# zengyan-97/X2-VLM

Hardware: AMD Instinct MI355X
Metric: image-text pairs/sec (fwd+bwd) X2VLM-base 224px bs=64/GPU (higher is better)
Workload: dtype bf16

## Files before the change

include/x2vlm_hip.h:

```cpp
#ifndef X2VLM_HIP_H
#define X2VLM_HIP_H
#include <stdint.h>
#ifdef __cplusplus
extern "C" {
#endif

const char* x2_last_error(void);
int x2_abi_version(void);
int x2_device_cus(void);
int x2_tune(int key, int value);
int x2_tune_get(int key);

int x2_gemm_nt(const void* A, const void* B, void* C, int M, int N, int K, int lda, int ldb, int ldc,
               const float* bias, const float* gamma, const float* resid, int ldr, void* aux, int ldaux,
               int act, int out_f32, unsigned drop_thr16, unsigned drop_seed, float drop_scale, const unsigned* drop_epoch,
               const float* rowscale, float* colsum, void* stream);

int x2_gemm_nt_dgelu_colparts(const void* A, const void* B, void* C, int M, int N, int K, int lda, int ldb, int ldc,
                              const void* aux, int ldaux, float* colparts, int* nrows_out, void* stream);
int x2_gemm_nt_splitk(const void* A, const void* B, float* C, int M, int N, int K, int lda, int ldb, int ldc,
                      int slices, float* ws, long ws_floats, void* stream);

int x2_gemm_tn_grouped(const int64_t* problems, int count, int accumulate, int split, float* ws, long ws_floats,
                       void* stream);

typedef struct X2AttnArgs {
  const void *Q, *K, *V, *O, *dO;
  void *Out, *dQ, *dK, *dV, *dS;
  float *LSE, *Delta;
  long q_bs, q_rs, k_bs, k_rs, v_bs, v_rs, o_bs, o_rs;
  long dq_bs, dq_rs, dk_bs, dk_rs, dv_bs, dv_rs, do_bs, do_rs;
  int B, Bkv, H, Lq, Lk;
  float scale;
  const float* bias;  int bias_ld;
  const float* biasT; int biasT_ld;
  const float* mask;  int mask_ld;
  const int* kv_idx;
  const int* seq_off; const int* seq_ids;
  int ds_ld;
  unsigned drop_thr16, drop_seed; float drop_scale;
  int dbg;
  int head_dim;
  const unsigned* drop_epoch;
  int grid_nx, grid_ny, grid_nz, grid_map;
  int phase;
  float* ws; long ws_floats;
  float* colsum_ws;
} X2AttnArgs;
int x2_attn_fwd(const X2AttnArgs* args, void* stream);
int x2_attn_bwd(const X2AttnArgs* args, void* stream);
int x2_attn_bwd_one_pass(const X2AttnArgs* args);

int x2_layernorm_fwd(const float* x, const float* w, const float* b, void* y_bf16, float* y_f32, float* mean,
                     float* rstd, int rows, int D, float eps, int period, unsigned drop_thr16, unsigned drop_seed,
                     float drop_scale, const unsigned* drop_epoch, void* stream);
int x2_layernorm_bwd(const void* dy , int dy_is_bf16, const float* x, const float* mean, const float* rstd, const float* w,
                     const float* dres, float* dx, void* dx_bf16, float* dw, float* db, float* dcol, int rows, int D,
                     int period, unsigned in_thr16, unsigned in_seed, float in_scale, unsigned out_thr16,
                     unsigned out_seed, float out_scale, const unsigned* drop_epoch, float* ws ,
                     int defer, int post, const float* post_rowscale, void* stream);
int x2_colsum_bf16(const void* y, float* out, int M, int N, int ld, float* ws , int defer, void* stream);
int x2_reduce_partials(const float* part, int nblk, int nk, int width, float* o0, float* o1, float* o2, void* stream);
int x2_reduce_partials_multi(const int64_t* desc, int count, void* stream);
int x2_layerscale_finish(const int64_t* desc, int count, void* stream);
int x2_rowscale_cast_colsum(const float* dx, const float* rowscale, void* dx_bf16, float* colsum, int M, int D,
                            float* ws , int defer, void* stream);
int x2_cast_bf16(const float* src, void* dst, long n, void* stream);
int x2_cast_transpose_bf16(const float* src, void* dst, void* dstT, int R, int C, int ldt, void* stream);
int x2_cast_transpose_multi(const int64_t* desc, int count, void* stream);
int x2_copy_f32_multi(const int64_t* desc, int count, void* stream);
int x2_patchify(const float* image, void* cols, int B, int R, int ps, void* stream);
int x2_assemble_tokens(const float* patch, const float* cls, float* x, int B, int P, int D, void* stream);
int x2_assemble_tokens_bwd(const float* dx, void* dpatch_bf16, float* dcls, int B, int P, int D, void* stream);
int x2_pool_tokens(float* x, const float* w, int B, int P, int D, int bwd, void* stream);
int x2_relpos_bias(const float* table, const long* index, const long* indexT , float* bias, float* biasT, int N, int H, int ld, int ldT,
                   float scale, void* stream);
int x2_relpos_bias_bwd(const void* dS, const int* inv_off, const int* inv_pos, float* dtable, int B, int N, int H, int ld,
                       int T, float* ws, int slices, void* stream);

int x2_embed_fwd(const long* ids, const float* word, const float* pos, const float* type0, float* out, int R, int L,
                 int D, void* stream);
int x2_embed_bwd(const long* ids, const float* g, float* dword, float* dpos, float* dtype0, int R, int L, int D,
                 float* scratch, void* stream);
int x2_gather_rows(const float* src, const int* idx, float* dst, void* dst_bf16, int R, long len, void* stream);
int x2_scatter_rows(const float* src, const int* idx, float* dst, int R, int D, long len, void* stream);
int x2_linear_f32(const float* A, const float* B, float* C, const float* bias, const float* alpha_ptr, float alpha,
                  int M, int N, int K, long sam, long sak, long sbn, long sbk, long ldc, int accumulate,
                  int ksplit ,
                  float* ws , void* stream);
int x2_l2norm(const float* x, const float* dy, float* out, int R, int D, int bwd, void* stream);
int x2_ce_fwd(const float* logits, long ld, const long* labels, int R, int C, float* lse, float* loss_row, float* out2,
              void* stream);
int x2_ce_bwd(const float* logits, long ld, const long* labels, const float* lse, const float* g, const float* stat,
              float gscale, int R, int C, float* dl_f32, void* dl_bf16, long ldd, void* stream);
int x2_mlm_ce_fwd(const void* X, const void* E, const float* bias, const long* labels, int R, int Vp, int V, int Hd,
                  int ldx, int lde, float* part, float* zlab, void* stream);
int x2_ce_combine(const float* part, int chunks, const float* zlab, const long* labels, int R, float* lse, float* loss_row,
                  float* out2, void* stream);
int x2_mlm_ce_bwd(const void* X, const void* E, const float* bias, const long* labels, const float* lse, const float* g,
                  const float* stat, float gscale, int R, int Vp, int V, int Hd, int ldx, int lde, void* dl_bf16, long ldd,
                  void* stream);
int x2_mask_tokens(const long* text_ids, const long* text_atts, int B, int L, const unsigned char* is_subword, int vocab,
                   const unsigned* words, int words_ld, unsigned seed, const unsigned* epoch, double mask_prob, int max_masks,
                   double skipgram_prb, int skipgram_size, int mask_whole_word, long cls_id, long mask_id, long pad_id, long pad_mask,
                   long* text_ids_masked, long* masked_pos, long* masked_ids, void* stream);
int x2_sample_negatives(const float* sim, int n, const long* group, const float* u, int* out, void* stream);
int x2_additive_mask(const long* atts, float* out, int S, int L, int Lp, float neg, void* stream);

int x2_attn_fwd_mask2d(const X2AttnArgs* args, const float* mask2d, int mask2d_ld, void* stream);
int x2_attn_bwd_mask2d(const X2AttnArgs* args, const float* mask2d, int mask2d_ld, void* stream);
int x2_additive_mask2d(const long* m, float* out, int S, int L, int Lp, float neg, void* stream);
int x2_embed_fwd_pid(const long* ids, const long* pids, const float* word, const float* pos, const float* type0, float* out, int R, int D,
                     void* stream);
int x2_embed_bwd_pid(const long* ids, const long* pids, const float* g, float* dword, float* dpos, float* dtype0, int R, int L, int D,
                     float* scratch, void* stream);
int x2_mlm_ls_fwd(const void* X, const void* E, const float* bias, const long* labels, long ignore, int R, int Vp, int V, int Hd, int ldx,
                  int lde, float* part, float* sumz, float* zlab, float* zign, void* stream);
int x2_ls_combine(const float* part, const float* sumz, int chunks, const float* zlab, const float* zign, const long* labels, const float* w,
                  int R, int V, long ignore, float ls, float* lse, float* kl_row, float* out2, void* stream);
int x2_mlm_ls_bwd(const void* X, const void* E, const float* bias, const long* labels, const float* w, const float* lse, const float* g,
                  const float* stat, float gscale, float ls, long ignore, int R, int Vp, int V, int Hd, int ldx, int lde, void* dl_bf16,
                  long ldd, void* stream);
int x2_kv_csr(const int* kv, int S, int Bi, int* off, int* order, void* stream);
int x2_tail_index(const int* ineg, const int* tneg, const long* text_atts , const long* image_atts , int B, int L,
                  int T, int with_match, int* t_idx, int* kv, long* atts_out , long* enc_out , void* stream);
int x2_droppath_rows(const float* rates, unsigned seed, const unsigned* epoch, int depth, int B, int T, float* out, void* stream);
int x2_frame_mean(const float* x, const float* pos, const float* dy, float* out, float* dpos, int Bc, int F, int T, int D, int bwd,
                  void* stream);
int x2_gelu_f32(const float* x, const float* dy, float* out, long n, void* stream);
int x2_colsum_f32(const float* x, float* out, int M, int N, void* stream);

int x2_attn_decode(const void* qkv, int qkv_ld, void* cache, void* out, int out_ld, int S, int H, int n_new, int hist, int Lmax, float scale,
                   void* stream);
int x2_beam_gather(const void* src, void* dst, const int* parent, int layers, int S, int Lmax, int row_elems, int hist, void* stream);
int x2_logprob_topk(const float* logits, int ldv, int V, int S, const int* seq, int Lseq, int seq_len, int ngram, int eos_id, int forbid_eos,
                    int K, float* out_vals, int* out_ids, float* logs, void* stream);

int x2_grad_norm(const void* table, int ntensors, int nblocks, float max_norm, float* partial, float* out2, void* stream);
int x2_adamw_multi(const void* table, int ntensors, int nblocks, const float* lr, const float* wd, int ngroups, float b1,
                   float b2, float eps, const float* clip2 , void* stream);

int x2_comm_unique_id(void* out128);
int x2_comm_init(const void* id128, int rank, int world, void** comm_out);
int x2_comm_info(void* comm, int* rank, int* world);
int x2_comm_allreduce_bucket(void* comm, void* buf, long count, int dtype, int average, void* done_event, void* stream);
int x2_comm_allgather(void* comm, const void* send, void* recv, long count_per_rank, int dtype, void* done_event, void* stream);
int x2_comm_broadcast(void* comm, void* buf, long count, int dtype, int root, void* done_event, void* stream);
int x2_comm_destroy(void* comm);

#ifdef __cplusplus
}
#endif
#endif
```

x2-vlm_amd/_lib.py:

```python
import ctypes as C
import os

import torch

_HERE = os.path.dirname(os.path.abspath(__file__))
LIB_PATH = os.environ.get("X2VLM_HIP_LIB") or os.path.join(_HERE, "libx2vlm_hip.so")

P, I, L, F, U = C.c_void_p, C.c_int, C.c_long, C.c_float, C.c_uint


class AttnArgs(C.Structure):
    _fields_ = [(n, P) for n in ("Q", "K", "V", "O", "dO", "Out", "dQ", "dK", "dV", "dS", "LSE", "Delta")] + \
               [(n, L) for n in ("q_bs", "q_rs", "k_bs", "k_rs", "v_bs", "v_rs", "o_bs", "o_rs",
                                 "dq_bs", "dq_rs", "dk_bs", "dk_rs", "dv_bs", "dv_rs", "do_bs", "do_rs")] + \
               [(n, I) for n in ("B", "Bkv", "H", "Lq", "Lk")] + [("scale", F)] + \
               [("bias", P), ("bias_ld", I), ("biasT", P), ("biasT_ld", I), ("mask", P), ("mask_ld", I),
                ("kv_idx", P), ("seq_off", P), ("seq_ids", P), ("ds_ld", I),
                ("drop_thr16", C.c_uint), ("drop_seed", C.c_uint), ("drop_scale", F), ("dbg", I), ("head_dim", I), ("drop_epoch", P),
                ("grid_nx", I), ("grid_ny", I), ("grid_nz", I), ("grid_map", I),
                ("phase", I), ("ws", P), ("ws_floats", L), ("colsum_ws", P)]


_SIGS = {
    "x2_gemm_nt": [P, P, P, I, I, I, I, I, I, P, P, P, I, P, I, I, I, U, U, F, P, P, P, P],
    "x2_gemm_nt_splitk": [P, P, P, I, I, I, I, I, I, I, P, L, P],
    "x2_gemm_nt_dgelu_colparts": [P, P, P, I, I, I, I, I, I, P, I, P, C.POINTER(I), P],
    "x2_gemm_tn_grouped": [P, I, I, I, P, L, P],
    "x2_attn_fwd": [C.POINTER(AttnArgs), P],
    "x2_attn_bwd": [C.POINTER(AttnArgs), P],
    "x2_layernorm_fwd": [P, P, P, P, P, P, P, I, I, F, I, U, U, F, P, P],
    "x2_layernorm_bwd": [P, I, P, P, P, P, P, P, P, P, P, P, I, I, I, U, U, F, U, U, F, P, P, I, I, P, P],
    "x2_colsum_bf16": [P, P, I, I, I, P, I, P],
    "x2_reduce_partials": [P, I, I, I, P, P, P, P],
    "x2_reduce_partials_multi": [P, I, P],
    "x2_cast_transpose_multi": [P, I, P],
    "x2_copy_f32_multi": [P, I, P],
    "x2_layerscale_finish": [P, I, P],
    "x2_rowscale_cast_colsum": [P, P, P, P, I, I, P, I, P],
    "x2_cast_bf16": [P, P, L, P],
    "x2_cast_transpose_bf16": [P, P, P, I, I, I, P],
    "x2_patchify": [P, P, I, I, I, P],
    "x2_assemble_tokens": [P, P, P, I, I, I, P],
    "x2_assemble_tokens_bwd": [P, P, P, I, I, I, P],
    "x2_pool_tokens": [P, P, I, I, I, I, P],
    "x2_relpos_bias": [P, P, P, P, P, I, I, I, I, F, P],
    "x2_relpos_bias_bwd": [P, P, P, P, I, I, I, I, I, P, I, P],
    "x2_embed_fwd": [P, P, P, P, P, I, I, I, P],
    "x2_embed_bwd": [P, P, P, P, P, I, I, I, P, P],
    "x2_gather_rows": [P, P, P, P, I, L, P],
    "x2_scatter_rows": [P, P, P, I, I, L, P],
    "x2_linear_f32": [P, P, P, P, P, F, I, I, I, L, L, L, L, L, I, I, P, P],
    "x2_l2norm": [P, P, P, I, I, I, P],
    "x2_ce_fwd": [P, L, P, I, I, P, P, P, P],
    "x2_ce_bwd": [P, L, P, P, P, P, F, I, I, P, P, L, P],
    "x2_mlm_ce_fwd": [P, P, P, P, I, I, I, I, I, I, P, P, P],
    "x2_ce_combine": [P, I, P, P, I, P, P, P, P],
    "x2_mlm_ce_bwd": [P, P, P, P, P, P, P, F, I, I, I, I, I, I, P, L, P],
    "x2_sample_negatives": [P, I, P, P, P, P],
    "x2_mask_tokens": [P, P, I, I, P, I, P, I, U, P, C.c_double, I, C.c_double, I, I, L, L, L, L, P, P, P, P],
    "x2_additive_mask": [P, P, I, I, I, F, P],
    "x2_kv_csr": [P, I, I, P, P, P],
    "x2_tail_index": [P, P, P, P, I, I, I, I, P, P, P, P, P],
    "x2_droppath_rows": [P, U, P, I, I, I, P, P],
    "x2_frame_mean": [P, P, P, P, P, I, I, I, I, I, P],
    "x2_gelu_f32": [P, P, P, L, P],
    "x2_grad_norm": [P, I, I, F, P, P, P],
    "x2_adamw_multi": [P, I, I, P, P, I, F, F, F, P, P],
    "x2_colsum_f32": [P, P, I, I, P],
    "x2_attn_fwd_mask2d": [C.POINTER(AttnArgs), P, I, P],
    "x2_attn_bwd_mask2d": [C.POINTER(AttnArgs), P, I, P],
    "x2_additive_mask2d": [P, P, I, I, I, F, P],
    "x2_embed_fwd_pid": [P, P, P, P, P, P, I, I, P],
    "x2_embed_bwd_pid": [P, P, P, P, P, P, I, I, I, P, P],
    "x2_mlm_ls_fwd": [P, P, P, P, L, I, I, I, I, I, I, P, P, P, P, P],
    "x2_ls_combine": [P, P, I, P, P, P, P, I, I, L, F, P, P, P, P],
    "x2_mlm_ls_bwd": [P, P, P, P, P, P, P, P, F, F, L, I, I, I, I, I, I, P, L, P],
    "x2_attn_decode": [P, I, P, P, I, I, I, I, I, I, F, P],
    "x2_beam_gather": [P, P, P, I, I, I, I, I, P],
    "x2_logprob_topk": [P, I, I, I, P, I, I, I, I, I, I, P, P, P, P],
}
_COMM_SIGS = {
    "x2_comm_unique_id": [P],
    "x2_comm_init": [P, I, I, C.POINTER(P)],
    "x2_comm_info": [P, C.POINTER(I), C.POINTER(I)],
    "x2_comm_allreduce_bucket": [P, P, L, I, I, P, P],
    "x2_comm_allgather": [P, P, P, L, I, P, P],
    "x2_comm_broadcast": [P, P, L, I, I, P, P],
    "x2_comm_destroy": [P],
}
EXPORTS = sorted(list(_SIGS) + list(_COMM_SIGS) + ["x2_last_error", "x2_abi_version", "x2_device_cus", "x2_tune", "x2_tune_get",
                                                         "x2_attn_bwd_one_pass"])

_lib = None


class X2HipError(RuntimeError):
    pass


def lib():
    global _lib
    if _lib is None:
        if not os.path.exists(LIB_PATH):
            raise X2HipError("HIP extension %s not built: run `python -c 'import __graft_entry__ as g; g.build()'`"
                             % LIB_PATH)
        try:
            h = C.CDLL(LIB_PATH)
        except OSError as e:
            raise X2HipError("cannot load %s: %s" % (LIB_PATH, e))
        for name, sig in list(_SIGS.items()) + list(_COMM_SIGS.items()):
            fn = getattr(h, name)
            fn.argtypes, fn.restype = sig, I
        h.x2_last_error.restype = C.c_char_p
        h.x2_abi_version.restype = I
        h.x2_device_cus.restype = I
        h.x2_tune.argtypes, h.x2_tune.restype = [I, I], I
        h.x2_tune_get.argtypes, h.x2_tune_get.restype = [I], I
        h.x2_attn_bwd_one_pass.argtypes, h.x2_attn_bwd_one_pass.restype = [C.POINTER(AttnArgs)], I
        for kv in filter(None, os.environ.get("X2_TUNE", "").split(",")):
            k, v = kv.split("=")
            if h.x2_tune(int(k), int(v)) != 0:
                raise X2HipError("X2_TUNE=%s: %s" % (kv, h.x2_last_error().decode()))
        _lib = h
    return _lib


_get_device = torch._C._cuda_getDevice if hasattr(torch._C, "_cuda_getDevice") else None
_get_raw_stream = getattr(torch._C, "_cuda_getCurrentRawStream", None)


def raw_stream():
    return _get_raw_stream(_get_device())


def call(name, *args):
    h = _lib or lib()
    rc = getattr(h, name)(*args, _get_raw_stream(_get_device()))
    if rc != 0:
        raise X2HipError("%s failed (%d): %s" % (name, rc, h.x2_last_error().decode()))


def ptr(t):
    return None if t is None else t.data_ptr()
```

x2-vlm_amd/csrc/gemm.hip:

```cpp
#include "x2_common.h"
#include <type_traits>

#define BM 128
#define BN 128
#define BK 64
#define TILE_BYTES (128 * 128)
#define STAGE_BYTES (2 * TILE_BYTES)
#define GEMM_LDS_BYTES (2 * STAGE_BYTES)

struct GemmNT {
  const bf16_t* A; const bf16_t* B; void* C;
  const float* bias; const float* gamma; const float* resid; bf16_t* aux;
  int M, N, K;
  int lda, ldb, ldc, ldr, ldaux;
  int act;
  int out_f32;
  int group_m;
  DropSpec drop;
  const uint32_t* drop_epoch;
  const float* rowscale;
  float* colsum;
  int dbg;
  int ksplit;
  const long* ce_labels;
  const float* ce_lse;
  const float* ce_g;
  const float* ce_stat;
  float* ce_part;
  float* ce_zlab;
  float ce_gscale;
  int ce_C;
  float* ce_sumz;
  float* ce_zign;
  long ce_ignore;
  float ce_ls;
  const float* ce_w;
};

__device__ __forceinline__ void tile_coords(int t, int tiles_m, int tiles_n, int gm, int& tm, int& tn) {
  const int gsz = gm * tiles_n, g = t / gsz, first = g * gm;
  const int rows = min(gm, tiles_m - first), r = t - g * gsz;
  tm = first + r % rows;
  tn = r / rows;
}

__device__ __forceinline__ void st16(void* p, u32x4 v, bool wt) {
  if (wt) asm volatile("global_store_dwordx4 %0, %1, off sc1\n\ts_nop 1" ::"v"(p), "v"(v) : "memory");
  else *reinterpret_cast<u32x4*>(p) = v;
}

#ifdef X2_PROBE
#define NT_DBG(p, bit) (((p).dbg & (bit)) != 0)
static __device__ unsigned long long* g_nt_probe = nullptr;
#define NT_STAMP(i) do { if (g_nt_probe && threadIdx.x == 0) g_nt_probe[(size_t)blockIdx.x * 4 + (i)] = wall_clock64(); } while (0)
#define NT_ABL_DECL(p) const bool abl_dma_ = NT_DBG(p, 32), abl_rd_ = NT_DBG(p, 64), abl_mm_ = NT_DBG(p, 128); bool rd_ = true
#define NT_ABL_NO_DMA(kt) if (abl_dma_ && (kt) >= 2) return
#define NT_ABL_NO_READ() if (!rd_) return
#define NT_ABL_NO_MFMA() if (abl_mm_) return
#define NT_ABL_STEP(kt) if (abl_rd_ && (kt) > 0) rd_ = false
#else
#define NT_ABL_DECL(p)
#define NT_ABL_NO_DMA(kt)
#define NT_ABL_NO_READ()
#define NT_ABL_NO_MFMA()
#define NT_ABL_STEP(kt)
#define NT_DBG(p, bit) false
#define NT_STAMP(i) do { } while (0)
#endif
typedef __attribute__((ext_vector_type(16))) float f32x16;
template <int TM>
__device__ __forceinline__ void epi_stage_half(f32x4 (&acc)[TM][4], int half, bool full, float* stg, int lane) {
  const int frow = lane & 15, fg = lane >> 4;
#pragma unroll
  for (int ii = 0; ii < 2; ++ii)
#pragma unroll
    for (int j = 0; j < 4; ++j)
      if (full || ii == 0) *reinterpret_cast<f32x4*>(stg + (ii * 16 + frow) * 68 + j * 16 + fg * 4) = acc[full ? half * 2 + ii : half * 2][j];
}
template <int RT>
__device__ __forceinline__ void epi_stage_half(f32x16 (&acc)[RT][2], int half, bool, float* stg, int lane) {
  const int row = lane & 31, h = lane >> 5;
#pragma unroll
  for (int tj = 0; tj < 2; ++tj)
#pragma unroll
    for (int g = 0; g < 4; ++g)
      *reinterpret_cast<f32x4*>(stg + row * 68 + tj * 32 + g * 8 + h * 4) =
          f32x4{acc[half][tj][4 * g], acc[half][tj][4 * g + 1], acc[half][tj][4 * g + 2], acc[half][tj][4 * g + 3]};
}
template <int V> struct EpiTraits {
  static constexpr bool generic = V == 4;
  static constexpr int act = V == 2 ? 1 : (V == 3 || V == 10) ? 2 : 0;
  static constexpr bool out_f32 = V == 1 || V == 5 || V == 6 || V == 7;
  static constexpr bool resid = V == 5 || V == 6;
  static constexpr bool scale = V == 6;
  static constexpr bool aux0 = false;
  static constexpr bool drop = V == 5;
  static constexpr bool colsum = false;
  static constexpr bool colparts = V == 10;
};
template <int TM, int VAR, class Acc>
__device__ __forceinline__ void nt_epilogue(const GemmNT& p, Acc& acc, char* smem, int wave, int lane, int mw0, int nw0, int prow = 0) {
  using E = EpiTraits<VAR>;
  const int act = E::generic ? p.act : E::act;
  const bool out_f32 = E::generic ? p.out_f32 != 0 : E::out_f32;
  const bool has_resid = E::generic ? p.resid != nullptr : E::resid;
  const bool has_scale = E::generic ? (p.gamma != nullptr || p.rowscale != nullptr) : E::scale;
  const bool has_aux0 = E::generic ? (p.act == 0 && p.aux != nullptr) : E::aux0;
  const bool has_drop = (E::generic || E::drop) ? p.drop.thr16 != 0 : false;
  const bool has_colsum = E::generic ? p.colsum != nullptr : (E::colsum && p.colsum != nullptr);
  float* stg = reinterpret_cast<float*>(smem) + wave * (32 * 68);
  const int er = lane >> 3, ec = (lane & 7) * 8;
  const int n = nw0 + ec;
  const bool nok = n < p.N;
  float bb[8], gg[8];
#pragma unroll
  for (int e = 0; e < 8; ++e) { bb[e] = 0.f; gg[e] = 1.f; }
  if (nok && p.bias) { const float4 b0 = *reinterpret_cast<const float4*>(p.bias + n), b1 = *reinterpret_cast<const float4*>(p.bias + n + 4);
    bb[0] = b0.x; bb[1] = b0.y; bb[2] = b0.z; bb[3] = b0.w; bb[4] = b1.x; bb[5] = b1.y; bb[6] = b1.z; bb[7] = b1.w; }
  if (nok && has_scale && p.gamma) { const float4 g0 = *reinterpret_cast<const float4*>(p.gamma + n), g1 = *reinterpret_cast<const float4*>(p.gamma + n + 4);
    gg[0] = g0.x; gg[1] = g0.y; gg[2] = g0.z; gg[3] = g0.w; gg[4] = g1.x; gg[5] = g1.y; gg[6] = g1.z; gg[7] = g1.w; }
  float cs[8] = {0.f, 0.f, 0.f, 0.f, 0.f, 0.f, 0.f, 0.f};
  const bool wt = NT_DBG(p, 16);
  const DropSpec drop_ = drop_at_epoch(p.drop, p.drop_epoch);
#pragma unroll
  for (int half = 0; half < (TM + 1) / 2; ++half) {
    const bool full = half * 2 + 1 < TM;
    float4 r0[4], r1[4];
    u32x4 pre[4];
    const int nc = nok ? n : 0;
    if (has_resid) {
#pragma unroll
      for (int rr = 0; rr < 4; ++rr) {
        if (!full && rr >= 2) continue;
        const int mc = min(mw0 + half * 32 + rr * 8 + er, p.M - 1);
        r0[rr] = *reinterpret_cast<const float4*>(p.resid + (size_t)mc * p.ldr + nc);
        r1[rr] = *reinterpret_cast<const float4*>(p.resid + (size_t)mc * p.ldr + nc + 4);
      }
    }
    if (act == 2) {
#pragma unroll
      for (int rr = 0; rr < 4; ++rr) {
        if (!full && rr >= 2) continue;
        const int mc = min(mw0 + half * 32 + rr * 8 + er, p.M - 1);
        pre[rr] = *reinterpret_cast<const u32x4*>(p.aux + (size_t)mc * p.ldaux + nc);
      }
    }
    epi_stage_half(acc, half, full, stg, lane);
#pragma unroll
    for (int rr = 0; rr < 4; ++rr) {
      if (!full && rr >= 2) continue;
      const int row = rr * 8 + er;
      const int m = mw0 + half * 32 + row;
      const float4 a0 = *reinterpret_cast<const float4*>(stg + row * 68 + ec), a1 = *reinterpret_cast<const float4*>(stg + row * 68 + ec + 4);
      if (m >= p.M || !nok) continue;
      float v[8] = {a0.x + bb[0], a0.y + bb[1], a0.z + bb[2], a0.w + bb[3], a1.x + bb[4], a1.y + bb[5], a1.z + bb[6], a1.w + bb[7]};
      if constexpr (VAR == 8) {
        const long lab = p.ce_labels[m];
        float mx = -INFINITY;
#pragma unroll
        for (int e = 0; e < 8; ++e) mx = n + e < p.ce_C ? fmaxf(mx, v[e]) : mx;
        mx = fmaxf(mx, __shfl_xor(mx, 1, 64)); mx = fmaxf(mx, __shfl_xor(mx, 2, 64)); mx = fmaxf(mx, __shfl_xor(mx, 4, 64));
        float se = 0.f;
#pragma unroll
        for (int e = 0; e < 8; ++e) {
          se += n + e < p.ce_C ? __expf(v[e] - mx) : 0.f;
          if ((long)(n + e) == lab) p.ce_zlab[m] = v[e];
        }
        se += __shfl_xor(se, 1, 64); se += __shfl_xor(se, 2, 64); se += __shfl_xor(se, 4, 64);
        if ((lane & 7) == 0) *reinterpret_cast<float2*>(p.ce_part + ((size_t)m * (p.N >> 6) + (nw0 >> 6)) * 2) = float2{mx, se};
        continue;
      }
      if constexpr (VAR == 11) {
        const long lab = p.ce_labels[m];
        float mx = -INFINITY, sz = 0.f;
#pragma unroll
        for (int e = 0; e < 8; ++e) { mx = n + e < p.ce_C ? fmaxf(mx, v[e]) : mx; sz += n + e < p.ce_C ? v[e] : 0.f; }
        mx = fmaxf(mx, __shfl_xor(mx, 1, 64)); mx = fmaxf(mx, __shfl_xor(mx, 2, 64)); mx = fmaxf(mx, __shfl_xor(mx, 4, 64));
        sz += __shfl_xor(sz, 1, 64); sz += __shfl_xor(sz, 2, 64); sz += __shfl_xor(sz, 4, 64);
        float se = 0.f;
#pragma unroll
        for (int e = 0; e < 8; ++e) {
          se += n + e < p.ce_C ? __expf(v[e] - mx) : 0.f;
          if ((long)(n + e) == lab) p.ce_zlab[m] = v[e];
          if ((long)(n + e) == p.ce_ignore) p.ce_zign[m] = v[e];
        }
        se += __shfl_xor(se, 1, 64); se += __shfl_xor(se, 2, 64); se += __shfl_xor(se, 4, 64);
        if ((lane & 7) == 0) {
          *reinterpret_cast<float2*>(p.ce_part + ((size_t)m * (p.N >> 6) + (nw0 >> 6)) * 2) = float2{mx, se};
          p.ce_sumz[(size_t)m * (p.N >> 6) + (nw0 >> 6)] = sz;
        }
        continue;
      }
      if constexpr (VAR == 12) {
        const long lab = p.ce_labels[m];
        const bool live = lab >= 0 && lab != p.ce_ignore;
        const float conf = 1.f - p.ce_ls, sm = p.ce_ls / (float)(p.ce_C - 2), qsum = conf + sm * (float)(p.ce_C - 2);
        const float sc = live ? p.ce_gscale * p.ce_g[0] * p.ce_w[m] / (p.ce_stat[1] + 1e-5f) : 0.f, l = p.ce_lse[m];
#pragma unroll
        for (int e = 0; e < 8; ++e) {
          const long c = n + e;
          const float q = c == lab ? conf : (c == p.ce_ignore ? 0.f : sm);
          v[e] = c < p.ce_C ? (qsum * __expf(v[e] - l) - q) * sc : 0.f;
        }
        st16(reinterpret_cast<bf16_t*>(p.C) + (size_t)m * p.ldc + n,
             u32x4{pack_bf16(v[0], v[1]), pack_bf16(v[2], v[3]), pack_bf16(v[4], v[5]), pack_bf16(v[6], v[7])}, false);
        continue;
      }
      if constexpr (VAR == 9) {
        const long lab = p.ce_labels[m];
        const float sc = lab >= 0 ? p.ce_gscale * p.ce_g[0] / p.ce_stat[1] : 0.f, l = p.ce_lse[m];
#pragma unroll
        for (int e = 0; e < 8; ++e) v[e] = n + e < p.ce_C ? (__expf(v[e] - l) - ((long)(n + e) == lab ? 1.f : 0.f)) * sc : 0.f;
        st16(reinterpret_cast<bf16_t*>(p.C) + (size_t)m * p.ldc + n,
             u32x4{pack_bf16(v[0], v[1]), pack_bf16(v[2], v[3]), pack_bf16(v[4], v[5]), pack_bf16(v[6], v[7])}, false);
        continue;
      }
      if (act == 1) {
        st16(p.aux + (size_t)m * p.ldaux + n, u32x4{pack_bf16(v[0], v[1]), pack_bf16(v[2], v[3]), pack_bf16(v[4], v[5]), pack_bf16(v[6], v[7])}, wt);
#pragma unroll
        for (int r = 0; r < 8; ++r) v[r] = gelu_f(v[r]);
      } else if (act == 2) {
#pragma unroll
        for (int r = 0; r < 4; ++r) { v[2 * r] *= dgelu_f(bf_lo(pre[rr][r])); v[2 * r + 1] *= dgelu_f(bf_hi(pre[rr][r])); }
      } else if (has_aux0) {
        st16(p.aux + (size_t)m * p.ldaux + n, u32x4{pack_bf16(v[0], v[1]), pack_bf16(v[2], v[3]), pack_bf16(v[4], v[5]), pack_bf16(v[6], v[7])}, wt);
      }
      if (has_drop) {
        float dm[4];
        drop_mul4(drop_, (uint32_t)m * (uint32_t)p.N + (uint32_t)n, dm);
        v[0] *= dm[0]; v[1] *= dm[1]; v[2] *= dm[2]; v[3] *= dm[3];
        drop_mul4(drop_, (uint32_t)m * (uint32_t)p.N + (uint32_t)n + 4u, dm);
        v[4] *= dm[0]; v[5] *= dm[1]; v[6] *= dm[2]; v[7] *= dm[3];
      }
      if (has_scale) {
        const float rs_ = p.rowscale ? p.rowscale[m] : 1.f;
#pragma unroll
        for (int r = 0; r < 8; ++r) v[r] *= gg[r] * rs_;
      }
      if (has_resid) {
        v[0] += r0[rr].x; v[1] += r0[rr].y; v[2] += r0[rr].z; v[3] += r0[rr].w;
        v[4] += r1[rr].x; v[5] += r1[rr].y; v[6] += r1[rr].z; v[7] += r1[rr].w;
      }
      if (has_colsum || E::colparts) {
#pragma unroll
        for (int r = 0; r < 8; ++r) cs[r] += v[r];
      }
      if (out_f32) {
        float* c = reinterpret_cast<float*>(p.C) + (size_t)m * p.ldc + n;
        st16(c, u32x4{__float_as_uint(v[0]), __float_as_uint(v[1]), __float_as_uint(v[2]), __float_as_uint(v[3])}, wt);
        st16(c + 4, u32x4{__float_as_uint(v[4]), __float_as_uint(v[5]), __float_as_uint(v[6]), __float_as_uint(v[7])}, wt);
      } else {
        st16(reinterpret_cast<bf16_t*>(p.C) + (size_t)m * p.ldc + n,
             u32x4{pack_bf16(v[0], v[1]), pack_bf16(v[2], v[3]), pack_bf16(v[4], v[5]), pack_bf16(v[6], v[7])}, wt);
      }
    }
  }
  if constexpr (E::colparts) {
#pragma unroll
    for (int e = 0; e < 8; ++e) { cs[e] += __shfl_xor(cs[e], 8, 64); cs[e] += __shfl_xor(cs[e], 16, 64); cs[e] += __shfl_xor(cs[e], 32, 64); }
    if (er == 0 && nok) {
      float* dst = p.colsum + (size_t)prow * p.N + n;
      *reinterpret_cast<float4*>(dst) = float4{cs[0], cs[1], cs[2], cs[3]};
      *reinterpret_cast<float4*>(dst + 4) = float4{cs[4], cs[5], cs[6], cs[7]};
    }
  }
  if (has_colsum) {
#pragma unroll
    for (int e = 0; e < 8; ++e) { cs[e] += __shfl_xor(cs[e], 8, 64); cs[e] += __shfl_xor(cs[e], 16, 64); cs[e] += __shfl_xor(cs[e], 32, 64); }
    if (er == 0 && nok) {
#pragma unroll
      for (int e = 0; e < 8; ++e) atomicAdd(p.colsum + n + e, cs[e]);
    }
  }
}

template <int TM, int VAR, class Acc>
__device__ __forceinline__ void nt_epilogue_f4(const GemmNT& p, Acc& acc, char* smem, int wave, int lane, int mw0, int nw0) {
  using E = EpiTraits<VAR>;
  static_assert(!E::generic && E::out_f32 && E::act == 0 && VAR <= 6, "nt_epilogue_f4: feature sets 1, 5, 6");
  const bool has_drop = E::drop ? p.drop.thr16 != 0 : false;
  float* stg = reinterpret_cast<float*>(smem) + wave * (32 * 68);
  const int er = lane >> 4, ec = (lane & 15) * 4;
  const int n = nw0 + ec;
  const bool nok = n < p.N;
  float bb[4] = {0.f, 0.f, 0.f, 0.f}, gg[4] = {1.f, 1.f, 1.f, 1.f};
  if (nok && p.bias) { const float4 b0 = *reinterpret_cast<const float4*>(p.bias + n); bb[0] = b0.x; bb[1] = b0.y; bb[2] = b0.z; bb[3] = b0.w; }
  if (E::scale && nok && p.gamma) { const float4 g0 = *reinterpret_cast<const float4*>(p.gamma + n); gg[0] = g0.x; gg[1] = g0.y; gg[2] = g0.z; gg[3] = g0.w; }
  const DropSpec drop_ = drop_at_epoch(p.drop, p.drop_epoch);
#pragma unroll
  for (int half = 0; half < (TM + 1) / 2; ++half) {
    const bool full = half * 2 + 1 < TM;
    float4 rs[4][2];
    const int nc = nok ? n : 0;
    if (E::resid) {
#pragma unroll
      for (int rr = 0; rr < 4; ++rr) {
        if (!full && rr >= 2) continue;
#pragma unroll
        for (int h = 0; h < 2; ++h) {
          const int mc = min(mw0 + half * 32 + rr * 8 + h * 4 + er, p.M - 1);
          rs[rr][h] = *reinterpret_cast<const float4*>(p.resid + (size_t)mc * p.ldr + nc);
        }
      }
    }
    epi_stage_half(acc, half, full, stg, lane);
#pragma unroll
    for (int rr = 0; rr < 4; ++rr) {
      if (!full && rr >= 2) continue;
#pragma unroll
      for (int h = 0; h < 2; ++h) {
        const int row = rr * 8 + h * 4 + er;
        const int m = mw0 + half * 32 + row;
        const float4 a0 = *reinterpret_cast<const float4*>(stg + row * 68 + ec);
        if (m >= p.M || !nok) continue;
        float v[4] = {a0.x + bb[0], a0.y + bb[1], a0.z + bb[2], a0.w + bb[3]};
        if (has_drop) {
          float dm[4];
          drop_mul4(drop_, (uint32_t)m * (uint32_t)p.N + (uint32_t)n, dm);
          v[0] *= dm[0]; v[1] *= dm[1]; v[2] *= dm[2]; v[3] *= dm[3];
        }
        if (E::scale) {
          const float rs_ = p.rowscale ? p.rowscale[m] : 1.f;
#pragma unroll
          for (int r = 0; r < 4; ++r) v[r] *= gg[r] * rs_;
        }
        if (E::resid) { v[0] += rs[rr][h].x; v[1] += rs[rr][h].y; v[2] += rs[rr][h].z; v[3] += rs[rr][h].w; }
        st16(reinterpret_cast<float*>(p.C) + (size_t)m * p.ldc + n,
             u32x4{__float_as_uint(v[0]), __float_as_uint(v[1]), __float_as_uint(v[2]), __float_as_uint(v[3])}, false);
      }
    }
  }
}

template <int TM, int VAR, bool F4 = false>
__global__ __launch_bounds__(256, 2) void gemm_nt_kernel(GemmNT p) {
  constexpr int BMT = 32 * TM;
  if constexpr (VAR == 7) {
    const int koff = blockIdx.y * p.ksplit;
    p.A += koff; p.B += koff;
    p.K = min(p.ksplit, p.K - koff);
    p.C = reinterpret_cast<float*>(p.C) + (size_t)blockIdx.y * p.M * p.ldc;
  }
  constexpr int A_BYTES = BMT * 128, STG = A_BYTES + TILE_BYTES;
  extern __shared__ __attribute__((aligned(16))) char smem[];
  const int tid = threadIdx.x, lane = tid & 63;
  const int wave = __builtin_amdgcn_readfirstlane(tid >> 6);
  const int wm = wave >> 1, wn = wave & 1;
  const int tiles_n = (p.N + BN - 1) / BN, tiles_m = (p.M + BMT - 1) / BMT;
  int tm, tn;
  tile_coords(xcd_remap(blockIdx.x, gridDim.x), tiles_m, tiles_n, p.group_m, tm, tn);
  const int m0 = tm * BMT, n0 = tn * BN;

  const bf16_t* srcA[TM]; const bf16_t* srcB[4];
#pragma unroll
  for (int i = 0; i < TM; ++i) {
    const int q = i * 256 + tid, row = q >> 3, c = (q & 7) ^ (row & 7);
    int ra = m0 + row; ra = ra < p.M ? ra : p.M - 1;
    srcA[i] = p.A + (size_t)ra * p.lda + c * 8;
  }
#pragma unroll
  for (int i = 0; i < 4; ++i) {
    const int q = i * 256 + tid, row = q >> 3, c = (q & 7) ^ (row & 7);
    int rb = n0 + row; rb = rb < p.N ? rb : p.N - 1;
    srcB[i] = p.B + (size_t)rb * p.ldb + c * 8;
  }
  auto stage = [&](int kt, int buf) {
    char* base = smem + buf * STG;
#pragma unroll
    for (int i = 0; i < TM; ++i) glds16(srcA[i] + (size_t)kt * BK, base + (i * 256 + wave * 64) * 16);
#pragma unroll
    for (int i = 0; i < 4; ++i) glds16(srcB[i] + (size_t)kt * BK, base + A_BYTES + (i * 256 + wave * 64) * 16);
  };

  f32x4 acc[TM][4];
#pragma unroll
  for (int i = 0; i < TM; ++i)
#pragma unroll
    for (int j = 0; j < 4; ++j) acc[i][j] = f32x4{0.f, 0.f, 0.f, 0.f};

  const uint32_t lds0 = lds_addr(smem);
  const int frow = lane & 15, fg = lane >> 4, fsw = lane & 7;
  const uint32_t offA = (uint32_t)((wm * 16 * TM + frow) * 128);
  const uint32_t offB = (uint32_t)(A_BYTES + (wn * 64 + frow) * 128);

  const int nk = p.K / BK;
  bf16x8 a0[TM], b0[4], a1[TM], b1[4];
  auto frags = [&](uint32_t sb, int ks, bf16x8 (&a)[TM], bf16x8 (&b)[4]) {
    const uint32_t cs = (uint32_t)(((ks * 4 + fg) ^ fsw) << 4);
#pragma unroll
    for (int j = 0; j < 4; ++j) b[j] = lds_read_b128(sb + offB + j * 2048 + cs);
#pragma unroll
    for (int i = 0; i < TM; ++i) a[i] = lds_read_b128(sb + offA + i * 2048 + cs);
  };
  auto mma = [&](bf16x8 (&a)[TM], bf16x8 (&b)[4], auto first, auto last) {
#pragma unroll
    for (int t = decltype(first)::value; t < decltype(last)::value; ++t)
      acc[t >> 2][t & 3] = __builtin_amdgcn_mfma_f32_16x16x32_bf16(b[t & 3], a[t >> 2], acc[t >> 2][t & 3], 0, 0, 0);
  };
  using I0 = std::integral_constant<int, 0>; using I1 = std::integral_constant<int, 1>; using IN = std::integral_constant<int, 4 * TM>;
  auto step = [&](int kt, auto refill, auto has_next) {
    mma(a0, b0, I0{}, I1{});
// ... 619 lines not shown
  X2_REQUIRE(K % BK == 0, "x2_gemm_nt: K=%d must be a multiple of %d", K, BK);
  X2_REQUIRE(N % 8 == 0, "x2_gemm_nt: N=%d must be a multiple of 8", N);
  X2_REQUIRE(lda % 8 == 0 && ldb % 8 == 0 && ldc % 8 == 0, "x2_gemm_nt: leading dims must keep 16-byte rows");
  X2_REQUIRE(act == 0 || aux, "x2_gemm_nt: act=%d needs aux", act);
  X2_REQUIRE((!resid || ldr % 4 == 0) && (!aux || ldaux % 8 == 0), "x2_gemm_nt: ldr/ldaux alignment");
  GemmNT p{(const bf16_t*)A, (const bf16_t*)B, C, bias, gamma, resid, (bf16_t*)aux, M, N, K, lda, ldb, ldc, ldr, ldaux, act, out_f32,
           g_tune[0] > 0 ? g_tune[0] : 8, DropSpec{drop_thr16, drop_seed, drop_scale}, drop_epoch, rowscale, colsum, g_tune[2], 0};
  int var = 4;
  {
    const bool plain = !gamma && !rowscale && !drop_thr16 && !colsum;
    if (act == 1 && !out_f32 && !resid && plain) var = 2;
    else if (act == 2 && !out_f32 && !resid && plain) var = 3;
    else if (act == 0 && !aux && !resid && plain) var = out_f32 ? 1 : 0;
    else if (act == 0 && !aux && resid && out_f32 && !gamma && !rowscale && !colsum) var = 5;
    else if (act == 0 && !aux && resid && out_f32 && gamma && !drop_thr16 && !colsum) var = 6;
  }
  double eff256 = 0.0;
  int tmw = nt256_plan(M, N, &eff256);
  if (g_tune[3] >= 5 && g_tune[3] <= 8) tmw = g_tune[3];
  const bool light = var == 0 || var == 1;
  bool auto256 = (light || K >= 2048) && eff256 * 100.0 >= NT256_MIN_FILL && !(resid && M < 8192);
  if ((var == 5 || var == 6) && M >= 8192 && eff256 * 100.0 >= NT256_MIN_FILL) auto256 = true;
  if (var == 2 && eff256 * 100.0 >= 90.0) auto256 = true;
  const bool use256 = var != 4 && N % 8 == 0 && (g_tune[1] == 3 || (g_tune[1] == 0 && g_tune[3] == 0 && auto256));
  const bool pp_ok = var != 4 && ((size_t)(M - 1) * lda + K) * 2 < (1ull << 31) && ((size_t)(N - 1) * ldb + K) * 2 < (1ull << 31);
  int pp_h = 0;
  if (g_tune[15] >= 3 && g_tune[15] <= 6) pp_h = g_tune[15];
  else if (g_tune[15] == 0 && g_tune[1] == 0 && g_tune[3] == 0 && !use256 && K >= 2048 && (var == 0 || var == 1 || var == 5)) {
    const int cus = x2_cus(), tn256 = (N + 255) / 256;
    for (int h = 3; h <= 4 && !pp_h; ++h) {
      const int tiles = ((M + 32 * h - 1) / (32 * h)) * tn256;
      if (tiles <= cus && tiles * 10 >= cus * 7) pp_h = h;
    }
  }
  if (pp_ok && pp_h) {
    switch (var) {
      case 0: launch_nt_pp_h<0>(p, pp_h, (hipStream_t)stream); break;
      case 1: launch_nt_pp_h<1>(p, pp_h, (hipStream_t)stream); break;
      case 2: launch_nt_pp_h<2>(p, pp_h, (hipStream_t)stream); break;
      case 3: launch_nt_pp_h<3>(p, pp_h, (hipStream_t)stream); break;
      case 5: launch_nt_pp_h<5>(p, pp_h, (hipStream_t)stream); break;
      default: launch_nt_pp_h<6>(p, pp_h, (hipStream_t)stream); break;
    }
    return x2_check_launch("x2_gemm_nt");
  }
  if (use256) {
    switch (var) {
      case 0: launch_nt256_h<0>(p, tmw, (hipStream_t)stream); break;
      case 1: launch_nt256_h<1>(p, tmw, (hipStream_t)stream); break;
      case 2: launch_nt256_h<2>(p, tmw, (hipStream_t)stream); break;
      case 3: launch_nt256_h<3>(p, tmw, (hipStream_t)stream); break;
      case 5: launch_nt256_h<5>(p, tmw, (hipStream_t)stream); break;
      default: launch_nt256_h<6>(p, tmw, (hipStream_t)stream); break;
    }
  } else {
    const int t128 = ((M + 127) / 128) * ((N + BN - 1) / BN), t192 = ((M + 191) / 192) * ((N + BN - 1) / BN);
    const int t64 = ((M + 63) / 64) * ((N + BN - 1) / BN);
    const int slots = 2 * x2_cus();
    const bool use64 = g_tune[3] == 3 || (g_tune[3] == 0 && (t128 <= slots || (t128 <= slots + slots / 6 && K <= 1024)));
    const bool use192 = !use64 && (g_tune[3] == 2 || (g_tune[3] == 0 && t128 > slots && t192 <= slots));
    const int t160 = ((M + 159) / 160) * ((N + BN - 1) / BN);
    const bool use160 = g_tune[3] == 4 || (use192 && g_tune[3] == 0 && t160 <= slots);
#define X2_NT_LAUNCH(V, SW)                                                                          \
    do {                                                                                              \
      if (use64) launch_nt<2, V, SW>(p, t64, (hipStream_t)stream);                                    \
      else if (use160) launch_nt<5, V, SW>(p, t160, (hipStream_t)stream);                             \
      else if (use192) launch_nt<6, V, SW>(p, t192, (hipStream_t)stream);                             \
      else launch_nt<4, V, SW>(p, t128, (hipStream_t)stream);                                         \
    } while (0)
    switch (var) {
      case 0: X2_NT_LAUNCH(0, false); break;
      case 2: X2_NT_LAUNCH(2, false); break;
      case 3: X2_NT_LAUNCH(3, false); break;
      case 1: X2_NT_LAUNCH(1, true); break;
      case 5: X2_NT_LAUNCH(5, true); break;
      case 6: X2_NT_LAUNCH(6, true); break;
      default: X2_NT_LAUNCH(4, false); break;
    }
#undef X2_NT_LAUNCH
  }
  return x2_check_launch("x2_gemm_nt");
}

extern "C" int x2_gemm_nt_dgelu_colparts(const void* A, const void* B, void* C, int M, int N, int K, int lda, int ldb, int ldc,
                                         const void* aux, int ldaux, float* colparts, int* nrows_out, void* stream) {
  X2_REQUIRE(A && B && C && aux && colparts && nrows_out, "x2_gemm_nt_dgelu_colparts: null argument");
  X2_REQUIRE(M > 0 && N > 0 && K > 0 && K % BK == 0 && N % 8 == 0, "x2_gemm_nt_dgelu_colparts: M=%d N=%d K=%d", M, N, K);
  X2_REQUIRE(lda % 8 == 0 && ldb % 8 == 0 && ldc % 8 == 0 && ldaux % 8 == 0, "x2_gemm_nt_dgelu_colparts: leading dims must keep 16-byte rows");
  GemmNT p{(const bf16_t*)A, (const bf16_t*)B, C, nullptr, nullptr, nullptr, (bf16_t*)aux, M, N, K, lda, ldb, ldc, 0, ldaux, 2, 0,
           g_tune[0] > 0 ? g_tune[0] : 8, DropSpec{0u, 0u, 1.f}, nullptr, nullptr, colparts, 0, 0};
  const int tiles_n = (N + BN - 1) / BN, t128 = ((M + 127) / 128) * tiles_n, t192 = ((M + 191) / 192) * tiles_n, t64 = ((M + 63) / 64) * tiles_n;
  const int slots = 2 * x2_cus();
  const bool use64 = g_tune[3] == 3 || (g_tune[3] == 0 && (t128 <= slots || (t128 <= slots + slots / 6 && K <= 1024)));
  const bool use192 = !use64 && (g_tune[3] == 2 || (g_tune[3] == 0 && t128 > slots && t192 <= slots));
  if (use64) { launch_nt<2, 10, false>(p, t64, (hipStream_t)stream); *nrows_out = 2 * ((M + 63) / 64); }
  else if (use192) { launch_nt<6, 10, false>(p, t192, (hipStream_t)stream); *nrows_out = 2 * ((M + 191) / 192); }
  else { launch_nt<4, 10, false>(p, t128, (hipStream_t)stream); *nrows_out = 2 * ((M + 127) / 128); }
  return x2_check_launch("x2_gemm_nt_dgelu_colparts");
}

__global__ __launch_bounds__(256) void gemm_nt_sum_slices_kernel(const float* __restrict__ ws, float* __restrict__ C, int M, int N, int ldc, int S) {
  const long e = (long)blockIdx.x * 256 + threadIdx.x, per = (long)M * N / 4;
  if (e >= per) return;
  const int m = (int)(e * 4 / N), n = (int)(e * 4 % N);
  float4 o = *reinterpret_cast<const float4*>(ws + e * 4);
  for (int s_ = 1; s_ < S; ++s_) {
    const float4 v = *reinterpret_cast<const float4*>(ws + (size_t)s_ * M * N + e * 4);
    o.x += v.x; o.y += v.y; o.z += v.z; o.w += v.w;
  }
  *reinterpret_cast<float4*>(C + (size_t)m * ldc + n) = o;
}
extern "C" int x2_gemm_nt_splitk(const void* A, const void* B, float* C, int M, int N, int K, int lda, int ldb, int ldc,
                                 int slices, float* ws, long ws_floats, void* stream) {
  X2_REQUIRE(A && B && C && M > 0 && N > 0 && K > 0, "x2_gemm_nt_splitk: empty problem M=%d N=%d K=%d", M, N, K);
  X2_REQUIRE(K % BK == 0 && N % 8 == 0, "x2_gemm_nt_splitk: K=%d must be a multiple of %d, N=%d of 8", K, BK, N);
  X2_REQUIRE(lda % 8 == 0 && ldb % 8 == 0 && ldc % 4 == 0 && ldc >= N, "x2_gemm_nt_splitk: leading dims must keep 16-byte rows");
  X2_REQUIRE(slices >= 0, "x2_gemm_nt_splitk: slices=%d", slices);
  const int nk = K / BK, tiles_n = (N + BN - 1) / BN;
  const bool small = M <= 64;
  const int tiles = (small ? (M + 63) / 64 : (M + 127) / 128) * tiles_n;
  int S = slices;
  if (S == 0) { S = (2 * x2_cus() + tiles - 1) / tiles; if (S > nk / 8) S = nk / 8; }
  if (S > nk) S = nk;
  const long per = (long)M * N;
  if (ws == nullptr) S = 1;
  else if ((long)S * per > ws_floats) S = (int)(ws_floats / per);
  if (S < 1) S = 1;
  const int steps = (nk + S - 1) / S;
  S = (nk + steps - 1) / steps;
  GemmNT p{(const bf16_t*)A, (const bf16_t*)B, S > 1 ? (void*)ws : (void*)C, nullptr, nullptr, nullptr, nullptr, M, N, K, lda, ldb,
           S > 1 ? N : ldc, 0, 0, 0, 1, g_tune[0] > 0 ? g_tune[0] : 8, DropSpec{0u, 0u, 1.f}, nullptr, nullptr, nullptr, 0, steps * BK};
  if (small) hipLaunchKernelGGL((gemm_nt_kernel<2, 7>), dim3(tiles, S), dim3(256), 2 * (64 * 128 + TILE_BYTES), (hipStream_t)stream, p);
  else hipLaunchKernelGGL((gemm_nt_kernel<4, 7>), dim3(tiles, S), dim3(256), GEMM_LDS_BYTES, (hipStream_t)stream, p);
  if (S > 1)
    hipLaunchKernelGGL(gemm_nt_sum_slices_kernel, dim3((unsigned)((per / 4 + 255) / 256)), dim3(256), 0, (hipStream_t)stream, ws, C, M, N, ldc, S);
  return x2_check_launch("x2_gemm_nt_splitk");
}

static int launch_nt_ce(GemmNT& p, int var, hipStream_t stream) {
  const int tiles_n = (p.N + BN - 1) / BN, t128 = ((p.M + 127) / 128) * tiles_n, t64 = ((p.M + 63) / 64) * tiles_n;
  const bool use64 = t128 <= 2 * x2_cus();
  if (var == 8) {
    if (use64) hipLaunchKernelGGL((gemm_nt_kernel<2, 8>), dim3(t64), dim3(256), 2 * (64 * 128 + TILE_BYTES), stream, p);
    else hipLaunchKernelGGL((gemm_nt_kernel<4, 8>), dim3(t128), dim3(256), GEMM_LDS_BYTES, stream, p);
  } else if (var == 11) {
    if (use64) hipLaunchKernelGGL((gemm_nt_kernel<2, 11>), dim3(t64), dim3(256), 2 * (64 * 128 + TILE_BYTES), stream, p);
    else hipLaunchKernelGGL((gemm_nt_kernel<4, 11>), dim3(t128), dim3(256), GEMM_LDS_BYTES, stream, p);
  } else if (var == 12) {
    if (use64) hipLaunchKernelGGL((gemm_nt_kernel<2, 12>), dim3(t64), dim3(256), 2 * (64 * 128 + TILE_BYTES), stream, p);
    else hipLaunchKernelGGL((gemm_nt_kernel<4, 12>), dim3(t128), dim3(256), GEMM_LDS_BYTES, stream, p);
  } else {
    if (use64) hipLaunchKernelGGL((gemm_nt_kernel<2, 9>), dim3(t64), dim3(256), 2 * (64 * 128 + TILE_BYTES), stream, p);
    else hipLaunchKernelGGL((gemm_nt_kernel<4, 9>), dim3(t128), dim3(256), GEMM_LDS_BYTES, stream, p);
  }
  return 0;
}
static bool mlm_ce_shapes_ok(int R, int Vp, int V, int Hd, int ldx, int lde) {
  return R > 0 && V > 0 && V <= Vp && Vp % 64 == 0 && Hd > 0 && Hd % BK == 0 && ldx % 8 == 0 && lde % 8 == 0 && ldx >= Hd && lde >= Hd;
}
extern "C" int x2_mlm_ce_fwd(const void* X, const void* E, const float* bias, const long* labels, int R, int Vp, int V, int Hd,
                             int ldx, int lde, float* part, float* zlab, void* stream) {
  X2_REQUIRE(X && E && labels && part && zlab, "x2_mlm_ce_fwd: null argument");
  X2_REQUIRE(mlm_ce_shapes_ok(R, Vp, V, Hd, ldx, lde), "x2_mlm_ce_fwd: R=%d Vp=%d V=%d Hd=%d ldx=%d lde=%d", R, Vp, V, Hd, ldx, lde);
  GemmNT p{(const bf16_t*)X, (const bf16_t*)E, nullptr, bias, nullptr, nullptr, nullptr, R, Vp, Hd, ldx, lde, Vp, 0, 0, 0, 0,
           g_tune[0] > 0 ? g_tune[0] : 8, DropSpec{0u, 0u, 1.f}, nullptr, nullptr, nullptr, 0, 0,
           labels, nullptr, nullptr, nullptr, part, zlab, 1.f, V};
// ... 395 lines not shown
```

x2-vlm_amd/csrc/heads.hip:

```cpp
#include "x2_common.h"
#define SCATTER_MAX_R_E 8192

__global__ __launch_bounds__(256) void embed_fwd_kernel(const long* __restrict__ ids, const float* __restrict__ word,
                                                        const float* __restrict__ pos, const float* __restrict__ type0,
                                                        float* __restrict__ out, int R, int L, int D) {
  const int r = blockIdx.x;
  const long id = ids[r];
  const int l = r % L;
  for (int d = threadIdx.x * 4; d < D; d += 1024) {
    const float4 a = *reinterpret_cast<const float4*>(word + id * D + d), b = *reinterpret_cast<const float4*>(pos + (long)l * D + d),
                 c = *reinterpret_cast<const float4*>(type0 + d);
    *reinterpret_cast<float4*>(out + (long)r * D + d) = float4{a.x + b.x + c.x, a.y + b.y + c.y, a.z + b.z + c.z, a.w + b.w + c.w};
  }
}
extern "C" int x2_embed_fwd(const long* ids, const float* word, const float* pos, const float* type0, float* out, int R, int L, int D,
                            void* stream) {
  X2_REQUIRE(R > 0 && L > 0 && D % 4 == 0, "x2_embed_fwd: R=%d L=%d D=%d", R, L, D);
  hipLaunchKernelGGL(embed_fwd_kernel, dim3(R), dim3(256), 0, (hipStream_t)stream, ids, word, pos, type0, out, R, L, D);
  return x2_check_launch("x2_embed_fwd");
}
__global__ __launch_bounds__(1024) void embed_bwd_word_kernel(const long* __restrict__ ids, const float* __restrict__ g, float* dword, int R,
                                                              int D) {
  __shared__ uint32_t bm[SCATTER_MAX_R_E / 32];
  __shared__ uint16_t lst[SCATTER_MAX_R_E];
// ... 369 lines not shown
  const int s_ = (int)(e / Lp), l = (int)(e % Lp);
  out[e] = l < L ? (1.0f - (float)atts[(long)s_ * L + l]) * neg : 0.f;
}
extern "C" int x2_additive_mask(const long* atts, float* out, int S, int L, int Lp, float neg, void* stream) {
  X2_REQUIRE(atts && out && S > 0 && L > 0 && Lp >= L, "x2_additive_mask: S=%d L=%d Lp=%d", S, L, Lp);
  hipLaunchKernelGGL(additive_mask_kernel, dim3((unsigned)(((long)S * Lp + 255) / 256)), dim3(256), 0, (hipStream_t)stream, atts, out, S, L, Lp, neg);
  return x2_check_launch("x2_additive_mask");
}
__global__ __launch_bounds__(256) void kv_csr_kernel(const int* __restrict__ kv, int S, int Bi, int* __restrict__ off, int* __restrict__ order) {
  extern __shared__ int cnt[];
  __shared__ int part[256];
  for (int b = threadIdx.x; b <= Bi; b += 256) cnt[b] = 0;
  __syncthreads();
  for (int e = threadIdx.x; e < S; e += 256) atomicAdd(&cnt[kv[e]], 1);
  __syncthreads();
  const int per = (Bi + 255) / 256, b0 = threadIdx.x * per, b1 = min(Bi, b0 + per);
  int sum = 0;
  for (int b = b0; b < b1; ++b) sum += cnt[b];
  part[threadIdx.x] = sum;
  __syncthreads();
  if (threadIdx.x == 0) { int run = 0; for (int t = 0; t < 256; ++t) { const int v = part[t]; part[t] = run; run += v; } }
  __syncthreads();
  int run = part[threadIdx.x];
  for (int b = b0; b < b1; ++b) { const int v = cnt[b]; cnt[b] = run; run += v; }
  __syncthreads();
  if (threadIdx.x == 0) cnt[Bi] = S;
  __syncthreads();
  for (int b = threadIdx.x; b <= Bi; b += 256) off[b] = cnt[b];
  for (int b = threadIdx.x; b < Bi; b += 256) {
    int pos = cnt[b];
    const int end = cnt[b + 1];
    for (int e = 0; e < S && pos < end; ++e) if (kv[e] == b) order[pos++] = e;
  }
}
extern "C" int x2_kv_csr(const int* kv, int S, int Bi, int* off, int* order, void* stream) {
  X2_REQUIRE(kv && off && order && S > 0 && Bi > 0 && Bi <= 8192, "x2_kv_csr: S=%d Bi=%d (Bi <= 8192)", S, Bi);
  hipLaunchKernelGGL(kv_csr_kernel, dim3(1), dim3(256), (size_t)(Bi + 1) * sizeof(int), (hipStream_t)stream, kv, S, Bi, off, order);
  return x2_check_launch("x2_kv_csr");
}

__global__ __launch_bounds__(256) void gelu_f32_kernel(const float* __restrict__ x, const float* __restrict__ dy, float* out, long n) {
  const long i = blockIdx.x * 256L + threadIdx.x;
  if (i < n) out[i] = dy ? dy[i] * dgelu_f(x[i]) : gelu_f(x[i]);
}
extern "C" int x2_gelu_f32(const float* x, const float* dy, float* out, long n, void* stream) {
  X2_REQUIRE(n > 0, "x2_gelu_f32: n=%ld", n);
  hipLaunchKernelGGL(gelu_f32_kernel, dim3((int)((n + 255) / 256)), dim3(256), 0, (hipStream_t)stream, x, dy, out, n);
  return x2_check_launch("x2_gelu_f32");
}
__global__ __launch_bounds__(256) void colsum_f32_kernel(const float* __restrict__ x, float* out, int M, int N) {
  const int n = blockIdx.x * 256 + threadIdx.x;
  if (n >= N) return;
  float s = 0.f;
  for (int m = 0; m < M; ++m) s += x[(long)m * N + n];
  out[n] += s;
}
extern "C" int x2_colsum_f32(const float* x, float* out, int M, int N, void* stream) {
  X2_REQUIRE(M > 0 && N > 0, "x2_colsum_f32: M=%d N=%d", M, N);
  hipLaunchKernelGGL(colsum_f32_kernel, dim3((N + 255) / 256), dim3(256), 0, (hipStream_t)stream, x, out, M, N);
  return x2_check_launch("x2_colsum_f32");
}

__global__ __launch_bounds__(256) void tail_index_kernel(const int* __restrict__ ineg, const int* __restrict__ tneg,
                                                         const long* __restrict__ text_atts, const long* __restrict__ image_atts, int B, int L,
                                                         int T, int with_match, int* __restrict__ t_idx, int* __restrict__ kv,
                                                         long* __restrict__ atts_out, long* __restrict__ enc_out) {
  const int r = blockIdx.x, q = with_match ? r / B : 3, b = r % B;
  const int ti = q == 2 ? tneg[b] : (q == 3 ? B + b : b), ki = q == 1 ? ineg[b] : b;
  if (threadIdx.x == 0) { t_idx[r] = ti; kv[r] = ki; }
  const long* ta = text_atts + (long)(ti % B) * L;
  for (int l = threadIdx.x; l < L; l += 256) atts_out[(long)r * L + l] = ta[l];
  const long* ia = image_atts + (long)ki * T;
  for (int t = threadIdx.x; t < T; t += 256) enc_out[(long)r * T + t] = ia[t];
}
extern "C" int x2_tail_index(const int* ineg, const int* tneg, const long* text_atts, const long* image_atts, int B, int L, int T,
                             int with_match, int* t_idx, int* kv, long* atts_out, long* enc_out, void* stream) {
  X2_REQUIRE(text_atts && image_atts && t_idx && kv && atts_out && enc_out && B > 0 && L > 0 && T > 0, "x2_tail_index: B=%d L=%d T=%d", B, L, T);
  X2_REQUIRE(!with_match || (ineg && tneg), "x2_tail_index: with_match needs the negative indices");
  hipLaunchKernelGGL(tail_index_kernel, dim3(with_match ? 4 * B : B), dim3(256), 0, (hipStream_t)stream, ineg, tneg, text_atts, image_atts, B, L, T,
                     with_match, t_idx, kv, atts_out, enc_out);
  return x2_check_launch("x2_tail_index");
}

__global__ __launch_bounds__(256) void droppath_rows_kernel(const float* __restrict__ rates, uint32_t seed, const uint32_t* __restrict__ epoch,
                                                            int depth, int B, int T, float* __restrict__ out) {
  const long e = blockIdx.x * 256L + threadIdx.x, rows = (long)B * T;
  if (e >= 2L * depth * rows) return;
  const int lb = (int)(e / rows), b = (int)((e % rows) / T), l = lb >> 1;
  uint32_t s_ = seed;
  if (epoch) s_ = x2_hash(s_ + 0x9E3779B1u * epoch[0]);
  const uint32_t h = x2_hash(((uint32_t)lb * (uint32_t)B + (uint32_t)b) ^ s_);
  const float rate = rates[l], u = (float)(h >> 8) * (1.0f / 16777216.0f);
  out[e] = u >= rate ? 1.0f / (1.0f - rate) : 0.0f;
}
extern "C" int x2_droppath_rows(const float* rates, unsigned seed, const unsigned* epoch, int depth, int B, int T, float* out, void* stream) {
  X2_REQUIRE(rates && out && depth > 0 && B > 0 && T > 0, "x2_droppath_rows: depth=%d B=%d T=%d", depth, B, T);
  const long n = 2L * depth * B * T;
  hipLaunchKernelGGL(droppath_rows_kernel, dim3((unsigned)((n + 255) / 256)), dim3(256), 0, (hipStream_t)stream, rates, seed, epoch, depth, B, T, out);
  return x2_check_launch("x2_droppath_rows");
}

__global__ __launch_bounds__(256) void frame_mean_fwd_kernel(const float* __restrict__ x, const float* __restrict__ pos, float* __restrict__ out,
                                                             int Bc, int F, long TD, int D) {
  const long e = (blockIdx.x * 256L + threadIdx.x) * 4;
  if (e >= (long)Bc * TD) return;
  const long b = e / TD, o = e % TD;
  const int d = (int)(o % D);
  float4 a = float4{0.f, 0.f, 0.f, 0.f};
  for (int f = 0; f < F; ++f) {
    const float4 v = *reinterpret_cast<const float4*>(x + (b * F + f) * TD + o);
    float4 pp = float4{0.f, 0.f, 0.f, 0.f};
    if (pos) pp = *reinterpret_cast<const float4*>(pos + (long)f * D + d);
    a.x += v.x + pp.x; a.y += v.y + pp.y; a.z += v.z + pp.z; a.w += v.w + pp.w;
  }
  const float inv = 1.0f / (float)F;
  *reinterpret_cast<float4*>(out + e) = float4{a.x * inv, a.y * inv, a.z * inv, a.w * inv};
}
__global__ __launch_bounds__(256) void frame_mean_bwd_kernel(const float* __restrict__ dy, float* __restrict__ dx, int Bc, int F, long TD) {
  const long e = (blockIdx.x * 256L + threadIdx.x) * 4;
  if (e >= (long)Bc * TD) return;
  const long b = e / TD, o = e % TD;
  const float inv = 1.0f / (float)F;
  float4 g = *reinterpret_cast<const float4*>(dy + e);
  g.x *= inv; g.y *= inv; g.z *= inv; g.w *= inv;
  for (int f = 0; f < F; ++f) *reinterpret_cast<float4*>(dx + (b * F + f) * TD + o) = g;
}
__global__ __launch_bounds__(256) void frame_pos_grad_kernel(const float* __restrict__ dy, float* __restrict__ dpos, long rows, int D, int F) {
  __shared__ float sh[4][64];
  const int c = blockIdx.x * 64 + (threadIdx.x & 63), sl = threadIdx.x >> 6;
  float s = 0.f;
  if (c < D) for (long r = sl; r < rows; r += 4) s += dy[r * D + c];
  sh[sl][threadIdx.x & 63] = s;
  __syncthreads();
  if (sl == 0 && c < D) {
    const float v = (sh[0][threadIdx.x] + sh[1][threadIdx.x] + sh[2][threadIdx.x] + sh[3][threadIdx.x]) / (float)F;
    for (int f = 0; f < F; ++f) dpos[(long)f * D + c] = v;
  }
}
extern "C" int x2_frame_mean(const float* x, const float* pos, const float* dy, float* out, float* dpos, int Bc, int F, int T, int D, int bwd,
                             void* stream) {
  X2_REQUIRE(Bc > 0 && F > 0 && T > 0 && D > 0 && D % 4 == 0, "x2_frame_mean: Bc=%d F=%d T=%d D=%d", Bc, F, T, D);
  const long TD = (long)T * D, n4 = (long)Bc * TD / 4;
  if (!bwd) {
    X2_REQUIRE(x && out, "x2_frame_mean: forward needs x and out");
    hipLaunchKernelGGL(frame_mean_fwd_kernel, dim3((unsigned)((n4 + 255) / 256)), dim3(256), 0, (hipStream_t)stream, x, pos, out, Bc, F, TD, D);
  } else {
    X2_REQUIRE(dy && out, "x2_frame_mean: backward needs dy and out (= dx)");
    hipLaunchKernelGGL(frame_mean_bwd_kernel, dim3((unsigned)((n4 + 255) / 256)), dim3(256), 0, (hipStream_t)stream, dy, out, Bc, F, TD);
    if (dpos) hipLaunchKernelGGL(frame_pos_grad_kernel, dim3((D + 63) / 64), dim3(256), 0, (hipStream_t)stream, dy, dpos, (long)Bc * T, D, F);
  }
  return x2_check_launch("x2_frame_mean");
}

__global__ __launch_bounds__(256) void embed_fwd_pid_kernel(const long* __restrict__ ids, const long* __restrict__ pids, const float* __restrict__ word,
                                                            const float* __restrict__ pos, const float* __restrict__ type0, float* __restrict__ out, int D) {
  const int r = blockIdx.x;
  const long id = ids[r], l = pids[r];
  for (int d = threadIdx.x * 4; d < D; d += 1024) {
    const float4 a = *reinterpret_cast<const float4*>(word + id * D + d), b = *reinterpret_cast<const float4*>(pos + l * D + d),
                 c = *reinterpret_cast<const float4*>(type0 + d);
    *reinterpret_cast<float4*>(out + (long)r * D + d) = float4{a.x + b.x + c.x, a.y + b.y + c.y, a.z + b.z + c.z, a.w + b.w + c.w};
  }
}
extern "C" int x2_embed_fwd_pid(const long* ids, const long* pids, const float* word, const float* pos, const float* type0, float* out, int R, int D,
                                void* stream) {
  X2_REQUIRE(ids && pids && word && pos && type0 && out && R > 0 && D % 4 == 0, "x2_embed_fwd_pid: R=%d D=%d", R, D);
// ... 91 lines not shown
```

x2-vlm_amd/csrc/rowwise.hip:

```cpp
#include "x2_common.h"

__device__ __forceinline__ long remap_row(int r, int period) { return period > 0 ? (long)r + r / period + 1 : r; }

#define LN_MAXV 8
#define LN_DISPATCH(D, CALL) do { const int nv_ = ((D) + 255) / 256; \
  if (nv_ <= 1) { CALL(1); } else if (nv_ == 2) { CALL(2); } else if (nv_ == 3) { CALL(3); } else if (nv_ == 4) { CALL(4); } \
  else if (nv_ <= 6) { CALL(6); } else { CALL(8); } } while (0)
template <int NV>
__global__ __launch_bounds__(256) void layernorm_fwd_kernel(const float* __restrict__ x, const float* __restrict__ w,
                                                            const float* __restrict__ bsh, bf16_t* yb, float* yf,
                                                            float* mean, float* rstd, int rows, int D, float eps, int period,
                                                            DropSpec drop_in_, const uint32_t* __restrict__ epoch) {
  const int row = blockIdx.x * 4 + (threadIdx.x >> 6), lane = threadIdx.x & 63;
  if (row >= rows) return;
  const DropSpec drop = drop_at_epoch(drop_in_, epoch);
  const long gr = remap_row(row, period);
  const float* xr = x + gr * D;
  float4 v[NV];
  float s = 0.f;
  const int nv = D >> 2;
#pragma unroll
  for (int i = 0; i < NV; ++i) {
    const int c = lane + i * 64;
    if (c < nv) { v[i] = *reinterpret_cast<const float4*>(xr + c * 4); s += v[i].x + v[i].y + v[i].z + v[i].w; }
// ... 122 lines not shown
}
extern "C" int x2_reduce_partials(const float* part, int nblk, int nk, int width, float* o0, float* o1, float* o2, void* stream) {
  X2_REQUIRE(part && nblk > 0 && nk >= 1 && nk <= 3 && width > 0, "x2_reduce_partials: nblk=%d nk=%d width=%d", nblk, nk, width);
  launch_reduce(part, nblk, nk, width, o0, o1, o2, (hipStream_t)stream);
  return x2_check_launch("x2_reduce_partials");
}

#define RPM_MAX 16
struct ReduceDesc { const float* part; float* o[4]; int nblk, nk, width, blk0; };
struct ReduceGroup { ReduceDesc d[RPM_MAX]; int count; };
#define RPM_COLS 16
__global__ __launch_bounds__(256) void reduce_partials_multi_kernel(ReduceGroup g) {
  int e = 0;
#pragma unroll
  for (int i = 1; i < RPM_MAX; ++i) if (i < g.count && (int)blockIdx.x >= g.d[i].blk0) e = i;
  const ReduceDesc d = g.d[e];
  const int local = blockIdx.x - d.blk0, ctiles = (d.width + RPM_COLS - 1) / RPM_COLS;
  const int k = local / ctiles, cg = threadIdx.x & 3, sl = threadIdx.x >> 2;
  const int c = (local % ctiles) * RPM_COLS + cg * 4;
  __shared__ float4 red[63][4];
  float4 s = float4{0.f, 0.f, 0.f, 0.f};
  float* o = d.o[k];
  const bool vec = (d.width & 3) == 0;
  if (o && c < d.width) {
    const float* base = d.part + (size_t)k * d.width + c;
    const size_t rs = (size_t)d.nk * d.width;
    if (vec) {
      int b = sl;
      for (; b + 192 < d.nblk; b += 256) {
        const float4 v0 = *reinterpret_cast<const float4*>(base + (size_t)b * rs), v1 = *reinterpret_cast<const float4*>(base + (size_t)(b + 64) * rs),
                     v2 = *reinterpret_cast<const float4*>(base + (size_t)(b + 128) * rs), v3 = *reinterpret_cast<const float4*>(base + (size_t)(b + 192) * rs);
        s.x += (v0.x + v1.x) + (v2.x + v3.x); s.y += (v0.y + v1.y) + (v2.y + v3.y);
        s.z += (v0.z + v1.z) + (v2.z + v3.z); s.w += (v0.w + v1.w) + (v2.w + v3.w);
      }
      for (; b < d.nblk; b += 64) {
        const float4 v = *reinterpret_cast<const float4*>(base + (size_t)b * rs);
        s.x += v.x; s.y += v.y; s.z += v.z; s.w += v.w;
      }
    } else {
      for (int b = sl; b < d.nblk; b += 64) {
        const float* r = base + (size_t)b * rs;
        s.x += r[0]; if (c + 1 < d.width) s.y += r[1]; if (c + 2 < d.width) s.z += r[2]; if (c + 3 < d.width) s.w += r[3];
      }
    }
  }
  if (sl > 0) red[sl - 1][cg] = s;
  __syncthreads();
  if (sl == 0 && o && c < d.width) {
#pragma unroll 9
    for (int i = 0; i < 63; ++i) { const float4 v = red[i][cg]; s.x += v.x; s.y += v.y; s.z += v.z; s.w += v.w; }
    o[c] += s.x;
    if (c + 1 < d.width) o[c + 1] += s.y;
    if (c + 2 < d.width) o[c + 2] += s.z;
    if (c + 3 < d.width) o[c + 3] += s.w;
  }
}
extern "C" int x2_reduce_partials_multi(const int64_t* desc, int count, void* stream) {
  X2_REQUIRE(desc && count >= 1, "x2_reduce_partials_multi: count=%d", count);
  for (int i0 = 0; i0 < count; i0 += RPM_MAX) {
    ReduceGroup g; g.count = count - i0 < RPM_MAX ? count - i0 : RPM_MAX;
    int blocks = 0;
    for (int i = 0; i < g.count; ++i) {
      const int64_t* q = desc + (size_t)(i0 + i) * 8;
      ReduceDesc& d = g.d[i];
      d.part = (const float*)q[0]; d.nblk = (int)q[1]; d.nk = (int)q[2]; d.width = (int)q[3];
      d.o[0] = (float*)q[4]; d.o[1] = (float*)q[5]; d.o[2] = (float*)q[6]; d.o[3] = (float*)q[7];
      X2_REQUIRE(d.part && d.nblk > 0 && d.nk >= 1 && d.nk <= 4 && d.width > 0, "x2_reduce_partials_multi[%d]: nblk=%d nk=%d width=%d",
                 i0 + i, d.nblk, d.nk, d.width);
      d.blk0 = blocks;
      blocks += ((d.width + RPM_COLS - 1) / RPM_COLS) * d.nk;
    }
    hipLaunchKernelGGL(reduce_partials_multi_kernel, dim3(blocks), dim3(256), 0, (hipStream_t)stream, g);
  }
  return x2_check_launch("x2_reduce_partials_multi");
}

#define LNB_ROWS 16
template <int NV, int MODE>
__global__ __launch_bounds__(256, NV <= 3 ? 4 : 1) void layernorm_bwd_kernel(const void* __restrict__ dy_, const float* __restrict__ x,
                                                            const float* __restrict__ mean, const float* __restrict__ rstd,
                                                            const float* __restrict__ w, const float* dres, float* dx, bf16_t* dxb,
                                                            float* ws, int rows, int D, int period,
                                                            DropSpec din_, DropSpec dout_, const uint32_t* __restrict__ epoch,
                                                            const float* __restrict__ post_rs) {
  constexpr int NSET = 3;
  constexpr bool DYB = MODE != 0;
  extern __shared__ __attribute__((aligned(16))) float red[];
  const DropSpec din = drop_at_epoch(din_, epoch), dout = drop_at_epoch(dout_, epoch);
  const int lane = threadIdx.x & 63, wv = threadIdx.x >> 6;
  const int nv = D >> 2;
  float4 ww[NV], aw[NV], ab[NV], ac[NV];
#pragma unroll
  for (int i = 0; i < NV; ++i) {
    const int c = lane + i * 64;
    ww[i] = c < nv ? *reinterpret_cast<const float4*>(w + c * 4) : float4{0.f, 0.f, 0.f, 0.f};
    aw[i] = float4{0.f, 0.f, 0.f, 0.f}; ab[i] = float4{0.f, 0.f, 0.f, 0.f}; ac[i] = float4{0.f, 0.f, 0.f, 0.f};
  }
  const int r0 = blockIdx.x * LNB_ROWS, r1 = min(rows, r0 + LNB_ROWS);
  for (int row = r0 + wv; row < r1; row += 4) {
    const long gr = remap_row(row, period);
    const float mu = mean[row], rs = rstd[row];
    float4 g[NV], xh[NV];
    float s1 = 0.f, s2 = 0.f;
#pragma unroll
    for (int i = 0; i < NV; ++i) {
      const int c = lane + i * 64;
      if (c < nv) {
        float4 d;
        if constexpr (DYB) {
          const u32x2 raw = *reinterpret_cast<const u32x2*>(reinterpret_cast<const bf16_t*>(dy_) + gr * D + c * 4);
          d = float4{bf_lo(raw.x), bf_hi(raw.x), bf_lo(raw.y), bf_hi(raw.y)};
        } else {
          d = *reinterpret_cast<const float4*>(reinterpret_cast<const float*>(dy_) + gr * D + c * 4);
        }
        const float4 xv = *reinterpret_cast<const float4*>(x + gr * D + c * 4);
        if (din.thr16) {
          float dm[4];
          drop_mul4(din, (uint32_t)gr * (uint32_t)D + (uint32_t)(c * 4), dm);
          d.x *= dm[0]; d.y *= dm[1]; d.z *= dm[2]; d.w *= dm[3];
        }
        xh[i] = float4{(xv.x - mu) * rs, (xv.y - mu) * rs, (xv.z - mu) * rs, (xv.w - mu) * rs};
        g[i] = float4{d.x * ww[i].x, d.y * ww[i].y, d.z * ww[i].z, d.w * ww[i].w};
        s1 += g[i].x + g[i].y + g[i].z + g[i].w;
        s2 += g[i].x * xh[i].x + g[i].y * xh[i].y + g[i].z * xh[i].z + g[i].w * xh[i].w;
        aw[i].x += d.x * xh[i].x; aw[i].y += d.y * xh[i].y; aw[i].z += d.z * xh[i].z; aw[i].w += d.w * xh[i].w;
        ab[i].x += d.x; ab[i].y += d.y; ab[i].z += d.z; ab[i].w += d.w;
      }
    }
    const float m1 = wave_sum(s1) / D, m2 = wave_sum(s2) / D;
#pragma unroll
    for (int i = 0; i < NV; ++i) {
      const int c = lane + i * 64;
      if (c < nv) {
        float4 o{rs * (g[i].x - m1 - xh[i].x * m2), rs * (g[i].y - m1 - xh[i].y * m2), rs * (g[i].z - m1 - xh[i].z * m2), rs * (g[i].w - m1 - xh[i].w * m2)};
        float4 om = o;
        if (dout.thr16) {
          float dm[4];
          drop_mul4(dout, (uint32_t)gr * (uint32_t)D + (uint32_t)(c * 4), dm);
          om.x *= dm[0]; om.y *= dm[1]; om.z *= dm[2]; om.w *= dm[3];
        }
        if (dres) { const float4 rr = *reinterpret_cast<const float4*>(dres + gr * D + c * 4); o.x += rr.x; o.y += rr.y; o.z += rr.z; o.w += rr.w; }
        if (dx) *reinterpret_cast<float4*>(dx + gr * D + c * 4) = o;
        if constexpr (MODE == 2) { om = o; if (post_rs) { const float f = post_rs[gr]; om.x *= f; om.y *= f; om.z *= f; om.w *= f; } }
        ac[i].x += om.x; ac[i].y += om.y; ac[i].z += om.z; ac[i].w += om.w;
        if (dxb) *reinterpret_cast<u32x2*>(dxb + gr * D + c * 4) = u32x2{pack_bf16(om.x, om.y), pack_bf16(om.z, om.w)};
      }
    }
  }
  if (wv > 0) {
#pragma unroll
    for (int i = 0; i < NV; ++i) {
      const int c = lane + i * 64;
      if (c < nv) {
        *reinterpret_cast<float4*>(red + ((0 * 3 + wv - 1) * D) + c * 4) = aw[i];
        *reinterpret_cast<float4*>(red + ((1 * 3 + wv - 1) * D) + c * 4) = ab[i];
        *reinterpret_cast<float4*>(red + ((2 * 3 + wv - 1) * D) + c * 4) = ac[i];
      }
    }
  }
  __syncthreads();
  if (wv == 0) {
#pragma unroll
    for (int i = 0; i < NV; ++i) {
      const int c = lane + i * 64;
      if (c < nv) {
#pragma unroll
        for (int k = 0; k < 3; ++k) {
          const float4 a = *reinterpret_cast<const float4*>(red + ((0 * 3 + k) * D) + c * 4), b = *reinterpret_cast<const float4*>(red + ((1 * 3 + k) * D) + c * 4),
                       cc = *reinterpret_cast<const float4*>(red + ((2 * 3 + k) * D) + c * 4);
          aw[i].x += a.x; aw[i].y += a.y; aw[i].z += a.z; aw[i].w += a.w;
          ab[i].x += b.x; ab[i].y += b.y; ab[i].z += b.z; ab[i].w += b.w;
          ac[i].x += cc.x; ac[i].y += cc.y; ac[i].z += cc.z; ac[i].w += cc.w;
        }
        float* wp = ws + (long)blockIdx.x * NSET * D + c * 4;
        *reinterpret_cast<float4*>(wp) = aw[i];
        *reinterpret_cast<float4*>(wp + D) = ab[i];
        *reinterpret_cast<float4*>(wp + 2 * D) = ac[i];
      }
    }
  }
}

extern "C" int x2_layernorm_bwd(const void* dy, int dy_is_bf16, const float* x, const float* mean, const float* rstd, const float* w,
                                const float* dres, float* dx, void* dx_bf16, float* dw, float* db, float* dcol, int rows, int D,
                                int period, unsigned in_thr16, unsigned in_seed, float in_scale, unsigned out_thr16,
                                unsigned out_seed, float out_scale, const unsigned* drop_epoch, float* ws, int defer, int post,
                                const float* post_rowscale, void* stream) {
  X2_REQUIRE(rows > 0 && D > 0 && D % 4 == 0 && D <= 256 * LN_MAXV, "x2_layernorm_bwd: rows=%d D=%d", rows, D);
  X2_REQUIRE(dw && db && ws, "x2_layernorm_bwd: dw/db and the workspace ws[ceil(rows/%d)*3*D] are required", LNB_ROWS);
  X2_REQUIRE(post || !(dcol && dres), "x2_layernorm_bwd: dcol sums the LN-input gradient, which excludes dres (post = 0)");
  X2_REQUIRE(!(out_thr16 && dres), "x2_layernorm_bwd: an output mask applies to the bf16 copy, which excludes dres");
  X2_REQUIRE(!post || (dy_is_bf16 && dx_bf16 && dcol && !out_thr16 && period == 0),
             "x2_layernorm_bwd: post = 1 (by-products of the final output) takes a bf16 dy, dx_bf16 and dcol, no output mask, period 0");
#define X2_LNB_T(NV, B) hipLaunchKernelGGL((layernorm_bwd_kernel<NV, B>), dim3((rows + LNB_ROWS - 1) / LNB_ROWS), dim3(256), 9 * D * sizeof(float), \
                     (hipStream_t)stream, dy, x, mean, rstd, w, dres, dx, (bf16_t*)dx_bf16, ws, rows, D, period,                \
                     DropSpec{in_thr16, in_seed, in_scale}, DropSpec{out_thr16, out_seed, out_scale}, drop_epoch, post_rowscale)
#define X2_LNB(NV) do { if (post) X2_LNB_T(NV, 2); else if (dy_is_bf16) X2_LNB_T(NV, 1); else X2_LNB_T(NV, 0); } while (0)
  LN_DISPATCH(D, X2_LNB);
  if (!defer) launch_reduce(ws, (rows + LNB_ROWS - 1) / LNB_ROWS, 3, D, dw, db, dcol, (hipStream_t)stream);
  return x2_check_launch("x2_layernorm_bwd");
}

#define CS_ROWS 64
__global__ __launch_bounds__(256) void colsum_bf16_kernel(const bf16_t* __restrict__ y, float* ws, int M, int N, int ld) {
  __shared__ float red[3][512];
  const int tx = threadIdx.x & 63, ty = threadIdx.x >> 6;
  const int c0 = blockIdx.y * 512 + tx * 8;
  const int r0 = blockIdx.x * CS_ROWS, r1 = min(M, r0 + CS_ROWS);
  float acc[8] = {0.f, 0.f, 0.f, 0.f, 0.f, 0.f, 0.f, 0.f};
  if (c0 < N) {
#pragma unroll 4
    for (int r = r0 + ty; r < r1; r += 4) {
      const u32x4 v = *reinterpret_cast<const u32x4*>(y + (long)r * ld + c0);
#pragma unroll
      for (int e = 0; e < 4; ++e) { acc[2 * e] += bf_lo(v[e]); acc[2 * e + 1] += bf_hi(v[e]); }
    }
  }
  if (ty > 0) {
#pragma unroll
    for (int e = 0; e < 8; ++e) red[ty - 1][tx * 8 + e] = acc[e];
  }
  __syncthreads();
  if (ty == 0 && c0 < N) {
#pragma unroll
    for (int e = 0; e < 8; ++e) {
      const float v = acc[e] + red[0][tx * 8 + e] + red[1][tx * 8 + e] + red[2][tx * 8 + e];
      if (c0 + e < N) ws[(long)blockIdx.x * N + c0 + e] = v;
    }
  }
}
extern "C" int x2_colsum_bf16(const void* y, float* out, int M, int N, int ld, float* ws, int defer, void* stream) {
  X2_REQUIRE(M > 0 && N > 0 && N % 8 == 0 && ld % 8 == 0, "x2_colsum_bf16: M=%d N=%d ld=%d (N, ld multiples of 8)", M, N, ld);
  X2_REQUIRE(ws, "x2_colsum_bf16: workspace ws[ceil(M/%d)*N] required", CS_ROWS);
  hipLaunchKernelGGL(colsum_bf16_kernel, dim3((M + CS_ROWS - 1) / CS_ROWS, (N + 511) / 512), dim3(256), 0, (hipStream_t)stream,
                     (const bf16_t*)y, ws, M, N, ld);
  if (!defer) launch_reduce(ws, (M + CS_ROWS - 1) / CS_ROWS, 1, N, out, nullptr, nullptr, (hipStream_t)stream);
  return x2_check_launch("x2_colsum_bf16");
}

#define LS_ROWS 32
__global__ __launch_bounds__(256) void rowscale_cast_colsum_kernel(const float* __restrict__ dx, const float* __restrict__ rowscale,
                                                                   bf16_t* dxb, float* ws, int M, int D) {
  __shared__ float red[3][256];
  const int tx = threadIdx.x & 63, ty = threadIdx.x >> 6;
  const int c0 = blockIdx.y * 256 + tx * 4;
  const int r0 = blockIdx.x * LS_ROWS, r1 = min(M, r0 + LS_ROWS);
  float ab[4] = {0.f, 0.f, 0.f, 0.f};
  if (c0 < D) {
#pragma unroll 4
    for (int r = r0 + ty; r < r1; r += 4) {
      float4 d = *reinterpret_cast<const float4*>(dx + (long)r * D + c0);
      if (rowscale) { const float rs_ = rowscale[r]; d.x *= rs_; d.y *= rs_; d.z *= rs_; d.w *= rs_; }
      *reinterpret_cast<u32x2*>(dxb + (long)r * D + c0) = u32x2{pack_bf16(d.x, d.y), pack_bf16(d.z, d.w)};
      ab[0] += d.x; ab[1] += d.y; ab[2] += d.z; ab[3] += d.w;
    }
  }
  if (ty > 0) {
#pragma unroll
    for (int e = 0; e < 4; ++e) red[ty - 1][tx * 4 + e] = ab[e];
  }
  __syncthreads();
  if (ty == 0 && c0 < D) {
#pragma unroll
    for (int e = 0; e < 4; ++e) ws[(long)blockIdx.x * D + c0 + e] = ab[e] + red[0][tx * 4 + e] + red[1][tx * 4 + e] + red[2][tx * 4 + e];
  }
}
extern "C" int x2_rowscale_cast_colsum(const float* dx, const float* rowscale, void* dx_bf16, float* colsum, int M, int D, float* ws,
                                       int defer, void* stream) {
  X2_REQUIRE(dx && dx_bf16 && colsum && M > 0 && D > 0 && D % 4 == 0 && ws,
             "x2_rowscale_cast_colsum: M=%d D=%d (workspace ws[ceil(M/%d)*D] required)", M, D, LS_ROWS);
  hipLaunchKernelGGL(rowscale_cast_colsum_kernel, dim3((M + LS_ROWS - 1) / LS_ROWS, (D + 255) / 256), dim3(256), 0, (hipStream_t)stream, dx,
                     rowscale, (bf16_t*)dx_bf16, ws, M, D);
  if (!defer) launch_reduce(ws, (M + LS_ROWS - 1) / LS_ROWS, 1, D, colsum, nullptr, nullptr, (hipStream_t)stream);
  return x2_check_launch("x2_rowscale_cast_colsum");
}

#define LSF_MAX 8
struct LsfDesc { float* G; const float* W; const float* bias; const float* gamma; const float* cs; float* dgamma; float* dbias; int N, K, blk0; };
struct LsfGroup { LsfDesc d[LSF_MAX]; int count; };
__global__ __launch_bounds__(256) void layerscale_finish_kernel(LsfGroup g) {
  int e = 0;
#pragma unroll
  for (int i = 1; i < LSF_MAX; ++i) if (i < g.count && (int)blockIdx.x >= g.d[i].blk0) e = i;
// ... 406 lines not shown
```

x2-vlm_amd/engine.py:

```python
import itertools
import math
import weakref

import torch

from . import kernels as K
from ._lib import raw_stream

BF16, F32 = torch.bfloat16, torch.float32



_SERIAL = itertools.count(1)


def _tok(w):
    t = w.__dict__.get("_x2_serial")
    if t is None:
        t = w.__dict__["_x2_serial"] = next(_SERIAL)
    return t


class TScale:

# ... 493 lines not shown
                dxb = K.rowscale_cast_colsum(dx, G["_cs2"], rowscale=rs2)
            dpre = K.gemm_nt_dgelu_colsum(dxb, w2T, pre, G["mlp.fc1.bias"])
            dh2 = K.gemm_nt(dpre, w1T)
            dx1, dx1b = K.layernorm_bwd(dh2, x1, mean2, rstd2, p[b + "norm2.weight"], G["norm2.weight"], G["norm2.bias"], dres=dx,
                                        post=(rs1, G["_cs1"]))
            datt = K.gemm_nt(dx1b, wprojT)
            dqkv = torch.empty_like(qkv)
            delta = torch.empty_like(lse)
            po = []
            dS_i = torch.empty_like(dS) if WGRAD_QUEUE is not None else dS
            cs = torch.empty(B, 2, D, device=qkv.device, dtype=F32)
            form = K.attn_bwd(K.view3(qkv, B, T, 0), K.view3(qkv, B, T, D), K.view3(qkv, B, T, 2 * D), K.view3(att, B, T),
                              K.view3(datt, B, T), B, B, H, T, T, scale, lse, delta, K.view3(dqkv, B, T, 0), K.view3(dqkv, B, T, D),
                              K.view3(dqkv, B, T, 2 * D), dS=dS_i, bias=bias, biasT=biasT, bias_log2=True, colsum_ws=cs)
            fused_cs = form in (1, 3)
            if fused_cs:
                item = (cs, B, 2, D, (G["qkv_bias"][:D], G["qkv_bias"][2 * D:]))
                if K.DEFERRED is not None:
                    K.DEFERRED.append(item)
                else:
                    K.reduce_partials(*item)
            if WGRAD_QUEUE is not None:
                tbl_a, qb_a = G["attn.relative_position_bias_table"].detach(), G["qkv_bias"].detach()
                po.append(lambda dS_i=dS_i, tbl_a=tbl_a: K.relpos_bias_bwd(dS_i, meta["rel_index"], tbl_a))
                if not fused_cs:
                    po.append(lambda dqkv=dqkv, qb_a=qb_a: K.colsum_bf16(dqkv, qb_a))
            else:
                K.relpos_bias_bwd(dS_i, meta["rel_index"], G["attn.relative_position_bias_table"])
                if not fused_cs:
                    K.colsum_bf16(dqkv, G["qkv_bias"])
            G.alias("attn.q_bias", G["qkv_bias"][:D])
            G.alias("attn.v_bias", G["qkv_bias"][2 * D:])
            dh1 = K.gemm_nt(dqkv, wqkvT)
            if i > lo:
                below = (dpath[i - 1][1] if dpath is not None else None, arenas[i - 1]["_cs2"])
                dxn, dxnb = K.layernorm_bwd(dh1, x, mean1, rstd1, p[b + "norm1.weight"], G["norm1.weight"], G["norm1.bias"], dres=dx1, post=below)
            else:
                dxn, dxnb = K.layernorm_bwd(dh1, x, mean1, rstd1, p[b + "norm1.weight"], G["norm1.weight"], G["norm1.bias"], dres=dx1)
            tn = [(dxb, act, G["mlp.fc2.weight"]), (dpre, h2, G["mlp.fc1.weight"]),
                  (dx1b, att, G["attn.proj.weight"]), (dqkv, h1, G["attn.qkv.weight"])]
            fin = [(G["mlp.fc2.weight"], p[b + "mlp.fc2.weight"], p[b + "mlp.fc2.bias"], p[b + "gamma_2"], G["_cs2"], G["gamma_2"], G["mlp.fc2.bias"]),
                   (G["attn.proj.weight"], p[b + "attn.proj.weight"], p[b + "attn.proj.bias"], p[b + "gamma_1"], G["_cs1"], G["gamma_1"],
                    G["attn.proj.bias"])]
            pairs.add(G, tn, po, fin)
            for n in names:
                if n.startswith(b):
                    out[n] = G.g[n[len(b):]]
            dx, dxb = dxn, dxnb
        pairs.flush()
        if stem:
            dpatch = K.assemble_tokens_bwd(dx.view(B, T, D), Gs["cls_token"].view(-1))
            K.colsum_bf16(dpatch, Gs["patch_embed.proj.bias"])
            K.gemm_tn_grouped([(dpatch, ctx.cols, Gs["patch_embed.proj.weight"].view(D, -1))], accumulate=True,
                              split=8 if B * P_ >= 4096 else 1)
            SIDE.join()
            Gs.publish()
            out.update(Gs.g)
            return (None, None) + tuple(out[n] for n in names)
        SIDE.join()
        return (dx.view(B, T, D), None) + tuple(out[n] for n in names)



_ATT = ("self.query.weight", "self.query.bias", "self.key.weight", "self.key.bias", "self.value.weight", "self.value.bias",
        "output.dense.weight", "output.dense.bias", "output.LayerNorm.weight", "output.LayerNorm.bias")
_FFN = ("intermediate.dense.weight", "intermediate.dense.bias", "output.dense.weight", "output.dense.bias",
        "output.LayerNorm.weight", "output.LayerNorm.bias")


def bert_layer_param_names(lo, hi, fusion_at, with_cross):
    names = []
    for i in range(lo, hi):
        b = "layer.%d." % i
        names += [b + "attention." + s for s in _ATT]
        if with_cross and i >= fusion_at:
            names += [b + "crossattention." + s for s in _ATT]
        names += [b + s for s in _FFN]
    return names


class BertLayersFn(torch.autograd.Function):

    @staticmethod
    def prepare_weights(p, lo, hi, fusion_at, cross):
        groups, vecs = [], []
        for i in range(lo, hi):
            b = "layer.%d." % i
            a, c = b + "attention.", b + "crossattention."
            groups += [(p[a + "self.query.weight"], p[a + "self.key.weight"], p[a + "self.value.weight"]),
                       (p[a + "output.dense.weight"],), (p[b + "intermediate.dense.weight"],), (p[b + "output.dense.weight"],)]
            vecs.append((p[a + "self.query.bias"], p[a + "self.key.bias"], p[a + "self.value.bias"]))
            if cross and i >= fusion_at:
                groups += [(p[c + "self.query.weight"],), (p[c + "self.key.weight"], p[c + "self.value.weight"]),
                           (p[c + "output.dense.weight"],)]
                vecs.append((p[c + "self.key.bias"], p[c + "self.value.bias"]))
        BANK.prepare(groups)
        BANK.prepare_vectors(vecs)

    @staticmethod
    def _drop(meta, layer, kind):
        d = meta.get("drop")
        if not d:
            return K.NO_DROP
        return K.dropout_spec(d["p_attn"] if kind in (0, 2) else d["p_hidden"], d["seed"], 8 * layer + kind)

    @staticmethod
    def forward(ctx, hidden, enc, meta, *params):
        cross = enc is not None
        names = bert_layer_param_names(meta["lo"], meta["hi"], meta["fusion_at"], cross)
        p = dict(zip(names, params))
        S, L, Hd = hidden.shape
        H, eps = meta["heads"], meta["eps"]
        M = S * L
        assert Hd == 64 * H, "hidden size %d / %d heads: the attention kernels are built for head dim 64" % (Hd, H)
        scale = 1.0 / math.sqrt(Hd // H)
        dev = hidden.device
        h = hidden.contiguous().view(M, Hd)
        hb = K.cast_bf16(h)
        encb = None
        if cross:
            Bi, T, Dv = enc.shape
            encb = K.cast_bf16(enc.contiguous().view(Bi * T, Dv))
        BertLayersFn.prepare_weights(p, meta["lo"], meta["hi"], meta["fusion_at"], cross)
        saved = []
        kv_ahead = {}
        use_aux = cross and AUX.enabled and not (AUX.auto and K.attn_bwd_form(L, enc.shape[1], shared_kv=meta.get("seq_off") is not None,
                                                                               dropout=BertLayersFn._drop(meta, meta["hi"] - 1, 2)[0] != 0) == 2)
        if use_aux:
            for i in range(max(meta["lo"], meta["fusion_at"]), meta["hi"]):
                c = "layer.%d.crossattention." % i
                wkv, _ = BANK.linear(p[c + "self.key.weight"], p[c + "self.value.weight"])
                bkv = BANK.vector(p[c + "self.key.bias"], p[c + "self.value.bias"])
                kv = torch.empty(Bi * T, wkv.shape[0], device=dev, dtype=BF16)
                kv_ahead[i] = (kv, AUX.launch(lambda kv=kv, wkv=wkv, bkv=bkv: K.gemm_nt(encb, wkv, bias=bkv, out=kv), [encb, wkv, bkv, kv]))
        for i in range(meta["lo"], meta["hi"]):
            b = "layer.%d." % i
            a = b + "attention."
            wqkv, _ = BANK.linear(p[a + "self.query.weight"], p[a + "self.key.weight"], p[a + "self.value.weight"])
            bqkv = BANK.vector(p[a + "self.query.bias"], p[a + "self.key.bias"], p[a + "self.value.bias"])
            qkv = K.gemm_nt(hb, wqkv, bias=bqkv)
            att = torch.empty(M, Hd, device=dev, dtype=BF16)
            lse = torch.empty(S * H * L, device=dev, dtype=F32)
            dr = BertLayersFn._drop
            if meta.get("self_mask2d") is not None:
                K.attn_fwd_mask2d(K.view3(qkv, S, L, 0), K.view3(qkv, S, L, Hd), K.view3(qkv, S, L, 2 * Hd), S, H, L, scale,
                                  K.view3(att, S, L), lse, meta["self_mask2d"], drop=dr(meta, i, 0))
            else:
                K.attn_fwd(K.view3(qkv, S, L, 0), K.view3(qkv, S, L, Hd), K.view3(qkv, S, L, 2 * Hd), S, S, H, L, L, scale,
                           K.view3(att, S, L), lse, mask=meta["self_mask"], drop=dr(meta, i, 0))
            wo, _ = BANK.linear(p[a + "output.dense.weight"])
            s1 = K.gemm_nt(att, wo, bias=p[a + "output.dense.bias"], resid=h, out_dtype=F32, drop=dr(meta, i, 1))
            h1b, h1, m1, r1 = K.layernorm_fwd(s1, p[a + "output.LayerNorm.weight"], p[a + "output.LayerNorm.bias"], eps, want_f32=True)
            cr = None
            h2b, h2 = h1b, h1
            if cross and i >= meta["fusion_at"]:
                c = b + "crossattention."
                wq, _ = BANK.linear(p[c + "self.query.weight"])
                wkv, _ = BANK.linear(p[c + "self.key.weight"], p[c + "self.value.weight"])
                bkv = BANK.vector(p[c + "self.key.bias"], p[c + "self.value.bias"])
                q2 = K.gemm_nt(h1b, wq, bias=p[c + "self.query.bias"])
                if i in kv_ahead:
                    kv, ev = kv_ahead.pop(i)
                    if ev is not None:
                        torch.cuda.current_stream().wait_event(ev)
                else:
                    kv = K.gemm_nt(encb, wkv, bias=bkv)
                att2 = torch.empty(M, Hd, device=dev, dtype=BF16)
                lse2 = torch.empty(S * H * L, device=dev, dtype=F32)
                K.attn_fwd(K.view3(q2, S, L), K.view3(kv, Bi, T, 0), K.view3(kv, Bi, T, Hd), S, Bi, H, L, T, scale,
                           K.view3(att2, S, L), lse2, mask=meta["enc_mask"], kv_idx=meta["kv_idx"], seq_off=meta.get("seq_off"),
                           seq_ids=meta.get("seq_ids"), drop=dr(meta, i, 2))
                wo2, _ = BANK.linear(p[c + "output.dense.weight"])
                s2 = K.gemm_nt(att2, wo2, bias=p[c + "output.dense.bias"], resid=h1, out_dtype=F32, drop=dr(meta, i, 3))
                h2b, h2, m2, r2 = K.layernorm_fwd(s2, p[c + "output.LayerNorm.weight"], p[c + "output.LayerNorm.bias"], eps, want_f32=True)
                cr = (q2, kv, att2, lse2, s2, m2, r2)
            wi, _ = BANK.linear(p[b + "intermediate.dense.weight"])
            wout, _ = BANK.linear(p[b + "output.dense.weight"])
            pre = torch.empty(M, wi.shape[0], device=dev, dtype=BF16)
            act = K.gemm_nt(h2b, wi, bias=p[b + "intermediate.dense.bias"], aux=pre, act=1)
            s3 = K.gemm_nt(act, wout, bias=p[b + "output.dense.bias"], resid=h2, out_dtype=F32, drop=dr(meta, i, 4))
            h3b, h3, m3, r3 = K.layernorm_fwd(s3, p[b + "output.LayerNorm.weight"], p[b + "output.LayerNorm.bias"], eps, want_f32=True)
            saved.append((hb, qkv, att, lse, s1, m1, r1, h1b, cr, h2b, pre, act, s3, m3, r3))
            h, hb = h3, h3b
        AUX.join()
        for i in range(meta["lo"], meta["hi"]):
            _count_call(("bert", id(p["layer.%d.attention.self.query.weight" % i])))
        ctx.meta, ctx.saved, ctx.params, ctx.encb = meta, saved, params, encb
        ctx.dims = (S, L, Hd, H, M, scale, cross, enc.shape if cross else None)
        return h.view(S, L, Hd)

    @staticmethod
    def backward(ctx, dh_out):
        meta, params, encb = ctx.meta, ctx.params, ctx.encb
        BANK.note_backward()
        S, L, Hd, H, M, scale, cross, enc_shape = ctx.dims
        names = bert_layer_param_names(meta["lo"], meta["hi"], meta["fusion_at"], cross)
        p = dict(zip(names, params))
        dev = dh_out.device
        dh = dh_out.contiguous().view(M, Hd)
        denc = None
        out = {}
        if cross:
            Bi, T, Dv = enc_shape
        pairs = _LayerPairs()
        arenas = {}
        for li, i in enumerate(range(meta["lo"], meta["hi"])):
            b = "layer.%d." % i
            Ff = p[b + "intermediate.dense.weight"].shape[0]
            spec = [("a.qkv_bias", (3 * Hd,), True), ("attention.output.dense.bias", (Hd,), True),
                    ("attention.output.LayerNorm.weight", (Hd,), True), ("attention.output.LayerNorm.bias", (Hd,), True),
                    ("intermediate.dense.bias", (Ff,), True), ("output.dense.bias", (Hd,), True),
                    ("output.LayerNorm.weight", (Hd,), True), ("output.LayerNorm.bias", (Hd,), True),
                    ("a.qkv_weight", (3 * Hd, Hd), False), ("attention.output.dense.weight", (Hd, Hd), False),
                    ("intermediate.dense.weight", (Ff, Hd), False), ("output.dense.weight", (Hd, Ff), False)]
            if ctx.saved[li][8] is not None:
                spec += [("crossattention.self.query.bias", (Hd,), True), ("c.kv_bias", (2 * Hd,), True),
                         ("crossattention.output.dense.bias", (Hd,), True), ("crossattention.output.LayerNorm.weight", (Hd,), True),
                         ("crossattention.output.LayerNorm.bias", (Hd,), True), ("crossattention.self.query.weight", (Hd, Hd), False),
                         ("c.kv_weight", (2 * Hd, Dv), False), ("crossattention.output.dense.weight", (Hd, Hd), False)]
            arenas[i] = Grads(dev, spec, key=("bert", id(p[b + "attention.self.query.weight"])), params=[p[n] for n in names if n.startswith(b)],
                              zero=False)
        Grads.zero_all(list(arenas.values()))
        for li, i in reversed(list(enumerate(range(meta["lo"], meta["hi"])))):
            b = "layer.%d." % i
            a = b + "attention."
            hb, qkv, att, lse, s1, m1, r1, h1b, cr, h2b, pre, act, s3, m3, r3 = ctx.saved[li]
            ctx.saved[li] = None
            Ff = p[b + "intermediate.dense.weight"].shape[0]
            G = arenas.pop(i)
            tn, po = [], []
            _begin_layer_backward()
            ds3, ds3b = K.layernorm_bwd(dh, s3, m3, r3, p[b + "output.LayerNorm.weight"], G["output.LayerNorm.weight"],
                                        G["output.LayerNorm.bias"], dcol=G["output.dense.bias"], want_bf16=True,
                                        drop_out=BertLayersFn._drop(meta, i, 4))
            _, woutT = BANK.linear(p[b + "output.dense.weight"])
            _, wiT = BANK.linear(p[b + "intermediate.dense.weight"])
            dpre = K.gemm_nt_dgelu_colsum(ds3b, woutT, pre, G["intermediate.dense.bias"])
            dh2 = K.gemm_nt(dpre, wiT, resid=ds3, out_dtype=F32)
            tn += [(ds3b, act, G["output.dense.weight"]), (dpre, h2b, G["intermediate.dense.weight"])]
            if cr is not None:
                c = b + "crossattention."
                q2, kv, att2, lse2, s2, m2, r2 = cr
                ds2, ds2b = K.layernorm_bwd(dh2, s2, m2, r2, p[c + "output.LayerNorm.weight"], G["crossattention.output.LayerNorm.weight"],
                                            G["crossattention.output.LayerNorm.bias"], dcol=G["crossattention.output.dense.bias"],
                                            want_bf16=True, drop_out=BertLayersFn._drop(meta, i, 3))
                _, wo2T = BANK.linear(p[c + "output.dense.weight"])
                datt2 = K.gemm_nt(ds2b, wo2T)
                dq2 = torch.empty_like(q2)
                dkv = torch.empty_like(kv)
                delta2 = torch.empty_like(lse2)
                kv_done = None

                def attn2(phase, ask_form=False):
                    return K.attn_bwd(K.view3(q2, S, L), K.view3(kv, Bi, T, 0), K.view3(kv, Bi, T, Hd), K.view3(att2, S, L),
                                      K.view3(datt2, S, L), S, Bi, H, L, T, scale, lse2, delta2, K.view3(dq2, S, L), K.view3(dkv, Bi, T, 0),
                                      K.view3(dkv, Bi, T, Hd), mask=meta["enc_mask"], kv_idx=meta["kv_idx"], seq_off=meta["seq_off"],
                                      seq_ids=meta["seq_ids"], drop=BertLayersFn._drop(meta, i, 2), phase=phase, ask_form=ask_form)
                one_pass = attn2(0, ask_form=True) != 0
                aux = AUX.enabled and not (AUX.auto and one_pass)
                attn2(1 if aux and not one_pass else 0)
                _param_only(po, K.colsum_bf16, dq2, G["crossattention.self.query.bias"])
                G.alias("crossattention.self.key.bias", G["c.kv_bias"][:Hd])
                G.alias("crossattention.self.value.bias", G["c.kv_bias"][Hd:])
                G.alias("crossattention.self.key.weight", G["c.kv_weight"][:Hd])
                G.alias("crossattention.self.value.weight", G["c.kv_weight"][Hd:])
                _, wqT = BANK.linear(p[c + "self.query.weight"])
                _, wkvT = BANK.linear(p[c + "self.key.weight"], p[c + "self.value.weight"])
                dh1 = K.gemm_nt(dq2, wqT, resid=ds2, out_dtype=F32)
                if aux:
                    first = denc is None
                    if first:
                        denc = torch.empty(Bi * T, Dv, device=dev, dtype=F32)

                    def kv_side(attn2=attn2, dkv=dkv, wkvT=wkvT, first=first, denc=denc, one_pass=one_pass):
                        if not one_pass:
                            attn2(2)
                        K.gemm_nt(dkv, wkvT, resid=None if first else denc, out=denc)
                    kv_done = AUX.launch(kv_side, [q2, kv, att2, datt2, lse2, delta2, dq2, dkv, wkvT, denc])
                else:
                    denc = K.gemm_nt(dkv, wkvT, resid=denc, out_dtype=F32)
                tn = [(dkv, encb, G["c.kv_weight"])] + tn + [(ds2b, att2, G["crossattention.output.dense.weight"]),
                                                            (dq2, h1b, G["crossattention.self.query.weight"])]
            else:
                dh1 = dh2
            ds1, ds1b = K.layernorm_bwd(dh1, s1, m1, r1, p[a + "output.LayerNorm.weight"], G["attention.output.LayerNorm.weight"],
                                        G["attention.output.LayerNorm.bias"], dcol=G["attention.output.dense.bias"], want_bf16=True,
                                        drop_out=BertLayersFn._drop(meta, i, 1))
            _, woT = BANK.linear(p[a + "output.dense.weight"])
            datt = K.gemm_nt(ds1b, woT)
            dqkv = torch.empty_like(qkv)
            delta = torch.empty_like(lse)
            if meta.get("self_mask2d") is not None:
                K.attn_bwd_mask2d(K.view3(qkv, S, L, 0), K.view3(qkv, S, L, Hd), K.view3(qkv, S, L, 2 * Hd), K.view3(att, S, L),
                                  K.view3(datt, S, L), S, H, L, scale, lse, delta, K.view3(dqkv, S, L, 0), K.view3(dqkv, S, L, Hd),
                                  K.view3(dqkv, S, L, 2 * Hd), meta["self_mask2d"], drop=BertLayersFn._drop(meta, i, 0))
            else:
                K.attn_bwd(K.view3(qkv, S, L, 0), K.view3(qkv, S, L, Hd), K.view3(qkv, S, L, 2 * Hd), K.view3(att, S, L), K.view3(datt, S, L),
                           S, S, H, L, L, scale, lse, delta, K.view3(dqkv, S, L, 0), K.view3(dqkv, S, L, Hd), K.view3(dqkv, S, L, 2 * Hd),
                           mask=meta["self_mask"], drop=BertLayersFn._drop(meta, i, 0))
            _param_only(po, K.colsum_bf16, dqkv, G["a.qkv_bias"])
            for k3, nm in enumerate(("query", "key", "value")):
                G.alias("attention.self.%s.bias" % nm, G["a.qkv_bias"][k3 * Hd:(k3 + 1) * Hd])
                G.alias("attention.self.%s.weight" % nm, G["a.qkv_weight"][k3 * Hd:(k3 + 1) * Hd])
            _, wqkvT = BANK.linear(p[a + "self.query.weight"], p[a + "self.key.weight"], p[a + "self.value.weight"])
            dh = K.gemm_nt(dqkv, wqkvT, resid=ds1, out_dtype=F32)
            tn += [(ds1b, att, G["attention.output.dense.weight"]), (dqkv, hb, G["a.qkv_weight"])]
            if cr is not None:
                if kv_done is not None and WGRAD_QUEUE is None:
                    torch.cuda.current_stream().wait_event(kv_done)
                _param_only(po, K.colsum_bf16, dkv, G["c.kv_bias"])
            pairs.add(G, tn, po)
            for n in names:
                if n.startswith(b):
                    out[n] = G.g[n[len(b):]]
        pairs.flush()
        SIDE.join()
        AUX.join()
        d_enc = denc.view(enc_shape) if denc is not None else None
        return (dh.view(S, L, Hd), d_enc, None) + tuple(out[n] for n in names)



class EmbeddingsFn(torch.autograd.Function):

    @staticmethod
    def forward(ctx, ids, eps, drop, word, pos, typ, lnw, lnb, pids=None):
        S, L = ids.shape
        ids = ids.contiguous()
        if pids is not None:
            pids = pids.to(torch.int64).expand(S, L).contiguous()
            e = K.embed_fwd_pid(ids, pids, word.detach(), pos.detach(), typ.detach())
        else:
            e = K.embed_fwd(ids, word.detach(), pos.detach(), typ.detach())
        _, y, mean, rstd = K.layernorm_fwd(e, lnw, lnb, eps, want_bf16=False, want_f32=True, drop=drop)
        ctx.save_for_backward(ids, e, mean, rstd, word, pos, typ, lnw)
        ctx.drop, ctx.pids = drop, pids
        return y.view(S, L, -1)

    @staticmethod
    def backward(ctx, dy):
        ids, e, mean, rstd, word, pos, typ, lnw = ctx.saved_tensors
        n = lnw.numel()
        zeros = torch.zeros(2 * n + pos.numel() + typ.numel(), device=dy.device, dtype=F32)
        dw, db = zeros[:n], zeros[n:2 * n]
        dpos, dtyp = zeros[2 * n:2 * n + pos.numel()].view_as(pos), zeros[2 * n + pos.numel():].view_as(typ)
        de, _ = K.layernorm_bwd(dy.contiguous().view(e.shape), e, mean, rstd, lnw, dw, db, drop_in=ctx.drop)
        dword = _TIED_DWORD.pop(_tok(word), None)
        if dword is None:
            dword = torch.zeros_like(word)
        if ctx.pids is not None:
            K.embed_bwd_pid(ids, ctx.pids, de, dword, dpos, dtyp)
        else:
            K.embed_bwd(ids, de, dword, dpos, dtyp)
        return None, None, None, dword, dpos, dtyp, dw, db, None



class MlmLossFn(torch.autograd.Function):

    @staticmethod
    def forward(ctx, rows, labels, eps, keep_logits, dw_, db_, lnw, lnb, dec_bias, word, smooth=None):
        R, Hd = rows.shape
        V = word.shape[0]
        rb = K.cast_bf16(rows.contiguous())
        wd, _ = BANK.linear(dw_)
        t_pre = torch.empty(R, Hd, device=rows.device, dtype=BF16)
        t_act = K.gemm_nt(rb, wd, bias=db_, aux=t_pre, act=1, out_dtype=F32)
        tb, _, mean, rstd = K.layernorm_fwd(t_act, lnw, lnb, eps)
        Eb, EbT = BANK.vocab(word)
        Vp = Eb.shape[0]
        bias_p = BANK.vector(dec_bias, Vp - V) if Vp > V else dec_bias.detach()
        labels = labels.contiguous().view(-1)
        ctx.smooth = smooth
        logits = None
        if keep_logits or KEEP_MLM_LOGITS:
            logits = K.gemm_nt(tb, Eb, bias=bias_p, out_dtype=F32)
        if smooth is not None:
            stat, lse = K.mlm_ls_fwd(tb, Eb, bias_p, labels, smooth[0], V, smooth[1], smooth[2])
        else:
            stat, lse = K.mlm_ce_fwd(tb, Eb, bias_p, labels, V)
        ctx.save_for_backward(rb, t_pre, t_act, mean, rstd, tb, bias_p, labels, lse, stat, dw_, lnw, word)
        ctx.V = V
        lse_out = lse.clone()
        ctx.mark_non_differentiable(*([lse_out] + ([logits] if logits is not None else [])))
        return stat[0].clone(), lse_out, logits

    @staticmethod
    def backward(ctx, g, _glse, _gl):
        rb, t_pre, t_act, mean, rstd, tb, bias_p, labels, lse, stat, dw_, lnw, word = ctx.saved_tensors
# ... 153 lines not shown
```

x2-vlm_amd/kernels.py:

```python
import ctypes as C

import torch

from . import _lib
from ._lib import AttnArgs, call, ptr, raw_stream

BF16, F32 = torch.bfloat16, torch.float32


GEMM_TIMER = None


class _timed:

    def __init__(self, flops, name="gemm_nt"):
        self.flops = flops
        self.name = name

    def __enter__(self):
        if GEMM_TIMER is not None:
            self.a = torch.cuda.Event(enable_timing=True)
            self.b = torch.cuda.Event(enable_timing=True)
            self.a.record()

# ... 33 lines not shown
    x = x ^ (x >> 15); x = (x * 0x846ca68b) & 0xFFFFFFFF
    x = x ^ (x >> 16)
    u = torch.where((e & 1) == 1, x >> 16, x & 0xFFFF)
    return (u >= thr).to(torch.float32) * scale


_WS = {}
_WS_RETIRED = []
_WS_CAPTURED = set()


def workspace(device, nfloats):
    key = (device, raw_stream())
    buf = _WS.get(key)
    if buf is None or buf.numel() < nfloats:
        if buf is not None and buf.data_ptr() in _WS_CAPTURED:
            _WS_RETIRED.append(buf)
        buf = torch.empty(max(nfloats, 1 << 22, 0 if buf is None else 2 * buf.numel()), device=device, dtype=F32)
        _WS[key] = buf
    if buf.is_cuda and torch.cuda.is_current_stream_capturing():
        _WS_CAPTURED.add(buf.data_ptr())
    return buf


DEFERRED = None


def _ws_and_defer(device, nfloats):
    if DEFERRED is not None:
        return torch.empty(nfloats, device=device, dtype=F32), 1
    return workspace(device, nfloats), 0


def reduce_partials(ws, nblk, nk, width, outs):
    o = list(outs) + [None] * (3 - len(outs))
    call("x2_reduce_partials", ptr(ws), nblk, nk, width, ptr(o[0]), ptr(o[1]), ptr(o[2]))


def reduce_partials_multi(items):
    flat = []
    for ws, nblk, nk, width, outs in items:
        o = list(outs) + [None] * (4 - len(outs))
        flat += [ws.data_ptr(), nblk, nk, width] + [0 if t is None else t.data_ptr() for t in o]
    call("x2_reduce_partials_multi", (C.c_int64 * len(flat))(*flat), len(items))


def cast_transpose_multi(desc):
    flat = [v for d in desc for v in (tuple(d) + (0,) if len(d) == 7 else d)]
    call("x2_cast_transpose_multi", (C.c_int64 * len(flat))(*flat), len(desc))


def copy_f32_multi(desc):
    flat = [v for d in desc for v in d]
    call("x2_copy_f32_multi", (C.c_int64 * len(flat))(*flat), len(desc))


def _rows(t):
    assert t.dim() == 2 and t.stride(1) == 1, "expected a row-major 2-D tensor (got strides %s)" % (t.stride(),)
    return t.stride(0)


def round_up(x, m):
    return (x + m - 1) // m * m



def gemm_nt(A, B, *, bias=None, gamma=None, resid=None, aux=None, act=0, out=None, out_dtype=BF16, drop=NO_DROP,
            rowscale=None, colsum=None):
    assert A.dtype == BF16 and B.dtype == BF16 and A.shape[1] == B.shape[1]
    M, K = A.shape
    N = B.shape[0]
    if out is None:
        out = torch.empty(M, N, device=A.device, dtype=out_dtype)
    assert out.shape == (M, N) and out.dtype in (BF16, F32)
    for t in (bias, gamma):
        assert t is None or (t.dtype == F32 and t.numel() == N and t.is_contiguous())
    assert resid is None or (resid.dtype == F32 and resid.shape == (M, N))
    assert aux is None or (aux.dtype == BF16 and aux.shape == (M, N))
    assert rowscale is None or (rowscale.dtype == F32 and rowscale.numel() == M and rowscale.is_contiguous())
    with _timed(2.0 * M * N * K):
        call("x2_gemm_nt", ptr(A), ptr(B), ptr(out), M, N, K, _rows(A), _rows(B), _rows(out), ptr(bias), ptr(gamma),
             ptr(resid), _rows(resid) if resid is not None else 0, ptr(aux), _rows(aux) if aux is not None else 0,
             act, 1 if out.dtype == F32 else 0, drop[0], drop[1], drop[2], ptr(drop[3]), ptr(rowscale), ptr(colsum))
    return out


def gemm_nt_dgelu_colsum(A, B, pre, colsum):
    assert A.dtype == BF16 and B.dtype == BF16 and A.shape[1] == B.shape[1] and pre.dtype == BF16
    M, K = A.shape
    N = B.shape[0]
    assert pre.shape == (M, N) and colsum.dtype == F32 and colsum.numel() == N
    out = torch.empty(M, N, device=A.device, dtype=BF16)
    ws, defer = _ws_and_defer(A.device, 2 * ((M + 63) // 64) * N)
    nrows = C.c_int(0)
    with _timed(2.0 * M * N * K):
        call("x2_gemm_nt_dgelu_colparts", ptr(A), ptr(B), ptr(out), M, N, K, _rows(A), _rows(B), _rows(out), ptr(pre), _rows(pre),
             ptr(ws), C.byref(nrows))
    if defer:
        DEFERRED.append((ws, nrows.value, 1, N, (colsum,)))
    else:
        reduce_partials(ws, nrows.value, 1, N, (colsum,))
    return out


def gemm_nt_splitk(A, B, out=None, slices=0):
    assert A.dtype == BF16 and B.dtype == BF16 and A.shape[1] == B.shape[1]
    M, K = A.shape
    N = B.shape[0]
    if out is None:
        out = torch.empty(M, N, device=A.device, dtype=F32)
    assert out.shape == (M, N) and out.dtype == F32
    ws = workspace(A.device, min(32, max(1, K // 64)) * M * N)
    with _timed(2.0 * M * N * K):
        call("x2_gemm_nt_splitk", ptr(A), ptr(B), ptr(out), M, N, K, _rows(A), _rows(B), _rows(out), slices, ptr(ws), ws.numel())
    return out


def gemm_tn_grouped(problems, accumulate=False, split=0):
    rows = []
    for pr in problems:
        dY, X, dW = pr[:3]
        assert dY.dtype == BF16 and X.dtype == BF16 and dW.dtype == F32 and dY.shape[0] == X.shape[0]
        N, K = dW.shape
        n_ld, k_ld = (pr[3], pr[4]) if len(pr) == 5 else (dY.shape[1], X.shape[1])
        assert dY.shape[1] >= N or n_ld >= N
        rows.append([dY.data_ptr(), X.data_ptr(), dW.data_ptr(), dY.shape[0], N, K, _rows(dY), _rows(X), _rows(dW),
                     n_ld, k_ld])
    dev = problems[0][0].device
    for i in range(0, len(rows), 8):
        chunk = rows[i:i + 8]
        arr = (C.c_int64 * (11 * len(chunk)))(*[v for r in chunk for v in r])
        tiles256 = sum(((r[4] + 255) // 256) * ((r[5] + 255) // 256) for r in chunk)
        want = (split if split else 4) * tiles256 * 65536
        ws = workspace(dev, want) if split != 1 else None
        with _timed(sum(2.0 * r[3] * r[4] * r[5] for r in chunk), "gemm_tn"):
            call("x2_gemm_tn_grouped", arr, len(chunk), 1 if accumulate else 0, split, ptr(ws), 0 if ws is None else ws.numel())



def _attn_args(q, k, v, B, Bkv, H, Lq, Lk, scale, bias=None, biasT=None, mask=None, kv_idx=None, seq_off=None,
               seq_ids=None, drop=NO_DROP, head_dim=64, bias_log2=False):
    a = AttnArgs()
    a.Q, a.q_bs, a.q_rs = q
    a.K, a.k_bs, a.k_rs = k
    a.V, a.v_bs, a.v_rs = v
    a.B, a.Bkv, a.H, a.Lq, a.Lk, a.scale = B, Bkv, H, Lq, Lk, scale
    a.head_dim = head_dim
    a.dbg = 16 if bias_log2 else 0
    a.drop_thr16, a.drop_seed, a.drop_scale = drop[:3]
    a.drop_epoch = ptr(drop[3])
    if bias is not None:
        assert bias.dtype == F32 and bias.dim() == 3 and bias.is_contiguous()
        a.bias, a.bias_ld = bias.data_ptr(), bias.shape[2]
    if biasT is not None:
        assert biasT.dtype == F32 and biasT.dim() == 3 and biasT.is_contiguous()
        a.biasT, a.biasT_ld = biasT.data_ptr(), biasT.shape[2]
    if mask is not None:
        assert mask.dtype == F32 and mask.dim() == 2 and mask.is_contiguous() and mask.shape[0] == B
        a.mask, a.mask_ld = mask.data_ptr(), mask.shape[1]
    if kv_idx is not None:
        assert kv_idx.dtype == torch.int32 and kv_idx.numel() == B
        a.kv_idx = kv_idx.data_ptr()
    if seq_off is not None:
        assert seq_off.dtype == torch.int32 and seq_ids.dtype == torch.int32
        a.seq_off, a.seq_ids = seq_off.data_ptr(), seq_ids.data_ptr()
    return a
# ... 41 lines not shown
    if phase == 0 and Lq > 208 and Lk > 208 and a.kv_idx is None and not a.drop_thr16:
        ws = workspace(lse.device, B * H * ((Lq + 127) // 128) * 8192)
        a.ws, a.ws_floats = ws.data_ptr(), ws.numel()
    if ask_form:
        return _lib.lib().x2_attn_bwd_one_pass(C.byref(a))
    if colsum_ws is not None:
        assert colsum_ws.dtype == F32 and colsum_ws.is_contiguous() and colsum_ws.shape == (B, 2, H * 64)
        form = _lib.lib().x2_attn_bwd_one_pass(C.byref(a))
        if form in (1, 3):
            a.colsum_ws = colsum_ws.data_ptr()
        call("x2_attn_bwd", C.byref(a))
        return form
    call("x2_attn_bwd", C.byref(a))


def _check_mask2d(mask2d, B, L):
    assert mask2d.dtype == F32 and mask2d.dim() == 3 and mask2d.is_contiguous() and mask2d.shape[:2] == (B, L)
    assert mask2d.shape[2] % 64 == 0 and mask2d.shape[2] >= L


def attn_fwd_mask2d(q, k, v, B, H, L, scale, out, lse, mask2d, drop=NO_DROP, head_dim=64):
    _check_mask2d(mask2d, B, L)
    a = _attn_args(q, k, v, B, B, H, L, L, scale, drop=drop, head_dim=head_dim)
    a.Out, a.o_bs, a.o_rs = out
    assert lse.dtype == F32 and lse.numel() == B * H * L
    a.LSE = lse.data_ptr()
    call("x2_attn_fwd_mask2d", C.byref(a), mask2d.data_ptr(), mask2d.shape[2])


def attn_bwd_mask2d(q, k, v, o, do, B, H, L, scale, lse, delta, dq, dk, dv, mask2d, drop=NO_DROP, head_dim=64):
    _check_mask2d(mask2d, B, L)
    a = _attn_args(q, k, v, B, B, H, L, L, scale, drop=drop, head_dim=head_dim)
    a.O, a.o_bs, a.o_rs = o
    a.dO, a.do_bs, a.do_rs = do
    a.dQ, a.dq_bs, a.dq_rs = dq
    a.dK, a.dk_bs, a.dk_rs = dk
    a.dV, a.dv_bs, a.dv_rs = dv
    a.LSE, a.Delta = lse.data_ptr(), delta.data_ptr()
    call("x2_attn_bwd_mask2d", C.byref(a), mask2d.data_ptr(), mask2d.shape[2])



def layernorm_fwd(x, w, b, eps, *, rows=None, period=0, want_bf16=True, want_f32=False, y_bf16=None, y_f32=None,
                  drop=NO_DROP):
    assert x.dtype == F32 and x.is_contiguous()
    D = x.shape[-1]
    x2 = x.view(-1, D)
    R = x2.shape[0] if rows is None else rows
    if want_bf16 and y_bf16 is None:
        y_bf16 = torch.empty_like(x2, dtype=BF16)
    if want_f32 and y_f32 is None:
        y_f32 = torch.empty_like(x2)
    mean = torch.empty(R, device=x.device, dtype=F32)
    rstd = torch.empty(R, device=x.device, dtype=F32)
    call("x2_layernorm_fwd", ptr(x2), ptr(w), ptr(b), ptr(y_bf16), ptr(y_f32), ptr(mean), ptr(rstd), R, D, eps, period,
         drop[0], drop[1], drop[2], ptr(drop[3]))
    return y_bf16, y_f32, mean, rstd


def layernorm_bwd(dy, x, mean, rstd, w, dw, db, *, dres=None, dcol=None, period=0, want_f32=True, want_bf16=False, dx=None,
                  drop_in=NO_DROP, drop_out=NO_DROP, post=None):
    assert dy.dtype in (F32, BF16) and x.dtype == F32 and dy.is_contiguous() and x.is_contiguous()
    D = x.shape[-1]
    R = mean.numel()
    if want_f32 and dx is None:
        dx = torch.empty_like(x) if period == 0 else torch.zeros_like(x)
    prs = None
    if post is not None:
        assert dcol is None and dy.dtype == BF16 and period == 0
        prs, dcol = post
        assert prs is None or (prs.dtype == F32 and prs.numel() == R and prs.is_contiguous())
        want_bf16 = True
    dxb = torch.empty(x.shape, device=x.device, dtype=BF16) if want_bf16 else None
    nblk = (R + 15) // 16
    ws, defer = _ws_and_defer(x.device, nblk * 3 * D)
    call("x2_layernorm_bwd", ptr(dy), 1 if dy.dtype == BF16 else 0, ptr(x), ptr(mean), ptr(rstd), ptr(w), ptr(dres), ptr(dx), ptr(dxb), ptr(dw), ptr(db),
         ptr(dcol), R, D, period, drop_in[0], drop_in[1], drop_in[2], drop_out[0], drop_out[1], drop_out[2],
         ptr(drop_in[3] if drop_in[3] is not None else drop_out[3]), ptr(ws), defer, 0 if post is None else 1, ptr(prs))
    if defer:
        DEFERRED.append((ws, nblk, 3, D, (dw, db, dcol)))
    return dx, dxb


def colsum_bf16(y, out):
    nblk = (y.shape[0] + 63) // 64
    ws, defer = _ws_and_defer(y.device, nblk * y.shape[1])
    call("x2_colsum_bf16", ptr(y), ptr(out), y.shape[0], y.shape[1], _rows(y), ptr(ws), defer)
    if defer:
        DEFERRED.append((ws, nblk, 1, y.shape[1], (out,)))


def rowscale_cast_colsum(dx, colsum, rowscale=None):
    assert dx.dtype == F32 and dx.is_contiguous() and dx.dim() == 2
    dxb = torch.empty_like(dx, dtype=BF16)
    nblk = (dx.shape[0] + 31) // 32
    ws, defer = _ws_and_defer(dx.device, nblk * dx.shape[1])
    call("x2_rowscale_cast_colsum", ptr(dx), ptr(rowscale), ptr(dxb), ptr(colsum), dx.shape[0], dx.shape[1], ptr(ws), defer)
    if defer:
        DEFERRED.append((ws, nblk, 1, dx.shape[1], (colsum,)))
    return dxb


def layerscale_finish(items):
    flat = []
    for G, W, bias, gamma, cs, dgamma, dbias in items:
        N, Kd = G.shape
        assert G.dtype == F32 and W.dtype == F32 and G.is_contiguous() and W.is_contiguous() and W.numel() == G.numel() and Kd % 4 == 0
        flat += [G.data_ptr(), W.data_ptr(), 0 if bias is None else bias.data_ptr(), gamma.data_ptr(), cs.data_ptr(), dgamma.data_ptr(),
                 0 if dbias is None else dbias.data_ptr(), N, Kd]
    call("x2_layerscale_finish", (C.c_int64 * len(flat))(*flat), len(items))


def cast_bf16(src, out=None):
    assert src.dtype == F32 and src.is_contiguous() and src.numel() % 4 == 0
    if out is None:
        out = torch.empty_like(src, dtype=BF16)
    call("x2_cast_bf16", ptr(src), ptr(out), src.numel())
    return out


def cast_transpose_bf16(src, want_plain=True, ldt=None):
    assert src.dtype == F32 and src.dim() == 2 and src.is_contiguous()
    R, Cc = src.shape
    ldt = R if ldt is None else ldt
    plain = torch.empty(R, Cc, device=src.device, dtype=BF16) if want_plain else None
    tr = (torch.zeros if ldt > R else torch.empty)(Cc, ldt, device=src.device, dtype=BF16)
    call("x2_cast_transpose_bf16", ptr(src), ptr(plain), ptr(tr), R, Cc, ldt)
    return plain, tr


def patchify(image, ps):
    assert image.dtype == F32 and image.is_contiguous() and image.dim() == 4 and image.shape[1] == 3
    B, _, R, _ = image.shape
    g = R // ps
    cols = torch.empty(B * g * g, 3 * ps * ps, device=image.device, dtype=BF16)
    call("x2_patchify", ptr(image), ptr(cols), B, R, ps)
    return cols


def assemble_tokens(patch, cls, B, P):
    D = patch.shape[1]
    x = torch.empty(B, P + 1, D, device=patch.device, dtype=F32)
    call("x2_assemble_tokens", ptr(patch), ptr(cls), ptr(x), B, P, D)
    return x


def assemble_tokens_bwd(dx, dcls):
    B, T, D = dx.shape
    dpatch = torch.empty(B * (T - 1), D, device=dx.device, dtype=BF16)
    call("x2_assemble_tokens_bwd", ptr(dx), ptr(dpatch), ptr(dcls), B, T - 1, D)
    return dpatch


def pool_tokens(x, w=None, bwd=False):
    B, T, D = x.shape
    assert x.dtype == F32 and x.is_contiguous() and (w is None or (w.dtype == F32 and w.shape == (B, T - 1) and w.is_contiguous()))
    call("x2_pool_tokens", ptr(x), ptr(w), B, T - 1, D, 1 if bwd else 0)
    return x


LOG2E = 1.4426950408889634


def relpos_bias(table, index, want_T=True, log2=False):
    N = index.shape[0]
    H = table.shape[1]
# ... 8 lines not shown
_RELPOS_CSR = {}
_RELPOS_T = {}


def _relpos_index_t(index):
    key = (index.data_ptr(), index._version)
    ent = _RELPOS_T.get(key)
    if ent is None:
        ent = _RELPOS_T[key] = (index.t().contiguous(), index)
    return ent[0]



def _relpos_csr(index, ld, T):
    key = (index.data_ptr(), index._version, ld, T)
    ent = _RELPOS_CSR.get(key)
    if ent is None:
        N = index.shape[0]
        flat = index.reshape(-1)
        order = torch.argsort(flat, stable=True)
        off = torch.zeros(T + 1, device=index.device, dtype=torch.int32)
        off[1:] = torch.cumsum(torch.bincount(flat, minlength=T), 0)
        pos = ((order // N) * ld + order % N).to(torch.int32).contiguous()
        ent = _RELPOS_CSR[key] = (off, pos, index)
    return ent[0], ent[1]


def relpos_bias_bwd(dS, index, dtable):
    B, H, N, ld = dS.shape
    T = dtable.shape[0]
    assert dS.dtype == BF16 and dS.is_contiguous() and dtable.dtype == F32 and dtable.is_contiguous() and dtable.shape[1] == H
    off, pos = _relpos_csr(index, ld, T)
    slices = 1
    ws = workspace(dS.device, slices * H * N * ld)
    call("x2_relpos_bias_bwd", ptr(dS), ptr(off), ptr(pos), ptr(dtable), B, N, H, ld, T, ptr(ws), slices)



def embed_fwd(ids, word, pos, type_emb):
    R, L = ids.numel(), ids.shape[-1]
    D = word.shape[1]
    out = torch.empty(R, D, device=word.device, dtype=F32)
    call("x2_embed_fwd", ptr(ids), ptr(word), ptr(pos), ptr(type_emb), ptr(out), R, L, D)
    return out


def embed_bwd(ids, g, dword, dpos, dtype):
    R, L = ids.numel(), ids.shape[-1]
    D = g.shape[-1]
    scratch = workspace(g.device, min(L, R) * D)
    call("x2_embed_bwd", ptr(ids), ptr(g), ptr(dword), ptr(dpos), ptr(dtype), R, L, D, ptr(scratch))


def embed_fwd_pid(ids, pids, word, pos, type_emb):
    assert ids.dtype == torch.int64 and pids.dtype == torch.int64 and ids.shape == pids.shape and ids.is_contiguous() and pids.is_contiguous()
    R = ids.numel()
    D = word.shape[1]
    out = torch.empty(R, D, device=word.device, dtype=F32)
    call("x2_embed_fwd_pid", ptr(ids), ptr(pids), ptr(word), ptr(pos), ptr(type_emb), ptr(out), R, D)
    return out


def embed_bwd_pid(ids, pids, g, dword, dpos, dtype):
    R, L = ids.numel(), ids.shape[-1]
    D = g.shape[-1]
    assert pids.dtype == torch.int64 and pids.shape == ids.shape and pids.is_contiguous()
    scratch = workspace(g.device, min(L, R) * D)
    call("x2_embed_bwd_pid", ptr(ids), ptr(pids), ptr(g), ptr(dword), ptr(dpos), ptr(dtype), R, L, D, ptr(scratch))


def gather_rows(src, idx, row_len, want_f32=True, want_bf16=False):
    R = idx.numel()
    assert src.dtype == F32 and src.is_contiguous() and idx.dtype == torch.int32
    dst = torch.empty(R, row_len, device=src.device, dtype=F32) if want_f32 else None
    dstb = torch.empty(R, row_len, device=src.device, dtype=BF16) if want_bf16 else None
    call("x2_gather_rows", ptr(src), ptr(idx), ptr(dst), ptr(dstb), R, row_len)
    return dst, dstb


def scatter_rows(src, idx, rows, row_len):
    assert src.dtype == F32 and src.is_contiguous() and idx.dtype == torch.int32 and src.numel() == idx.numel() * row_len
    dst = torch.empty(rows, row_len, device=src.device, dtype=F32)
    call("x2_scatter_rows", ptr(src), ptr(idx), ptr(dst), idx.numel(), rows, row_len)
    return dst


def linear_f32(A, B, *, bias=None, transA=False, transB=False, alpha=1.0, alpha_ptr=None, out=None, accumulate=False):
    assert A.dtype == F32 and B.dtype == F32 and A.dim() == 2 and B.dim() == 2
    M, K = (A.shape[1], A.shape[0]) if transA else A.shape
    N = B.shape[1] if transB else B.shape[0]
    sam, sak = (A.stride(1), A.stride(0)) if transA else (A.stride(0), A.stride(1))
    sbn, sbk = (B.stride(1), B.stride(0)) if transB else (B.stride(0), B.stride(1))
    tiles = ((M + 63) // 64) * ((N + 63) // 64)
    ksplit = 1 if tiles >= 64 or K < 128 else max(1, min(16, K // 64, 256 // tiles))
    if out is None:
        assert not accumulate
        out = torch.empty(M, N, device=A.device, dtype=F32)
    ws = workspace(A.device, ksplit * M * N) if ksplit > 1 else None
    call("x2_linear_f32", ptr(A), ptr(B), ptr(out), ptr(bias), ptr(alpha_ptr), alpha, M, N, K, sam, sak, sbn, sbk,
         out.stride(0), 1 if accumulate else 0, ksplit, ptr(ws))
    return out


def l2norm(x, dy=None):
    out = torch.empty_like(x)
    call("x2_l2norm", ptr(x), ptr(dy), ptr(out), x.shape[0], x.shape[1], 0 if dy is None else 1)
    return out


def ce_fwd(logits, labels, C_valid=None):
    R, ld = logits.shape
    Cv = ld if C_valid is None else C_valid
    lse = torch.empty(R, device=logits.device, dtype=F32)
    rows = torch.empty(R, device=logits.device, dtype=F32)
    stat = torch.empty(2, device=logits.device, dtype=F32)
    call("x2_ce_fwd", ptr(logits), ld, ptr(labels), R, Cv, ptr(lse), ptr(rows), ptr(stat))
    return stat, lse


def ce_bwd(logits, labels, lse, g, stat, C_valid=None, gscale=1.0, out_dtype=F32):
    R, ld = logits.shape
    Cv = ld if C_valid is None else C_valid
    dl = torch.empty(R, ld, device=logits.device, dtype=out_dtype)
    call("x2_ce_bwd", ptr(logits), ld, ptr(labels), ptr(lse), ptr(g), ptr(stat), gscale, R, Cv,
         ptr(dl) if out_dtype == F32 else None, ptr(dl) if out_dtype == BF16 else None, ld)
    return dl


def mlm_ce_fwd(x, E, bias, labels, V):
    assert x.dtype == BF16 and E.dtype == BF16 and x.shape[1] == E.shape[1] and bias.dtype == F32 and bias.numel() == E.shape[0]
    assert labels.dtype == torch.int64 and labels.numel() == x.shape[0]
    R, Hd = x.shape
    Vp = E.shape[0]
    dev = x.device
    part = torch.empty(R, Vp // 64, 2, device=dev, dtype=F32)
    small = torch.empty(3 * R + 2, device=dev, dtype=F32)
    zlab, lse, rows, stat = small[:R], small[R:2 * R], small[2 * R:3 * R], small[3 * R:]
    with _timed(2.0 * R * Vp * Hd):
        call("x2_mlm_ce_fwd", ptr(x), ptr(E), ptr(bias), ptr(labels), R, Vp, V, Hd, _rows(x), _rows(E), ptr(part), ptr(zlab))
    call("x2_ce_combine", ptr(part), Vp // 64, ptr(zlab), ptr(labels), R, ptr(lse), ptr(rows), ptr(stat))
    return stat, lse


def mlm_ce_bwd(x, E, bias, labels, lse, g, stat, V, gscale=1.0):
    R, Hd = x.shape
    Vp = E.shape[0]
    dl = torch.empty(R, Vp, device=x.device, dtype=BF16)
    with _timed(2.0 * R * Vp * Hd, "gemm_nt_recompute"):
        call("x2_mlm_ce_bwd", ptr(x), ptr(E), ptr(bias), ptr(labels), ptr(lse), ptr(g), ptr(stat), gscale, R, Vp, V, Hd,
             _rows(x), _rows(E), ptr(dl), Vp)
    return dl


def mlm_ls_fwd(x, E, bias, labels, weights, V, ignore, ls):
    assert x.dtype == BF16 and E.dtype == BF16 and x.shape[1] == E.shape[1] and bias.dtype == F32 and bias.numel() == E.shape[0]
    assert labels.dtype == torch.int64 and labels.numel() == x.shape[0] and weights.dtype == F32 and weights.numel() == x.shape[0]
    R, Hd = x.shape
    Vp = E.shape[0]
    dev = x.device
    part = torch.empty(R, Vp // 64, 2, device=dev, dtype=F32)
    sumz = torch.empty(R, Vp // 64, device=dev, dtype=F32)
    small = torch.empty(4 * R + 2, device=dev, dtype=F32)
    zlab, zign, lse, rows, stat = small[:R], small[R:2 * R], small[2 * R:3 * R], small[3 * R:4 * R], small[4 * R:]
    with _timed(2.0 * R * Vp * Hd):
        call("x2_mlm_ls_fwd", ptr(x), ptr(E), ptr(bias), ptr(labels), int(ignore), R, Vp, V, Hd, _rows(x), _rows(E), ptr(part), ptr(sumz),
             ptr(zlab), ptr(zign))
# ... 178 lines not shown
```

x2-vlm_amd/model_pretrain.py:

```python
import torch

from . import kernels as K
from . import ops
from .xvlm import XVLMBase


class XVLM(XVLMBase):
    def __init__(self, config, load_vision_params=True, load_text_params=True, pretraining=True):
        super().__init__(config, load_vision_params=load_vision_params, load_text_params=load_text_params,
                         use_contrastive_loss=True, use_matching_loss=True, use_mlm_loss=True, use_bbox_loss=True,
                         config_text=None, pretraining=pretraining)
        self.overlap_towers = True
        self._text_stream = None

    def tower_text(self, text_ids, text_atts, text_ids_masked):
        return self.get_text_embeds(torch.cat([text_ids, text_ids_masked]), torch.cat([text_atts, text_atts]))

    def tower_vision(self, image, image_atts=None, idx_to_group_img=None, ret_bbox_loss=False):
        if ret_bbox_loss:
            return self.get_vision_embeds(image, image_atts=image_atts, idx_to_group_img=idx_to_group_img)
        return self.get_vision_embeds(image) + (None,)

    def tail_features(self, image_embeds, both):
        return self.get_features(image_embeds, both[:image_embeds.shape[0]])

    def tail_losses(self, image_embeds, image_atts, both, image_feat, text_feat, text_atts, masked_pos, masked_ids,
                    image_embeds_fullatts=None, target_bbox=None, is_image=None, ret_bbox_loss=False, ret_match_loss=True,
                    gathered=None):
        B = image_embeds.shape[0]
        dev = both.device
        text_embeds = both[:B]
        loss_itc = self.get_contrastive_loss(image_feat, text_feat, gathered=gathered)
        ineg, tneg = self.get_hard_negatives(image_feat, text_feat) if ret_match_loss else (None, None)
        if both.is_cuda:
            t_idx, kv, atts, enc_atts = K.tail_index(ineg, tneg, text_atts.contiguous(), image_atts.contiguous(), with_match=ret_match_loss)
        else:
            ar = torch.arange(B, device=dev, dtype=torch.int32)
            t_idx, kv = (torch.cat([ar, ar, tneg, ar + B]), torch.cat([ar, ineg, ar, ar])) if ret_match_loss else (ar + B, ar)
            atts, enc_atts = torch.cat([text_atts, text_atts])[t_idx.long()], image_atts[kv.long()]
        h0 = ops.gather_rows(both, t_idx)
        fused = self.get_cross_embeds(image_embeds, enc_atts, text_embeds=h0, text_atts=atts, kv_idx=kv)
        if ret_match_loss:
            loss_itm = self._itm_loss(fused[:3 * B, 0, :], B)
        else:
            loss_itm = torch.tensor(0.0)
        loss_mlm, self.last_mlm_lse, self.last_mlm_logits = self.text_encoder.mlm_loss_from_hidden(fused[-B:], masked_pos, masked_ids)
        loss = {"loss_itc": loss_itc, "loss_itm": loss_itm, "loss_mlm": loss_mlm}
        self.last = dict(image_embeds=image_embeds.detach(), text_embeds=text_embeds.detach(), image_feat=image_feat.detach(),
                         text_feat=text_feat.detach())
        if ret_bbox_loss:
            output_coord = self.predict_bbox(image_embeds_fullatts, text_embeds, text_atts)
            self.last["bbox_coord"] = output_coord.detach()
            loss["loss_bbox"], loss["loss_giou"] = self.get_bbox_loss(output_coord, target_bbox, is_image=is_image)
        return loss

    def forward_multimodal(self, image, text_ids, text_atts, text_ids_masked=None, masked_pos=None, masked_ids=None,
                           image_atts=None, idx_to_group_img=None, target_bbox=None, is_image=None,
                           ret_bbox_loss=False, ret_match_loss=True):
        overlap = self.overlap_towers and image.is_cuda
        if overlap:
            if self._text_stream is None:
                self._text_stream = torch.cuda.Stream()
            main = torch.cuda.current_stream()
            self._text_stream.wait_stream(main)
            with torch.cuda.stream(self._text_stream):
                both = self.tower_text(text_ids, text_atts, text_ids_masked)
        image_embeds, image_atts, image_embeds_fullatts = self.tower_vision(image, image_atts, idx_to_group_img, ret_bbox_loss)
        if overlap:
            main.wait_stream(self._text_stream)
            both.record_stream(main)
        else:
            both = self.tower_text(text_ids, text_atts, text_ids_masked)
        image_feat, text_feat = self.tail_features(image_embeds, both)
        return self.tail_losses(image_embeds, image_atts, both, image_feat, text_feat, text_atts, masked_pos, masked_ids,
                                image_embeds_fullatts=image_embeds_fullatts, target_bbox=target_bbox, is_image=is_image,
                                ret_bbox_loss=ret_bbox_loss, ret_match_loss=ret_match_loss)

    def forward_text(self, text_ids=None, text_atts=None, text_ids_masked=None, masked_pos=None, masked_ids=None):
        seq = self._bert(text_ids_masked, attention_mask=text_atts, mode="multi_modal").last_hidden_state
        loss, self.last_mlm_lse, self.last_mlm_logits = self.text_encoder.mlm_loss_from_hidden(seq, masked_pos, masked_ids)
        self.last = dict(text_embeds=seq.detach())
        return {"loss_mlm": loss}

    def forward(self, image=None, text_ids=None, text_atts=None, text_ids_masked=None, masked_pos=None, masked_ids=None,
                image_atts=None, idx_to_group_img=None, target_bbox=None, is_image=None, ret_bbox_loss=False,
                ret_match_loss=True):
        if image is None:
            return self.forward_text(text_ids, text_atts, text_ids_masked, masked_pos, masked_ids)
        return self.forward_multimodal(image, text_ids, text_atts, text_ids_masked, masked_pos, masked_ids, image_atts,
                                       idx_to_group_img, target_bbox, is_image, ret_bbox_loss, ret_match_loss=ret_match_loss)
```

x2-vlm_amd/xbert.py:

```python
import json
import os
from types import SimpleNamespace

import torch
import torch.nn as nn

from . import kernels as K
from . import ops
from .engine import BertLayersFn, EmbeddingsFn, MlmLossFn, _mask_pad, bert_layer_param_names


_FIXED_SEEDS = []


def _key_mask(atts, neg):
    if atts.is_cuda and atts.dtype == torch.int64:
        return K.additive_mask(atts.contiguous(), neg)
    return _mask_pad((1.0 - atts.float()) * neg, atts.shape[1])


def _text_masks(atts):
    if atts.dim() == 3:
        return None, K.additive_mask2d(atts.to(torch.int64).contiguous(), -10000.0)
    return _key_mask(atts, -10000.0), None
# ... 19 lines not shown
    def from_json_file(cls, path):
        with open(path) as f:
            return cls(**json.load(f))


class BertEmbeddings(nn.Module):
    def __init__(self, config):
        super().__init__()
        self.word_embeddings = nn.Embedding(config.vocab_size, config.hidden_size, padding_idx=config.pad_token_id)
        self.position_embeddings = nn.Embedding(config.max_position_embeddings, config.hidden_size)
        self.token_type_embeddings = nn.Embedding(config.type_vocab_size, config.hidden_size)
        self.LayerNorm = nn.LayerNorm(config.hidden_size, eps=config.layer_norm_eps)
        self.register_buffer("position_ids", torch.arange(config.max_position_embeddings).expand((1, -1)))
        self.eps = config.layer_norm_eps
        self.config = config

    def forward(self, input_ids, position_ids=None):
        drop = K.NO_DROP
        if self.training and self.config.hidden_dropout_prob > 0:
            drop = K.dropout_spec(self.config.hidden_dropout_prob, next_dropout_seed(), 1000)
        args = (input_ids, self.eps, drop, self.word_embeddings.weight, self.position_embeddings.weight,
                self.token_type_embeddings.weight, self.LayerNorm.weight, self.LayerNorm.bias)
        if position_ids is None:
            return EmbeddingsFn.apply(*args)
        return EmbeddingsFn.apply(*args, position_ids)


class BertSelfAttention(nn.Module):
    def __init__(self, config, is_cross_attention):
        super().__init__()
        kin = config.encoder_width if is_cross_attention else config.hidden_size
        self.query = nn.Linear(config.hidden_size, config.hidden_size)
        self.key = nn.Linear(kin, config.hidden_size)
        self.value = nn.Linear(kin, config.hidden_size)


class BertSelfOutput(nn.Module):
    def __init__(self, config):
        super().__init__()
        self.dense = nn.Linear(config.hidden_size, config.hidden_size)
        self.LayerNorm = nn.LayerNorm(config.hidden_size, eps=config.layer_norm_eps)


class BertAttention(nn.Module):
    def __init__(self, config, is_cross_attention=False):
        super().__init__()
        self.self = BertSelfAttention(config, is_cross_attention)
        self.output = BertSelfOutput(config)


class BertIntermediate(nn.Module):
    def __init__(self, config):
        super().__init__()
        self.dense = nn.Linear(config.hidden_size, config.intermediate_size)


class BertOutput(nn.Module):
    def __init__(self, config):
        super().__init__()
        self.dense = nn.Linear(config.intermediate_size, config.hidden_size)
        self.LayerNorm = nn.LayerNorm(config.hidden_size, eps=config.layer_norm_eps)


class BertLayer(nn.Module):
    def __init__(self, config, layer_num):
        super().__init__()
        self.attention = BertAttention(config)
        self.has_cross_attention = layer_num >= config.fusion_layer
        if self.has_cross_attention:
            self.crossattention = BertAttention(config, is_cross_attention=True)
        self.intermediate = BertIntermediate(config)
        self.output = BertOutput(config)


_IDENTITY_CSR = {}


class BertEncoder(nn.Module):
    def __init__(self, config):
        super().__init__()
        self.config = config
        self.layer = nn.ModuleList([BertLayer(config, i) for i in range(config.num_hidden_layers)])

    def run(self, hidden, text_atts, enc=None, enc_atts=None, mode="multi_modal", kv_idx=None):
        cfg = self.config
        lo, hi = {"text": (0, cfg.fusion_layer), "fusion": (cfg.fusion_layer, cfg.num_hidden_layers),
                  "multi_modal": (0, cfg.num_hidden_layers)}[mode]
        S, L, _ = hidden.shape
        drop = None
        if self.training and (cfg.hidden_dropout_prob > 0 or cfg.attention_probs_dropout_prob > 0):
            drop = dict(seed=next_dropout_seed(), p_hidden=cfg.hidden_dropout_prob, p_attn=cfg.attention_probs_dropout_prob)
        meta = dict(lo=lo, hi=hi, fusion_at=cfg.fusion_layer, heads=cfg.num_attention_heads, eps=cfg.layer_norm_eps,
                    self_mask=None, self_mask2d=None, enc_mask=None, kv_idx=None,
                    seq_off=None, seq_ids=None, drop=drop)
        meta["self_mask"], meta["self_mask2d"] = _text_masks(text_atts)
        cross = enc is not None and hi > cfg.fusion_layer
        if cross:
            Bi = enc.shape[0]
            meta["enc_mask"] = _key_mask(enc_atts, -1e9)
            if kv_idx is None:
                assert Bi == S, "encoder batch %d != text batch %d and no kv_idx given" % (Bi, S)
                if enc.is_cuda and torch.is_grad_enabled() and (hidden.requires_grad or enc.requires_grad or self.training) \
                        and K.attn_bwd_form(L, enc.shape[1], shared_kv=True) == 2:
                    ident = _IDENTITY_CSR.get((S, enc.device))
                    if ident is None:
                        ar = torch.arange(S + 1, device=enc.device, dtype=torch.int32)
                        ident = (ar[:S].contiguous(), ar, ar[:S].contiguous())
                        if not torch.cuda.is_current_stream_capturing():
                            _IDENTITY_CSR[(S, enc.device)] = ident
                    meta.update(kv_idx=ident[0], seq_off=ident[1], seq_ids=ident[2])
            else:
                kv = kv_idx.to(torch.int32).contiguous()
                if kv.is_cuda:
                    off, order = K.kv_csr(kv, Bi)
                else:
                    order = torch.argsort(kv, stable=True).to(torch.int32).contiguous()
                    off = torch.zeros(Bi + 1, device=kv.device, dtype=torch.int32)
                    off[1:] = torch.cumsum(torch.bincount(kv, minlength=Bi), 0)
                meta.update(kv_idx=kv, seq_off=off, seq_ids=order)
        cache = self.__dict__.setdefault("_param_lists", {})
        params = cache.get((lo, hi, cross))
        if params is None:
            sd = dict(self.named_parameters())
            params = cache[(lo, hi, cross)] = [sd[n] for n in bert_layer_param_names(lo, hi, cfg.fusion_layer, cross)]
        return BertLayersFn.apply(hidden, enc if cross else None, meta, *params)


class BertModel(nn.Module):
    def __init__(self, config, add_pooling_layer=False):
        super().__init__()
        assert not add_pooling_layer
        self.config = config
        self.embeddings = BertEmbeddings(config)
        self.encoder = BertEncoder(config)
        self.apply(lambda m: _bert_init(m, config.initializer_range))

    def get_input_embeddings(self):
        return self.embeddings.word_embeddings

    def forward(self, input_ids=None, attention_mask=None, encoder_embeds=None, encoder_hidden_states=None,
                encoder_attention_mask=None, return_dict=True, mode="multi_modal", kv_idx=None, position_ids=None, **unused):
        _refuse_unused("BertModel", unused)
        hidden = self.embeddings(input_ids, position_ids) if encoder_embeds is None else encoder_embeds
        S, L = hidden.shape[:2]
        if attention_mask is None:
            attention_mask = torch.ones(S, L, device=hidden.device)
        if encoder_hidden_states is not None and encoder_attention_mask is None:
            encoder_attention_mask = torch.ones(S, encoder_hidden_states.shape[1], device=hidden.device)
        out = self.encoder.run(hidden, attention_mask, encoder_hidden_states, encoder_attention_mask, mode, kv_idx)
        return SimpleNamespace(last_hidden_state=out) if return_dict else (out,)


class BertPredictionHeadTransform(nn.Module):
    def __init__(self, config):
        super().__init__()
        self.dense = nn.Linear(config.hidden_size, config.hidden_size)
        self.LayerNorm = nn.LayerNorm(config.hidden_size, eps=config.layer_norm_eps)


class BertLMPredictionHead(nn.Module):
    def __init__(self, config):
        super().__init__()
        self.transform = BertPredictionHeadTransform(config)
        self.decoder = nn.Linear(config.hidden_size, config.vocab_size, bias=False)
        self.bias = nn.Parameter(torch.zeros(config.vocab_size))


class BertOnlyMLMHead(nn.Module):
    def __init__(self, config):
        super().__init__()
        self.predictions = BertLMPredictionHead(config)


class BertForMaskedLM(nn.Module):

    def __init__(self, config):
        super().__init__()
        self.config = config
        self.bert = BertModel(config)
        self.cls = BertOnlyMLMHead(config)
        self.apply(lambda m: _bert_init(m, config.initializer_range))
        self.cls.predictions.decoder.weight = self.bert.embeddings.word_embeddings.weight

    def mlm_loss_from_hidden(self, sequence_output, masked_pos, labels, keep_logits=False):
        B, L, Hd = sequence_output.shape
        flat = (torch.arange(B, device=masked_pos.device).unsqueeze(1) * L + masked_pos).reshape(-1)
        rows = ops.gather_rows(sequence_output.reshape(B * L, Hd), flat)
        pr = self.cls.predictions
        return MlmLossFn.apply(rows, labels, self.config.layer_norm_eps, keep_logits, pr.transform.dense.weight, pr.transform.dense.bias,
                               pr.transform.LayerNorm.weight, pr.transform.LayerNorm.bias, pr.bias,
                               self.bert.embeddings.word_embeddings.weight)

    def smoothed_mlm_loss_from_hidden(self, sequence_output, masked_pos, labels, weights, ignore_index, label_smoothing, keep_logits=False):
        B, L, Hd = sequence_output.shape
        flat = (torch.arange(B, device=masked_pos.device).unsqueeze(1) * L + masked_pos).reshape(-1)
        rows = ops.gather_rows(sequence_output.reshape(B * L, Hd), flat)
        pr = self.cls.predictions
        w = weights.reshape(-1).to(torch.float32).contiguous()
        return MlmLossFn.apply(rows, labels, self.config.layer_norm_eps, keep_logits, pr.transform.dense.weight, pr.transform.dense.bias,
                               pr.transform.LayerNorm.weight, pr.transform.LayerNorm.bias, pr.bias,
                               self.bert.embeddings.word_embeddings.weight, (w, int(ignore_index), float(label_smoothing)))

    def forward(self, input_ids=None, attention_mask=None, encoder_hidden_states=None, encoder_attention_mask=None,
                labels=None, return_dict=True, mode="multi_modal", masked_pos=None, return_logits=False, position_ids=None, **unused):
        _refuse_unused("BertForMaskedLM", unused)
        if masked_pos is None:
            raise NotImplementedError("need check!")
        h = self.bert(input_ids, attention_mask=attention_mask, encoder_hidden_states=encoder_hidden_states,
                      encoder_attention_mask=encoder_attention_mask, mode=mode, position_ids=position_ids).last_hidden_state
        lab = labels if labels is not None else torch.full_like(masked_pos, -100)
        loss, _, logits = self.mlm_loss_from_hidden(h, masked_pos, lab, keep_logits=return_logits)
        if logits is not None:
            logits = logits[:, :self.config.vocab_size].view(masked_pos.shape[0], masked_pos.shape[1], -1)
        if return_logits:
            return logits
        return SimpleNamespace(loss=loss if labels is not None else None, logits=logits)


def _refuse_unused(who, unused):
    for k, v in unused.items():
        if v not in (None, False):
            raise NotImplementedError("%s.forward(%s=...) is not supported by the HIP path" % (who, k))


def _bert_init(m, std):
    if isinstance(m, (nn.Linear, nn.Embedding)):
        m.weight.data.normal_(mean=0.0, std=std)
    elif isinstance(m, nn.LayerNorm):
        m.bias.data.zero_()
        m.weight.data.fill_(1.0)
    if isinstance(m, nn.Linear) and m.bias is not None:
        m.bias.data.zero_()


def get_bert_config(encoder_rpath, num_hidden_layers=12, cross_start_at=12):
    config = BertConfig.from_json_file(os.path.join(encoder_rpath, "config.json"))
    config.num_hidden_layers = num_hidden_layers
    config.fusion_layer = cross_start_at
    config.embedding_dim = config.hidden_size
    return config
```

x2-vlm_amd/xvlm.py:

```python
import os

import torch
import torch.distributed as dist
import torch.nn as nn

from . import box_ops, checkpoint, ops
from . import kernels as K
from .beit2 import beit_base_patch16, beit_large_patch16, read_json, trunc_normal_
from .xbert import BertForMaskedLM, BertModel, get_bert_config


class AllGather(torch.autograd.Function):

    @staticmethod
    def forward(ctx, tensor, rank, world_size):
        out = [torch.empty_like(tensor) for _ in range(world_size)]
        dist.all_gather(out, tensor.contiguous())
        ctx.rank, ctx.batch_size = rank, tensor.shape[0]
        return torch.cat(out, 0)

    @staticmethod
    def backward(ctx, grad_output):
        return grad_output[ctx.batch_size * ctx.rank: ctx.batch_size * (ctx.rank + 1)], None, None

# ... 71 lines not shown
            self.update_init_params(["text_proj." + n for n, _ in self.text_proj.named_parameters()])
            if config.get("fix_temp", False):
                self.temp = torch.ones([]) * config["temp"]
            else:
                self.temp = nn.Parameter(torch.ones([]) * config["temp"])
                self.update_init_params(["temp"])
        self.use_matching_loss = use_matching_loss
        if use_matching_loss:
            self.itm_head = build_mlp(self.text_width, 2)
            self.update_init_params(["itm_head." + n for n, _ in self.itm_head.named_parameters()])
        self.use_bbox_loss = use_bbox_loss
        if use_bbox_loss:
            self.bbox_head = build_mlp(self.text_width, 4)
            self.update_init_params(["bbox_head." + n for n, _ in self.bbox_head.named_parameters()])
        if not pretraining:
            self.init_params = []
        self.injected_negatives = None

    def update_init_params(self, missing_keys=None):
        for k in missing_keys or []:
            if k not in self.init_params:
                self.init_params.append(k)
        named = set(n for n, _ in self.named_parameters())
        self.init_params = [n for n in self.init_params if n in named]

    def load_pretrained(self, ckpt_rpath, config, is_eval=False, is_domain_pretrain=False):
        if is_domain_pretrain:
            state = checkpoint._model_state(ckpt_rpath)
            if config.get("init_timesformer", False):
                checkpoint.init_timesformer_keys(state)
        else:
            state = checkpoint.load_pretrained(self, ckpt_rpath, config, is_eval=is_eval, load_text=True)
        own = getattr(self, "absolute_frame_pos_embed", None)
        given = state.get("absolute_frame_pos_embed")
        if own is not None and given is not None and given.shape != own.shape:
            n = min(given.shape[1], own.shape[1])
            with torch.no_grad():
                own[:, :n] = given[:, :n]
            del state["absolute_frame_pos_embed"]
            print("frame position embedding: %d of %d checkpoint frames used" % (n, given.shape[1]), flush=True)
        result = self.load_state_dict(state, strict=False)
        self.update_init_params(list(result.missing_keys))
        print("checkpoint %s: %d unexpected keys; trained from scratch: %s"
              % (ckpt_rpath, len(result.unexpected_keys), sorted(self.init_params)), flush=True)
        return result

    @property
    def _bert(self):
        return self.text_encoder.bert if hasattr(self.text_encoder, "bert") else self.text_encoder

    def get_frame_embeds(self, frame, **unused):
        assert frame.dim() == 5
        B, Fr = frame.shape[:2]
        e = self.vision_encoder(frame.reshape(B * Fr, *frame.shape[2:]))
        pos = self.absolute_frame_pos_embed if self.add_frame_pos else torch.zeros(1, Fr, 1, e.shape[-1], device=e.device)
        e = ops.frame_mean(e, pos, Fr)
        return e, torch.ones(e.shape[:2], dtype=torch.long, device=e.device)

    def get_image_embeds(self, image, image_atts=None, idx_to_group_img=None, **unused):
        assert image.dim() == 4
        if idx_to_group_img is None:
            e = self.vision_encoder(image)
            return e, torch.ones(e.shape[:2], dtype=torch.long, device=image.device)
        if image_atts is None:
            full = ops.gather_rows(self.vision_encoder(image), idx_to_group_img)
            return full, torch.ones(full.shape[:2], dtype=torch.long, device=image.device)
        assert image_atts.size(0) == idx_to_group_img.size(0)
        e, full = self.vision_encoder(image, idx_to_group_img=idx_to_group_img, image_atts=image_atts)
        return e, image_atts, ops.gather_rows(full, idx_to_group_img)

    def get_vision_embeds(self, image, image_atts=None, idx_to_group_img=None, output_hidden_states=None, output_attentions=None):
        assert output_hidden_states == output_attentions
        if image.dim() == 5:
            assert idx_to_group_img is None, "not supported"
            return self.get_frame_embeds(image)
        return self.get_image_embeds(image, image_atts=image_atts, idx_to_group_img=idx_to_group_img)

    def get_text_embeds(self, text_ids, text_atts, **unused):
        return self._bert(text_ids, attention_mask=text_atts, mode="text").last_hidden_state

    def get_text_embeds_12L(self, text_ids, text_atts, **unused):
        return self._bert(text_ids, attention_mask=text_atts).last_hidden_state

    def get_cross_embeds(self, image_embeds, image_atts, text_ids=None, text_embeds=None, text_atts=None, kv_idx=None, **unused):
        assert text_atts is not None
        if text_embeds is not None:
            return self._bert(encoder_embeds=text_embeds, attention_mask=text_atts, encoder_hidden_states=image_embeds,
                              encoder_attention_mask=image_atts, mode="fusion", kv_idx=kv_idx).last_hidden_state
        if text_ids is not None:
            return self._bert(text_ids, attention_mask=text_atts, encoder_hidden_states=image_embeds,
                              encoder_attention_mask=image_atts, kv_idx=kv_idx).last_hidden_state
        raise ValueError

    def get_features(self, image_embeds=None, text_embeds=None):
        fi = ft = None
        if image_embeds is not None:
            fi = ops.normalize(ops.linear(image_embeds[:, 0, :], self.vision_proj.weight, self.vision_proj.bias))
        if text_embeds is not None:
            ft = ops.normalize(ops.linear(text_embeds[:, 0, :], self.text_proj.weight, self.text_proj.bias))
        if image_embeds is None:
            return ft
        if text_embeds is None:
            return fi
        return fi, ft

    def _sim(self, a, b):
        return ops.linear(a, b) / self.temp

    def get_contrastive_loss(self, image_feat, text_feat, idx=None, gathered=None):
        assert image_feat.size(-1) == self.embed_dim and text_feat.size(-1) == self.embed_dim
        fi, ft = gathered if gathered is not None else (allgather(image_feat), allgather(text_feat))
        logits = self._sim(fi, ft)
        n = logits.shape[0]
        if idx is None:
            labels = torch.arange(n, device=logits.device)
            return (ops.cross_entropy(logits, labels) + ops.cross_entropy(logits.t(), labels)) / 2
        idx = idx.view(-1, 1)
        idx_all = allgather(idx)
        pos = torch.eq(idx_all, idx_all.t()).float()
        lab = pos / pos.sum(1, keepdim=True)
        li = -torch.sum(torch.log_softmax(logits, dim=1) * lab, dim=1).mean()
        lt = -torch.sum(torch.log_softmax(logits.t(), dim=1) * lab, dim=1).mean()
        return (li + lt) / 2

    def get_hard_negatives(self, image_feat, text_feat, idx=None):
        if self.injected_negatives is not None:
            return tuple(torch.as_tensor(n, dtype=torch.int32, device=image_feat.device) for n in self.injected_negatives)
        with torch.no_grad():
            fi, ft = image_feat.detach(), text_feat.detach()
            temp = self.temp.detach().reshape(1).float()
            bs = fi.shape[0]
            sim_i2t = K.linear_f32(fi, ft, alpha_ptr=None) / temp
            sim_t2i = K.linear_f32(ft, fi, alpha_ptr=None) / temp
            u = torch.rand(2, bs, device=fi.device)
            grp = idx.view(-1).long().contiguous() if idx is not None else None
            if grp is not None and bool((grp.view(-1, 1) == grp.view(1, -1)).all(1).any()):
                raise RuntimeError("get_hard_negatives: a row has no candidate with a different idx (invalid multinomial distribution)")
            return K.sample_negatives(sim_t2i, u[0].contiguous(), grp), K.sample_negatives(sim_i2t, u[1].contiguous(), grp)

    def get_matching_loss(self, image_embeds, image_atts, image_feat, text_embeds, text_atts, text_feat, idx=None):
        ineg, tneg = self.get_hard_negatives(image_feat, text_feat, idx=idx)
        B = image_embeds.shape[0]
        ar = torch.arange(B, device=image_embeds.device, dtype=torch.int32)
        t_idx = torch.cat([ar, ar, tneg])
        kv = torch.cat([ar, ineg, ar])
        cls = self._fusion_cls(image_embeds, image_atts, text_embeds, text_atts, t_idx, kv)
        return self._itm_loss(cls, B)

    def _fusion_cls(self, image_embeds, image_atts, text_embeds, text_atts, t_idx, kv):
        h0 = ops.gather_rows(text_embeds, t_idx)
        out = self.get_cross_embeds(image_embeds, image_atts[kv.long()], text_embeds=h0, text_atts=text_atts[t_idx.long()], kv_idx=kv)
        return out[:, 0, :]

    def _itm_loss(self, cls, B):
        logits = ops.mlp_head(self.itm_head, cls)
        cache = self.__dict__.setdefault("_itm_labels", {})
        labels = cache.get((B, cls.device))
        if labels is None:
            labels = torch.zeros(3 * B, dtype=torch.long, device=cls.device)
            labels[:B] = 1
            cache[(B, cls.device)] = labels
        self.last_itm_logits = logits.detach()
        return ops.cross_entropy(logits, labels)

    def get_mlm_loss(self, text_ids_masked, text_atts, image_embeds, image_atts, masked_pos, masked_ids):
        return self.text_encoder(text_ids_masked, attention_mask=text_atts, encoder_hidden_states=image_embeds,
                                 encoder_attention_mask=image_atts, labels=masked_ids, masked_pos=masked_pos).loss

    def predict_bbox(self, image_embeds, text_embeds, text_atts):
        assert image_embeds.size(0) == text_embeds.size(0)
        ones = torch.ones(image_embeds.shape[:2], device=image_embeds.device)
        cls = self.get_cross_embeds(image_embeds, ones, text_embeds=text_embeds, text_atts=text_atts)[:, 0, :]
        return ops.mlp_head(self.bbox_head, cls).sigmoid()

    def get_bbox_loss(self, output_coord, target_bbox, is_image=None):
        loss_bbox = (output_coord - target_bbox).abs()
        b1, b2 = box_ops.box_cxcywh_to_xyxy(output_coord), box_ops.box_cxcywh_to_xyxy(target_bbox)
        degenerate = ((b1[:, 2:] < b1[:, :2]).any() | (b2[:, 2:] < b2[:, :2]).any())
        unit = torch.cat([torch.zeros_like(b1[:, :2]), torch.ones_like(b1[:, 2:])], dim=-1)
        giou = 1 - box_ops.generalized_box_iou_pairs(torch.where(degenerate, unit, b1), torch.where(degenerate, unit, b2))
        loss_giou = torch.where(degenerate, torch.zeros_like(giou), giou)
        if is_image is None:
            num_boxes = target_bbox.size(0)
        else:
            keep = (1 - is_image).to(loss_bbox.dtype)
            num_boxes = keep.sum()
            loss_bbox = loss_bbox * keep.view(-1, 1)
            loss_giou = loss_giou * keep
        return loss_bbox.sum() / num_boxes, loss_giou.sum() / num_boxes
```

Baseline: 2910.

## Compute last fusion layer only for rows consumed by ITM and MLM heads

Adds a row-selective path through the final cross-encoder layer so only the CLS rows (for ITM/bbox) and masked-token rows (for MLM) are carried through the output projection, FFN and LayerNorm. New kernels build the row table, gather and scatter rows, and a GEMM/LayerNorm-backward variant keys dropout on the original row index so the masks stay consistent. This removes the work spent on the many final-layer outputs that no loss reads, at the cost of extra gather/scatter launches and a more complex backward path.

```diff
diff --git a/include/x2vlm_hip.h b/include/x2vlm_hip.h
--- a/include/x2vlm_hip.h
+++ b/include/x2vlm_hip.h
@@ -15,6 +15,9 @@
                const float* bias, const float* gamma, const float* resid, int ldr, void* aux, int ldaux,
                int act, int out_f32, unsigned drop_thr16, unsigned drop_seed, float drop_scale, const unsigned* drop_epoch,
                const float* rowscale, float* colsum, void* stream);
+int x2_gemm_nt_rows(const void* A, const void* B, void* C, int M, int N, int K, int lda, int ldb, int ldc,
+                    const float* bias, const float* resid, int ldr, int out_f32, unsigned drop_thr16, unsigned drop_seed,
+                    float drop_scale, const unsigned* drop_epoch, float* colsum, const int* drop_rows , void* stream);
 
 int x2_gemm_nt_dgelu_colparts(const void* A, const void* B, void* C, int M, int N, int K, int lda, int ldb, int ldc,
                               const void* aux, int ldaux, float* colparts, int* nrows_out, void* stream);
@@ -59,6 +62,10 @@
                      int period, unsigned in_thr16, unsigned in_seed, float in_scale, unsigned out_thr16,
                      unsigned out_seed, float out_scale, const unsigned* drop_epoch, float* ws ,
                      int defer, int post, const float* post_rowscale, void* stream);
+int x2_layernorm_bwd_rows(const float* dy, const float* x, const float* mean, const float* rstd, const float* w, float* dx,
+                          void* dx_bf16, float* dw, float* db, float* dcol, int rows, int D, unsigned out_thr16,
+                          unsigned out_seed, float out_scale, const unsigned* drop_epoch, const int* drop_rows ,
+                          float* ws , int defer, void* stream);
 int x2_colsum_bf16(const void* y, float* out, int M, int N, int ld, float* ws , int defer, void* stream);
 int x2_reduce_partials(const float* part, int nblk, int nk, int width, float* o0, float* o1, float* o2, void* stream);
 int x2_reduce_partials_multi(const int64_t* desc, int count, void* stream);
@@ -124,6 +131,11 @@
 int x2_kv_csr(const int* kv, int S, int Bi, int* off, int* order, void* stream);
 int x2_tail_index(const int* ineg, const int* tneg, const long* text_atts , const long* image_atts , int B, int L,
                   int T, int with_match, int* t_idx, int* kv, long* atts_out , long* enc_out , void* stream);
+int x2_fusion_rows(const long* masked_pos , int B, int n, int S, int L, int n_cls, int* rows ,
+                   int* slot , void* stream);
+int x2_gather_rows_z(const void* src, const int* rows, void* dst, int R, int D, long row_bytes, void* stream);
+int x2_scatter_rows_zero(const void* src, const int* rows, void* dst, int R, int D, long row_bytes, void* stream);
+int x2_add_rows(const float* src, const int* rows, float* dst, int R, int D, long len, void* stream);
 int x2_droppath_rows(const float* rates, unsigned seed, const unsigned* epoch, int depth, int B, int T, float* out, void* stream);
 int x2_frame_mean(const float* x, const float* pos, const float* dy, float* out, float* dpos, int Bc, int F, int T, int D, int bwd,
                   void* stream);
diff --git a/x2-vlm_amd/_lib.py b/x2-vlm_amd/_lib.py
--- a/x2-vlm_amd/_lib.py
+++ b/x2-vlm_amd/_lib.py
@@ -78,6 +78,12 @@
     "x2_attn_decode": [P, I, P, P, I, I, I, I, I, I, F, P],
     "x2_beam_gather": [P, P, P, I, I, I, I, I, P],
     "x2_logprob_topk": [P, I, I, I, P, I, I, I, I, I, I, P, P, P, P],
+    "x2_gemm_nt_rows": [P, P, P, I, I, I, I, I, I, P, P, I, I, U, U, F, P, P, P, P],
+    "x2_layernorm_bwd_rows": [P, P, P, P, P, P, P, P, P, P, I, I, U, U, F, P, P, P, I, P],
+    "x2_fusion_rows": [P, I, I, I, I, I, P, P, P],
+    "x2_gather_rows_z": [P, P, P, I, I, L, P],
+    "x2_scatter_rows_zero": [P, P, P, I, I, L, P],
+    "x2_add_rows": [P, P, P, I, I, L, P],
 }
 _COMM_SIGS = {
     "x2_comm_unique_id": [P],
diff --git a/x2-vlm_amd/csrc/gemm.hip b/x2-vlm_amd/csrc/gemm.hip
--- a/x2-vlm_amd/csrc/gemm.hip
+++ b/x2-vlm_amd/csrc/gemm.hip
@@ -35,6 +35,7 @@
   long ce_ignore;
   float ce_ls;
   const float* ce_w;
+  const int* drop_rows;
 };
 
 __device__ __forceinline__ void tile_coords(int t, int tiles_m, int tiles_n, int gm, int& tm, int& tn) {
@@ -88,13 +89,14 @@
           f32x4{acc[half][tj][4 * g], acc[half][tj][4 * g + 1], acc[half][tj][4 * g + 2], acc[half][tj][4 * g + 3]};
 }
 template <int V> struct EpiTraits {
-  static constexpr bool generic = V == 4;
+  static constexpr bool generic = V == 4 || V == 14;
   static constexpr int act = V == 2 ? 1 : (V == 3 || V == 10) ? 2 : 0;
-  static constexpr bool out_f32 = V == 1 || V == 5 || V == 6 || V == 7;
-  static constexpr bool resid = V == 5 || V == 6;
+  static constexpr bool out_f32 = V == 1 || V == 5 || V == 6 || V == 7 || V == 13;
+  static constexpr bool resid = V == 5 || V == 6 || V == 13;
   static constexpr bool scale = V == 6;
   static constexpr bool aux0 = false;
-  static constexpr bool drop = V == 5;
+  static constexpr bool drop = V == 5 || V == 13;
+  static constexpr bool rows = V == 13 || V == 14;
   static constexpr bool colsum = false;
   static constexpr bool colparts = V == 10;
 };
@@ -227,9 +229,11 @@
       }
       if (has_drop) {
         float dm[4];
-        drop_mul4(drop_, (uint32_t)m * (uint32_t)p.N + (uint32_t)n, dm);
+        uint32_t dr_ = (uint32_t)m;
+        if constexpr (E::rows) dr_ = (uint32_t)max(p.drop_rows[m], 0);
+        drop_mul4(drop_, dr_ * (uint32_t)p.N + (uint32_t)n, dm);
         v[0] *= dm[0]; v[1] *= dm[1]; v[2] *= dm[2]; v[3] *= dm[3];
-        drop_mul4(drop_, (uint32_t)m * (uint32_t)p.N + (uint32_t)n + 4u, dm);
+        drop_mul4(drop_, dr_ * (uint32_t)p.N + (uint32_t)n + 4u, dm);
         v[4] *= dm[0]; v[5] *= dm[1]; v[6] *= dm[2]; v[7] *= dm[3];
       }
       if (has_scale) {
@@ -277,7 +281,7 @@
 template <int TM, int VAR, class Acc>
 __device__ __forceinline__ void nt_epilogue_f4(const GemmNT& p, Acc& acc, char* smem, int wave, int lane, int mw0, int nw0) {
   using E = EpiTraits<VAR>;
-  static_assert(!E::generic && E::out_f32 && E::act == 0 && VAR <= 6, "nt_epilogue_f4: feature sets 1, 5, 6");
+  static_assert(!E::generic && E::out_f32 && E::act == 0 && (VAR <= 6 || VAR == 13), "nt_epilogue_f4: feature sets 1, 5, 6, 13");
   const bool has_drop = E::drop ? p.drop.thr16 != 0 : false;
   float* stg = reinterpret_cast<float*>(smem) + wave * (32 * 68);
   const int er = lane >> 4, ec = (lane & 15) * 4;
@@ -316,7 +320,9 @@
         float v[4] = {a0.x + bb[0], a0.y + bb[1], a0.z + bb[2], a0.w + bb[3]};
         if (has_drop) {
           float dm[4];
-          drop_mul4(drop_, (uint32_t)m * (uint32_t)p.N + (uint32_t)n, dm);
+          uint32_t dr_ = (uint32_t)m;
+          if constexpr (E::rows) dr_ = (uint32_t)max(p.drop_rows[m], 0);
+          drop_mul4(drop_, dr_ * (uint32_t)p.N + (uint32_t)n, dm);
           v[0] *= dm[0]; v[1] *= dm[1]; v[2] *= dm[2]; v[3] *= dm[3];
         }
         if (E::scale) {
@@ -1102,6 +1108,29 @@
   return x2_check_launch("x2_gemm_nt");
 }
 
+extern "C" int x2_gemm_nt_rows(const void* A, const void* B, void* C, int M, int N, int K, int lda, int ldb, int ldc,
+                               const float* bias, const float* resid, int ldr, int out_f32, unsigned drop_thr16, unsigned drop_seed,
+                               float drop_scale, const unsigned* drop_epoch, float* colsum, const int* drop_rows, void* stream) {
+  X2_REQUIRE(A && B && C && drop_rows, "x2_gemm_nt_rows: null argument");
+  X2_REQUIRE(M > 0 && N > 0 && K > 0, "x2_gemm_nt_rows: empty problem M=%d N=%d K=%d", M, N, K);
+  X2_REQUIRE(drop_thr16 < 65536u, "x2_gemm_nt_rows: drop_thr16=%u", drop_thr16);
+  X2_REQUIRE(K % BK == 0, "x2_gemm_nt_rows: K=%d must be a multiple of %d", K, BK);
+  X2_REQUIRE(N % 8 == 0, "x2_gemm_nt_rows: N=%d must be a multiple of 8", N);
+  X2_REQUIRE(lda % 8 == 0 && ldb % 8 == 0 && ldc % 8 == 0, "x2_gemm_nt_rows: leading dims must keep 16-byte rows");
+  X2_REQUIRE(!resid || ldr % 4 == 0, "x2_gemm_nt_rows: ldr alignment");
+  GemmNT p{(const bf16_t*)A, (const bf16_t*)B, C, bias, nullptr, resid, nullptr, M, N, K, lda, ldb, ldc, ldr, 0, 0, out_f32,
+           g_tune[0] > 0 ? g_tune[0] : 8, DropSpec{drop_thr16, drop_seed, drop_scale}, drop_epoch, nullptr, colsum, 0, 0};
+  p.drop_rows = drop_rows;
+  const int tiles_n = (N + BN - 1) / BN, t128 = ((M + 127) / 128) * tiles_n, t64 = ((M + 63) / 64) * tiles_n;
+  const bool use64 = t128 <= 2 * x2_cus();
+  if (resid && out_f32 && !colsum) {
+    if (use64) launch_nt<2, 13, true>(p, t64, (hipStream_t)stream); else launch_nt<4, 13, true>(p, t128, (hipStream_t)stream);
+  } else {
+    if (use64) launch_nt<2, 14, false>(p, t64, (hipStream_t)stream); else launch_nt<4, 14, false>(p, t128, (hipStream_t)stream);
+  }
+  return x2_check_launch("x2_gemm_nt_rows");
+}
+
 extern "C" int x2_gemm_nt_dgelu_colparts(const void* A, const void* B, void* C, int M, int N, int K, int lda, int ldb, int ldc,
                                          const void* aux, int ldaux, float* colparts, int* nrows_out, void* stream) {
   X2_REQUIRE(A && B && C && aux && colparts && nrows_out, "x2_gemm_nt_dgelu_colparts: null argument");
diff --git a/x2-vlm_amd/csrc/heads.hip b/x2-vlm_amd/csrc/heads.hip
--- a/x2-vlm_amd/csrc/heads.hip
+++ b/x2-vlm_amd/csrc/heads.hip
@@ -475,6 +475,81 @@
   return x2_check_launch("x2_tail_index");
 }
 
+__global__ __launch_bounds__(256) void fusion_rows_kernel(const long* __restrict__ masked_pos, int B, int n, int S, int L, int n_cls,
+                                                          int* __restrict__ rows, int* __restrict__ slot) {
+  const int i = blockIdx.x * 256 + threadIdx.x;
+  if (i >= n_cls + B * n) return;
+  if (i < n_cls) { rows[i] = i * L; slot[i] = i; return; }
+  const int b = (i - n_cls) / n, j = (i - n_cls) % n, s = S - B + b;
+  const long pos = masked_pos[(long)b * n + j];
+  int owner = i;
+  if (pos == 0 && s < n_cls) owner = s;
+  else
+    for (int k = 0; k < j; ++k)
+      if (masked_pos[(long)b * n + k] == pos) { owner = n_cls + b * n + k; break; }
+  rows[i] = owner == i ? s * L + (int)pos : -1;
+  slot[i] = owner;
+}
+extern "C" int x2_fusion_rows(const long* masked_pos, int B, int n, int S, int L, int n_cls, int* rows, int* slot, void* stream) {
+  X2_REQUIRE(rows && slot && S > 0 && L > 0 && B >= 0 && B <= S && n_cls >= 0 && n_cls <= S && (B == 0 || (masked_pos && n > 0)) && n_cls + (long)B * n > 0 &&
+             (long)S * L <= 2147483647L, "x2_fusion_rows: B=%d n=%d S=%d L=%d n_cls=%d", B, n, S, L, n_cls);
+  const int R = n_cls + B * n;
+  hipLaunchKernelGGL(fusion_rows_kernel, dim3((R + 255) / 256), dim3(256), 0, (hipStream_t)stream, masked_pos, B, n, S, L, n_cls, rows, slot);
+  return x2_check_launch("x2_fusion_rows");
+}
+
+__global__ __launch_bounds__(256) void gather_rows_z_kernel(const u32x4* __restrict__ src, const int* __restrict__ rows, u32x4* __restrict__ dst,
+                                                            int D, long chunks) {
+  const long r = blockIdx.y;
+  const int d = rows[r];
+  const bool ok = d >= 0 && d < D;
+  for (long e = blockIdx.x * 256L + threadIdx.x; e < chunks; e += (long)gridDim.x * 256)
+    dst[r * chunks + e] = ok ? src[(long)d * chunks + e] : u32x4{0u, 0u, 0u, 0u};
+}
+__global__ __launch_bounds__(256) void zero_rows_kernel(u32x4* __restrict__ dst, long chunks_total) {
+  for (long e = blockIdx.x * 256L + threadIdx.x; e < chunks_total; e += (long)gridDim.x * 256) dst[e] = u32x4{0u, 0u, 0u, 0u};
+}
+__global__ __launch_bounds__(256) void scatter_rows_u_kernel(const u32x4* __restrict__ src, const int* __restrict__ rows, u32x4* __restrict__ dst,
+                                                             int D, long chunks) {
+  const long r = blockIdx.y;
+  const int d = rows[r];
+  if (d < 0 || d >= D) return;
+  for (long e = blockIdx.x * 256L + threadIdx.x; e < chunks; e += (long)gridDim.x * 256) dst[(long)d * chunks + e] = src[r * chunks + e];
+}
+__global__ __launch_bounds__(256) void add_rows_kernel(const float4* __restrict__ src, const int* __restrict__ rows, float4* __restrict__ dst,
+                                                       int D, long chunks) {
+  const long r = blockIdx.y;
+  const int d = rows[r];
+  if (d < 0 || d >= D) return;
+  for (long e = blockIdx.x * 256L + threadIdx.x; e < chunks; e += (long)gridDim.x * 256) {
+    const float4 a = src[r * chunks + e];
+    float4 o = dst[(long)d * chunks + e];
+    o.x += a.x; o.y += a.y; o.z += a.z; o.w += a.w;
+    dst[(long)d * chunks + e] = o;
+  }
+}
+static int rows_grid_x(long chunks) { return (int)((chunks + 255) / 256 < 64 ? (chunks + 255) / 256 : 64); }
+extern "C" int x2_gather_rows_z(const void* src, const int* rows, void* dst, int R, int D, long row_bytes, void* stream) {
+  X2_REQUIRE(src && rows && dst && R > 0 && R <= 65535 && D > 0 && row_bytes > 0 && row_bytes % 16 == 0, "x2_gather_rows_z: R=%d D=%d row_bytes=%ld", R, D, row_bytes);
+  const long chunks = row_bytes / 16;
+  hipLaunchKernelGGL(gather_rows_z_kernel, dim3(rows_grid_x(chunks), R), dim3(256), 0, (hipStream_t)stream, (const u32x4*)src, rows, (u32x4*)dst, D, chunks);
+  return x2_check_launch("x2_gather_rows_z");
+}
+extern "C" int x2_scatter_rows_zero(const void* src, const int* rows, void* dst, int R, int D, long row_bytes, void* stream) {
+  X2_REQUIRE(src && rows && dst && R > 0 && R <= 65535 && D > 0 && row_bytes > 0 && row_bytes % 16 == 0, "x2_scatter_rows_zero: R=%d D=%d row_bytes=%ld", R, D, row_bytes);
+  const long chunks = row_bytes / 16;
+  const long total = chunks * D, zb = (total + 255) / 256;
+  hipLaunchKernelGGL(zero_rows_kernel, dim3((unsigned)(zb < 4096 ? zb : 4096)), dim3(256), 0, (hipStream_t)stream, (u32x4*)dst, total);
+  hipLaunchKernelGGL(scatter_rows_u_kernel, dim3(rows_grid_x(chunks), R), dim3(256), 0, (hipStream_t)stream, (const u32x4*)src, rows, (u32x4*)dst, D, chunks);
+  return x2_check_launch("x2_scatter_rows_zero");
+}
+extern "C" int x2_add_rows(const float* src, const int* rows, float* dst, int R, int D, long len, void* stream) {
+  X2_REQUIRE(src && rows && dst && R > 0 && R <= 65535 && D > 0 && len > 0 && len % 4 == 0, "x2_add_rows: R=%d D=%d len=%ld", R, D, len);
+  const long chunks = len / 4;
+  hipLaunchKernelGGL(add_rows_kernel, dim3(rows_grid_x(chunks), R), dim3(256), 0, (hipStream_t)stream, (const float4*)src, rows, (float4*)dst, D, chunks);
+  return x2_check_launch("x2_add_rows");
+}
+
 __global__ __launch_bounds__(256) void droppath_rows_kernel(const float* __restrict__ rates, uint32_t seed, const uint32_t* __restrict__ epoch,
                                                             int depth, int B, int T, float* __restrict__ out) {
   const long e = blockIdx.x * 256L + threadIdx.x, rows = (long)B * T;
diff --git a/x2-vlm_amd/csrc/rowwise.hip b/x2-vlm_amd/csrc/rowwise.hip
--- a/x2-vlm_amd/csrc/rowwise.hip
+++ b/x2-vlm_amd/csrc/rowwise.hip
@@ -228,9 +228,9 @@
                                                             const float* __restrict__ w, const float* dres, float* dx, bf16_t* dxb,
                                                             float* ws, int rows, int D, int period,
                                                             DropSpec din_, DropSpec dout_, const uint32_t* __restrict__ epoch,
-                                                            const float* __restrict__ post_rs) {
+                                                            const float* __restrict__ post_rs, const int* __restrict__ drop_rows) {
   constexpr int NSET = 3;
-  constexpr bool DYB = MODE != 0;
+  constexpr bool DYB = MODE == 1 || MODE == 2;
   extern __shared__ __attribute__((aligned(16))) float red[];
   const DropSpec din = drop_at_epoch(din_, epoch), dout = drop_at_epoch(dout_, epoch);
   const int lane = threadIdx.x & 63, wv = threadIdx.x >> 6;
@@ -246,6 +246,8 @@
   for (int row = r0 + wv; row < r1; row += 4) {
     const long gr = remap_row(row, period);
     const float mu = mean[row], rs = rstd[row];
+    uint32_t orow = (uint32_t)gr;
+    if constexpr (MODE == 3) orow = (uint32_t)max(drop_rows[row], 0);
     float4 g[NV], xh[NV];
     float s1 = 0.f, s2 = 0.f;
 #pragma unroll
@@ -282,7 +284,7 @@
         float4 om = o;
         if (dout.thr16) {
           float dm[4];
-          drop_mul4(dout, (uint32_t)gr * (uint32_t)D + (uint32_t)(c * 4), dm);
+          drop_mul4(dout, orow * (uint32_t)D + (uint32_t)(c * 4), dm);
           om.x *= dm[0]; om.y *= dm[1]; om.z *= dm[2]; om.w *= dm[3];
         }
         if (dres) { const float4 rr = *reinterpret_cast<const float4*>(dres + gr * D + c * 4); o.x += rr.x; o.y += rr.y; o.z += rr.z; o.w += rr.w; }
@@ -340,11 +342,26 @@
              "x2_layernorm_bwd: post = 1 (by-products of the final output) takes a bf16 dy, dx_bf16 and dcol, no output mask, period 0");
 #define X2_LNB_T(NV, B) hipLaunchKernelGGL((layernorm_bwd_kernel<NV, B>), dim3((rows + LNB_ROWS - 1) / LNB_ROWS), dim3(256), 9 * D * sizeof(float), \
                      (hipStream_t)stream, dy, x, mean, rstd, w, dres, dx, (bf16_t*)dx_bf16, ws, rows, D, period,                \
-                     DropSpec{in_thr16, in_seed, in_scale}, DropSpec{out_thr16, out_seed, out_scale}, drop_epoch, post_rowscale)
+                     DropSpec{in_thr16, in_seed, in_scale}, DropSpec{out_thr16, out_seed, out_scale}, drop_epoch, post_rowscale, drop_rows)
 #define X2_LNB(NV) do { if (post) X2_LNB_T(NV, 2); else if (dy_is_bf16) X2_LNB_T(NV, 1); else X2_LNB_T(NV, 0); } while (0)
+  const int* drop_rows = nullptr;
   LN_DISPATCH(D, X2_LNB);
   if (!defer) launch_reduce(ws, (rows + LNB_ROWS - 1) / LNB_ROWS, 3, D, dw, db, dcol, (hipStream_t)stream);
   return x2_check_launch("x2_layernorm_bwd");
+}
+extern "C" int x2_layernorm_bwd_rows(const float* dy, const float* x, const float* mean, const float* rstd, const float* w, float* dx,
+                                     void* dx_bf16, float* dw, float* db, float* dcol, int rows, int D, unsigned out_thr16,
+                                     unsigned out_seed, float out_scale, const unsigned* drop_epoch, const int* drop_rows, float* ws,
+                                     int defer, void* stream) {
+  X2_REQUIRE(rows > 0 && D > 0 && D % 4 == 0 && D <= 256 * LN_MAXV, "x2_layernorm_bwd_rows: rows=%d D=%d", rows, D);
+  X2_REQUIRE(dy && x && mean && rstd && w && dw && db && ws && drop_rows, "x2_layernorm_bwd_rows: null argument (ws[ceil(rows/%d)*3*D])", LNB_ROWS);
+  const float* dres = nullptr; const float* post_rowscale = nullptr;
+  const int period = 0; const unsigned in_thr16 = 0, in_seed = 0; const float in_scale = 1.f;
+#define X2_LNBR(NV) X2_LNB_T(NV, 3)
+  LN_DISPATCH(D, X2_LNBR);
+#undef X2_LNBR
+  if (!defer) launch_reduce(ws, (rows + LNB_ROWS - 1) / LNB_ROWS, 3, D, dw, db, dcol, (hipStream_t)stream);
+  return x2_check_launch("x2_layernorm_bwd_rows");
 }
 
 #define CS_ROWS 64
diff --git a/x2-vlm_amd/engine.py b/x2-vlm_amd/engine.py
--- a/x2-vlm_amd/engine.py
+++ b/x2-vlm_amd/engine.py
@@ -599,6 +599,18 @@
 class BertLayersFn(torch.autograd.Function):
 
     @staticmethod
+    def _out_linear(A, W, bias, resid, drop, rows):
+        if rows is not None and drop[0] != 0:
+            return K.gemm_nt_rows(A, W, rows, bias=bias, resid=resid, out_dtype=F32, drop=drop)
+        return K.gemm_nt(A, W, bias=bias, resid=resid, out_dtype=F32, drop=drop)
+
+    @staticmethod
+    def _ln_bwd_out(dy, s, m, r, w, gw, gb, dcol, drop, rows):
+        if rows is not None and drop[0] != 0:
+            return K.layernorm_bwd_rows(dy, s, m, r, w, gw, gb, rows, dcol=dcol, drop_out=drop)
+        return K.layernorm_bwd(dy, s, m, r, w, gw, gb, dcol=dcol, want_bf16=True, drop_out=drop)
+
+    @staticmethod
     def prepare_weights(p, lo, hi, fusion_at, cross):
         groups, vecs = [], []
         for i in range(lo, hi):
@@ -641,6 +653,8 @@
         BertLayersFn.prepare_weights(p, meta["lo"], meta["hi"], meta["fusion_at"], cross)
         saved = []
         kv_ahead = {}
+        out_rows = meta.get("out_rows")
+        assert out_rows is None or (out_rows.dtype == torch.int32 and out_rows.dim() == 1 and out_rows.is_contiguous() and meta["hi"] > meta["lo"])
         use_aux = cross and AUX.enabled and not (AUX.auto and K.attn_bwd_form(L, enc.shape[1], shared_kv=meta.get("seq_off") is not None,
                                                                                dropout=BertLayersFn._drop(meta, meta["hi"] - 1, 2)[0] != 0) == 2)
         if use_aux:
@@ -666,7 +680,12 @@
                 K.attn_fwd(K.view3(qkv, S, L, 0), K.view3(qkv, S, L, Hd), K.view3(qkv, S, L, 2 * Hd), S, S, H, L, L, scale,
                            K.view3(att, S, L), lse, mask=meta["self_mask"], drop=dr(meta, i, 0))
             wo, _ = BANK.linear(p[a + "output.dense.weight"])
-            s1 = K.gemm_nt(att, wo, bias=p[a + "output.dense.bias"], resid=h, out_dtype=F32, drop=dr(meta, i, 1))
+            rows = out_rows if i == meta["hi"] - 1 else None
+            cmp = None
+            att_r = att
+            if rows is not None:
+                att_r, h = K.gather_rows_z(att, rows), K.gather_rows_z(h, rows)
+            s1 = BertLayersFn._out_linear(att_r, wo, p[a + "output.dense.bias"], h, dr(meta, i, 1), rows)
             h1b, h1, m1, r1 = K.layernorm_fwd(s1, p[a + "output.LayerNorm.weight"], p[a + "output.LayerNorm.bias"], eps, want_f32=True)
             cr = None
             h2b, h2 = h1b, h1
@@ -676,6 +695,8 @@
                 wkv, _ = BANK.linear(p[c + "self.key.weight"], p[c + "self.value.weight"])
                 bkv = BANK.vector(p[c + "self.key.bias"], p[c + "self.value.bias"])
                 q2 = K.gemm_nt(h1b, wq, bias=p[c + "self.query.bias"])
+                if rows is not None:
+                    q2 = K.scatter_rows_zero(q2, rows, M)
                 if i in kv_ahead:
                     kv, ev = kv_ahead.pop(i)
                     if ev is not None:
@@ -688,23 +709,26 @@
                            K.view3(att2, S, L), lse2, mask=meta["enc_mask"], kv_idx=meta["kv_idx"], seq_off=meta.get("seq_off"),
                            seq_ids=meta.get("seq_ids"), drop=dr(meta, i, 2))
                 wo2, _ = BANK.linear(p[c + "output.dense.weight"])
-                s2 = K.gemm_nt(att2, wo2, bias=p[c + "output.dense.bias"], resid=h1, out_dtype=F32, drop=dr(meta, i, 3))
+                att2_r = K.gather_rows_z(att2, rows) if rows is not None else att2
+                s2 = BertLayersFn._out_linear(att2_r, wo2, p[c + "output.dense.bias"], h1, dr(meta, i, 3), rows)
                 h2b, h2, m2, r2 = K.layernorm_fwd(s2, p[c + "output.LayerNorm.weight"], p[c + "output.LayerNorm.bias"], eps, want_f32=True)
-                cr = (q2, kv, att2, lse2, s2, m2, r2)
+                cr = (q2, kv, att2, lse2, s2, m2, r2, att2_r)
             wi, _ = BANK.linear(p[b + "intermediate.dense.weight"])
             wout, _ = BANK.linear(p[b + "output.dense.weight"])
-            pre = torch.empty(M, wi.shape[0], device=dev, dtype=BF16)
+            pre = torch.empty(h2b.shape[0], wi.shape[0], device=dev, dtype=BF16)
             act = K.gemm_nt(h2b, wi, bias=p[b + "intermediate.dense.bias"], aux=pre, act=1)
-            s3 = K.gemm_nt(act, wout, bias=p[b + "output.dense.bias"], resid=h2, out_dtype=F32, drop=dr(meta, i, 4))
+            s3 = BertLayersFn._out_linear(act, wout, p[b + "output.dense.bias"], h2, dr(meta, i, 4), rows)
             h3b, h3, m3, r3 = K.layernorm_fwd(s3, p[b + "output.LayerNorm.weight"], p[b + "output.LayerNorm.bias"], eps, want_f32=True)
-            saved.append((hb, qkv, att, lse, s1, m1, r1, h1b, cr, h2b, pre, act, s3, m3, r3))
+            if rows is not None:
+                cmp = (rows, att_r)
+            saved.append((hb, qkv, att, lse, s1, m1, r1, h1b, cr, h2b, pre, act, s3, m3, r3, cmp))
             h, hb = h3, h3b
         AUX.join()
         for i in range(meta["lo"], meta["hi"]):
             _count_call(("bert", id(p["layer.%d.attention.self.query.weight" % i])))
         ctx.meta, ctx.saved, ctx.params, ctx.encb = meta, saved, params, encb
         ctx.dims = (S, L, Hd, H, M, scale, cross, enc.shape if cross else None)
-        return h.view(S, L, Hd)
+        return h if out_rows is not None else h.view(S, L, Hd)
 
     @staticmethod
     def backward(ctx, dh_out):
@@ -714,7 +738,7 @@
         names = bert_layer_param_names(meta["lo"], meta["hi"], meta["fusion_at"], cross)
         p = dict(zip(names, params))
         dev = dh_out.device
-        dh = dh_out.contiguous().view(M, Hd)
+        dh = dh_out.contiguous().view(-1, Hd)
         denc = None
         out = {}
         if cross:
@@ -741,15 +765,15 @@
         for li, i in reversed(list(enumerate(range(meta["lo"], meta["hi"])))):
             b = "layer.%d." % i
             a = b + "attention."
-            hb, qkv, att, lse, s1, m1, r1, h1b, cr, h2b, pre, act, s3, m3, r3 = ctx.saved[li]
+            hb, qkv, att, lse, s1, m1, r1, h1b, cr, h2b, pre, act, s3, m3, r3, cmp = ctx.saved[li]
             ctx.saved[li] = None
+            rows, att_r = cmp if cmp is not None else (None, att)
             Ff = p[b + "intermediate.dense.weight"].shape[0]
             G = arenas.pop(i)
             tn, po = [], []
             _begin_layer_backward()
-            ds3, ds3b = K.layernorm_bwd(dh, s3, m3, r3, p[b + "output.LayerNorm.weight"], G["output.LayerNorm.weight"],
-                                        G["output.LayerNorm.bias"], dcol=G["output.dense.bias"], want_bf16=True,
-                                        drop_out=BertLayersFn._drop(meta, i, 4))
+            ds3, ds3b = BertLayersFn._ln_bwd_out(dh, s3, m3, r3, p[b + "output.LayerNorm.weight"], G["output.LayerNorm.weight"],
+                                                 G["output.LayerNorm.bias"], G["output.dense.bias"], BertLayersFn._drop(meta, i, 4), rows)
             _, woutT = BANK.linear(p[b + "output.dense.weight"])
             _, wiT = BANK.linear(p[b + "intermediate.dense.weight"])
             dpre = K.gemm_nt_dgelu_colsum(ds3b, woutT, pre, G["intermediate.dense.bias"])
@@ -757,12 +781,14 @@
             tn += [(ds3b, act, G["output.dense.weight"]), (dpre, h2b, G["intermediate.dense.weight"])]
             if cr is not None:
                 c = b + "crossattention."
-                q2, kv, att2, lse2, s2, m2, r2 = cr
-                ds2, ds2b = K.layernorm_bwd(dh2, s2, m2, r2, p[c + "output.LayerNorm.weight"], G["crossattention.output.LayerNorm.weight"],
-                                            G["crossattention.output.LayerNorm.bias"], dcol=G["crossattention.output.dense.bias"],
-                                            want_bf16=True, drop_out=BertLayersFn._drop(meta, i, 3))
+                q2, kv, att2, lse2, s2, m2, r2, att2_r = cr
+                ds2, ds2b = BertLayersFn._ln_bwd_out(dh2, s2, m2, r2, p[c + "output.LayerNorm.weight"], G["crossattention.output.LayerNorm.weight"],
+                                                     G["crossattention.output.LayerNorm.bias"], G["crossattention.output.dense.bias"],
+                                                     BertLayersFn._drop(meta, i, 3), rows)
                 _, wo2T = BANK.linear(p[c + "output.dense.weight"])
                 datt2 = K.gemm_nt(ds2b, wo2T)
+                if rows is not None:
+                    datt2 = K.scatter_rows_zero(datt2, rows, M)
                 dq2 = torch.empty_like(q2)
                 dkv = torch.empty_like(kv)
                 delta2 = torch.empty_like(lse2)
@@ -776,14 +802,15 @@
                 one_pass = attn2(0, ask_form=True) != 0
                 aux = AUX.enabled and not (AUX.auto and one_pass)
                 attn2(1 if aux and not one_pass else 0)
-                _param_only(po, K.colsum_bf16, dq2, G["crossattention.self.query.bias"])
+                dq2_r = K.gather_rows_z(dq2, rows) if rows is not None else dq2
+                _param_only(po, K.colsum_bf16, dq2_r, G["crossattention.self.query.bias"])
                 G.alias("crossattention.self.key.bias", G["c.kv_bias"][:Hd])
                 G.alias("crossattention.self.value.bias", G["c.kv_bias"][Hd:])
                 G.alias("crossattention.self.key.weight", G["c.kv_weight"][:Hd])
                 G.alias("crossattention.self.value.weight", G["c.kv_weight"][Hd:])
                 _, wqT = BANK.linear(p[c + "self.query.weight"])
                 _, wkvT = BANK.linear(p[c + "self.key.weight"], p[c + "self.value.weight"])
-                dh1 = K.gemm_nt(dq2, wqT, resid=ds2, out_dtype=F32)
+                dh1 = K.gemm_nt(dq2_r, wqT, resid=ds2, out_dtype=F32)
                 if aux:
                     first = denc is None
                     if first:
@@ -796,15 +823,17 @@
                     kv_done = AUX.launch(kv_side, [q2, kv, att2, datt2, lse2, delta2, dq2, dkv, wkvT, denc])
                 else:
                     denc = K.gemm_nt(dkv, wkvT, resid=denc, out_dtype=F32)
-                tn = [(dkv, encb, G["c.kv_weight"])] + tn + [(ds2b, att2, G["crossattention.output.dense.weight"]),
-                                                            (dq2, h1b, G["crossattention.self.query.weight"])]
+                tn = [(dkv, encb, G["c.kv_weight"])] + tn + [(ds2b, att2_r, G["crossattention.output.dense.weight"]),
+                                                            (dq2_r, h1b, G["crossattention.self.query.weight"])]
             else:
                 dh1 = dh2
-            ds1, ds1b = K.layernorm_bwd(dh1, s1, m1, r1, p[a + "output.LayerNorm.weight"], G["attention.output.LayerNorm.weight"],
-                                        G["attention.output.LayerNorm.bias"], dcol=G["attention.output.dense.bias"], want_bf16=True,
-                                        drop_out=BertLayersFn._drop(meta, i, 1))
+            ds1, ds1b = BertLayersFn._ln_bwd_out(dh1, s1, m1, r1, p[a + "output.LayerNorm.weight"], G["attention.output.LayerNorm.weight"],
+                                                 G["attention.output.LayerNorm.bias"], G["attention.output.dense.bias"],
+                                                 BertLayersFn._drop(meta, i, 1), rows)
             _, woT = BANK.linear(p[a + "output.dense.weight"])
             datt = K.gemm_nt(ds1b, woT)
+            if rows is not None:
+                datt = K.scatter_rows_zero(datt, rows, M)
             dqkv = torch.empty_like(qkv)
             delta = torch.empty_like(lse)
             if meta.get("self_mask2d") is not None:
@@ -820,8 +849,11 @@
                 G.alias("attention.self.%s.bias" % nm, G["a.qkv_bias"][k3 * Hd:(k3 + 1) * Hd])
                 G.alias("attention.self.%s.weight" % nm, G["a.qkv_weight"][k3 * Hd:(k3 + 1) * Hd])
             _, wqkvT = BANK.linear(p[a + "self.query.weight"], p[a + "self.key.weight"], p[a + "self.value.weight"])
-            dh = K.gemm_nt(dqkv, wqkvT, resid=ds1, out_dtype=F32)
-            tn += [(ds1b, att, G["attention.output.dense.weight"]), (dqkv, hb, G["a.qkv_weight"])]
+            if rows is not None:
+                dh = K.add_rows(ds1, rows, K.gemm_nt(dqkv, wqkvT, out_dtype=F32))
+            else:
+                dh = K.gemm_nt(dqkv, wqkvT, resid=ds1, out_dtype=F32)
+            tn += [(ds1b, att_r, G["attention.output.dense.weight"]), (dqkv, hb, G["a.qkv_weight"])]
             if cr is not None:
                 if kv_done is not None and WGRAD_QUEUE is None:
                     torch.cuda.current_stream().wait_event(kv_done)
diff --git a/x2-vlm_amd/kernels.py b/x2-vlm_amd/kernels.py
--- a/x2-vlm_amd/kernels.py
+++ b/x2-vlm_amd/kernels.py
@@ -139,6 +139,21 @@
         call("x2_gemm_nt", ptr(A), ptr(B), ptr(out), M, N, K, _rows(A), _rows(B), _rows(out), ptr(bias), ptr(gamma),
              ptr(resid), _rows(resid) if resid is not None else 0, ptr(aux), _rows(aux) if aux is not None else 0,
              act, 1 if out.dtype == F32 else 0, drop[0], drop[1], drop[2], ptr(drop[3]), ptr(rowscale), ptr(colsum))
+    return out
+
+
+def gemm_nt_rows(A, B, drop_rows, *, bias=None, resid=None, out_dtype=BF16, drop=NO_DROP, colsum=None):
+    assert A.dtype == BF16 and B.dtype == BF16 and A.shape[1] == B.shape[1]
+    M, K = A.shape
+    N = B.shape[0]
+    assert drop_rows.dtype == torch.int32 and drop_rows.numel() == M and drop_rows.is_contiguous()
+    assert bias is None or (bias.dtype == F32 and bias.numel() == N and bias.is_contiguous())
+    assert resid is None or (resid.dtype == F32 and resid.shape == (M, N))
+    out = torch.empty(M, N, device=A.device, dtype=out_dtype)
+    with _timed(2.0 * M * N * K):
+        call("x2_gemm_nt_rows", ptr(A), ptr(B), ptr(out), M, N, K, _rows(A), _rows(B), _rows(out), ptr(bias), ptr(resid),
+             _rows(resid) if resid is not None else 0, 1 if out.dtype == F32 else 0, drop[0], drop[1], drop[2], ptr(drop[3]),
+             ptr(colsum), ptr(drop_rows))
     return out
 
 
@@ -346,6 +361,22 @@
     return dx, dxb
 
 
+def layernorm_bwd_rows(dy, x, mean, rstd, w, dw, db, drop_rows, *, dcol=None, drop_out=NO_DROP):
+    assert dy.dtype == F32 and x.dtype == F32 and dy.is_contiguous() and x.is_contiguous() and dy.shape == x.shape
+    D = x.shape[-1]
+    R = mean.numel()
+    assert drop_rows.dtype == torch.int32 and drop_rows.numel() == R and drop_rows.is_contiguous()
+    dx = torch.empty_like(x)
+    dxb = torch.empty(x.shape, device=x.device, dtype=BF16)
+    nblk = (R + 15) // 16
+    ws, defer = _ws_and_defer(x.device, nblk * 3 * D)
+    call("x2_layernorm_bwd_rows", ptr(dy), ptr(x), ptr(mean), ptr(rstd), ptr(w), ptr(dx), ptr(dxb), ptr(dw), ptr(db), ptr(dcol), R, D,
+         drop_out[0], drop_out[1], drop_out[2], ptr(drop_out[3]), ptr(drop_rows), ptr(ws), defer)
+    if defer:
+        DEFERRED.append((ws, nblk, 3, D, (dw, db, dcol)))
+    return dx, dxb
+
+
 def colsum_bf16(y, out):
     nblk = (y.shape[0] + 63) // 64
     ws, defer = _ws_and_defer(y.device, nblk * y.shape[1])
@@ -520,6 +551,43 @@
     assert src.dtype == F32 and src.is_contiguous() and idx.dtype == torch.int32 and src.numel() == idx.numel() * row_len
     dst = torch.empty(rows, row_len, device=src.device, dtype=F32)
     call("x2_scatter_rows", ptr(src), ptr(idx), ptr(dst), idx.numel(), rows, row_len)
+    return dst
+
+
+def fusion_rows(masked_pos, S, L, n_cls):
+    B, n = masked_pos.shape
+    assert masked_pos.dtype == torch.int64 and masked_pos.is_contiguous() and B <= S and n_cls <= S
+    dev = masked_pos.device
+    rows = torch.empty(n_cls + B * n, device=dev, dtype=torch.int32)
+    slot = torch.empty(n_cls + B * n, device=dev, dtype=torch.int32)
+    call("x2_fusion_rows", ptr(masked_pos), B, n, S, L, n_cls, ptr(rows), ptr(slot))
+    return rows, slot
+
+
+def _row_table(src, rows):
+    assert src.dim() == 2 and src.is_contiguous() and src.dtype in (BF16, F32) and rows.dtype == torch.int32 and rows.is_contiguous()
+    return src.shape[1] * src.element_size()
+
+
+def gather_rows_z(src, rows):
+    nbytes = _row_table(src, rows)
+    out = torch.empty(rows.numel(), src.shape[1], device=src.device, dtype=src.dtype)
+    call("x2_gather_rows_z", ptr(src), ptr(rows), ptr(out), rows.numel(), src.shape[0], nbytes)
+    return out
+
+
+def scatter_rows_zero(src, rows, D):
+    nbytes = _row_table(src, rows)
+    assert src.shape[0] == rows.numel()
+    out = torch.empty(D, src.shape[1], device=src.device, dtype=src.dtype)
+    call("x2_scatter_rows_zero", ptr(src), ptr(rows), ptr(out), rows.numel(), D, nbytes)
+    return out
+
+
+def add_rows(src, rows, dst):
+    _row_table(src, rows)
+    assert src.dtype == F32 and dst.dtype == F32 and dst.is_contiguous() and dst.shape[1] == src.shape[1] and src.shape[0] == rows.numel()
+    call("x2_add_rows", ptr(src), ptr(rows), ptr(dst), rows.numel(), dst.shape[0], src.shape[1])
     return dst
 
 
diff --git a/x2-vlm_amd/model_pretrain.py b/x2-vlm_amd/model_pretrain.py
--- a/x2-vlm_amd/model_pretrain.py
+++ b/x2-vlm_amd/model_pretrain.py
@@ -39,12 +39,20 @@
             t_idx, kv = (torch.cat([ar, ar, tneg, ar + B]), torch.cat([ar, ineg, ar, ar])) if ret_match_loss else (ar + B, ar)
             atts, enc_atts = torch.cat([text_atts, text_atts])[t_idx.long()], image_atts[kv.long()]
         h0 = ops.gather_rows(both, t_idx)
-        fused = self.get_cross_embeds(image_embeds, enc_atts, text_embeds=h0, text_atts=atts, kv_idx=kv)
-        if ret_match_loss:
-            loss_itm = self._itm_loss(fused[:3 * B, 0, :], B)
+        if self.fusion_rows and both.is_cuda:
+            S, L = h0.shape[:2]
+            n_cls = 3 * B if ret_match_loss else 0
+            rows, slot = K.fusion_rows(masked_pos.long().contiguous(), S, L, n_cls)
+            fused = self.get_cross_embeds(image_embeds, enc_atts, text_embeds=h0, text_atts=atts, kv_idx=kv, out_rows=rows)
+            loss_itm = self._itm_loss(fused[:n_cls], B) if ret_match_loss else torch.tensor(0.0)
+            loss_mlm, self.last_mlm_lse, self.last_mlm_logits = self.text_encoder.mlm_loss_from_rows(fused, slot[n_cls:], masked_ids)
         else:
-            loss_itm = torch.tensor(0.0)
-        loss_mlm, self.last_mlm_lse, self.last_mlm_logits = self.text_encoder.mlm_loss_from_hidden(fused[-B:], masked_pos, masked_ids)
+            fused = self.get_cross_embeds(image_embeds, enc_atts, text_embeds=h0, text_atts=atts, kv_idx=kv)
+            if ret_match_loss:
+                loss_itm = self._itm_loss(fused[:3 * B, 0, :], B)
+            else:
+                loss_itm = torch.tensor(0.0)
+            loss_mlm, self.last_mlm_lse, self.last_mlm_logits = self.text_encoder.mlm_loss_from_hidden(fused[-B:], masked_pos, masked_ids)
         loss = {"loss_itc": loss_itc, "loss_itm": loss_itm, "loss_mlm": loss_mlm}
         self.last = dict(image_embeds=image_embeds.detach(), text_embeds=text_embeds.detach(), image_feat=image_feat.detach(),
                          text_feat=text_feat.detach())
diff --git a/x2-vlm_amd/xbert.py b/x2-vlm_amd/xbert.py
--- a/x2-vlm_amd/xbert.py
+++ b/x2-vlm_amd/xbert.py
@@ -125,7 +125,7 @@
         self.config = config
         self.layer = nn.ModuleList([BertLayer(config, i) for i in range(config.num_hidden_layers)])
 
-    def run(self, hidden, text_atts, enc=None, enc_atts=None, mode="multi_modal", kv_idx=None):
+    def run(self, hidden, text_atts, enc=None, enc_atts=None, mode="multi_modal", kv_idx=None, out_rows=None):
         cfg = self.config
         lo, hi = {"text": (0, cfg.fusion_layer), "fusion": (cfg.fusion_layer, cfg.num_hidden_layers),
                   "multi_modal": (0, cfg.num_hidden_layers)}[mode]
@@ -135,7 +135,7 @@
             drop = dict(seed=next_dropout_seed(), p_hidden=cfg.hidden_dropout_prob, p_attn=cfg.attention_probs_dropout_prob)
         meta = dict(lo=lo, hi=hi, fusion_at=cfg.fusion_layer, heads=cfg.num_attention_heads, eps=cfg.layer_norm_eps,
                     self_mask=None, self_mask2d=None, enc_mask=None, kv_idx=None,
-                    seq_off=None, seq_ids=None, drop=drop)
+                    seq_off=None, seq_ids=None, drop=drop, out_rows=out_rows)
         meta["self_mask"], meta["self_mask2d"] = _text_masks(text_atts)
         cross = enc is not None and hi > cfg.fusion_layer
         if cross:
@@ -182,7 +182,7 @@
         return self.embeddings.word_embeddings
 
     def forward(self, input_ids=None, attention_mask=None, encoder_embeds=None, encoder_hidden_states=None,
-                encoder_attention_mask=None, return_dict=True, mode="multi_modal", kv_idx=None, position_ids=None, **unused):
+                encoder_attention_mask=None, return_dict=True, mode="multi_modal", kv_idx=None, position_ids=None, out_rows=None, **unused):
         _refuse_unused("BertModel", unused)
         hidden = self.embeddings(input_ids, position_ids) if encoder_embeds is None else encoder_embeds
         S, L = hidden.shape[:2]
@@ -190,7 +190,7 @@
             attention_mask = torch.ones(S, L, device=hidden.device)
         if encoder_hidden_states is not None and encoder_attention_mask is None:
             encoder_attention_mask = torch.ones(S, encoder_hidden_states.shape[1], device=hidden.device)
-        out = self.encoder.run(hidden, attention_mask, encoder_hidden_states, encoder_attention_mask, mode, kv_idx)
+        out = self.encoder.run(hidden, attention_mask, encoder_hidden_states, encoder_attention_mask, mode, kv_idx, out_rows)
         return SimpleNamespace(last_hidden_state=out) if return_dict else (out,)
 
 
@@ -229,6 +229,13 @@
         B, L, Hd = sequence_output.shape
         flat = (torch.arange(B, device=masked_pos.device).unsqueeze(1) * L + masked_pos).reshape(-1)
         rows = ops.gather_rows(sequence_output.reshape(B * L, Hd), flat)
+        pr = self.cls.predictions
+        return MlmLossFn.apply(rows, labels, self.config.layer_norm_eps, keep_logits, pr.transform.dense.weight, pr.transform.dense.bias,
+                               pr.transform.LayerNorm.weight, pr.transform.LayerNorm.bias, pr.bias,
+                               self.bert.embeddings.word_embeddings.weight)
+
+    def mlm_loss_from_rows(self, rows_out, slot, labels, keep_logits=False):
+        rows = ops.gather_rows(rows_out, slot)
         pr = self.cls.predictions
         return MlmLossFn.apply(rows, labels, self.config.layer_norm_eps, keep_logits, pr.transform.dense.weight, pr.transform.dense.bias,
                                pr.transform.LayerNorm.weight, pr.transform.LayerNorm.bias, pr.bias,
diff --git a/x2-vlm_amd/xvlm.py b/x2-vlm_amd/xvlm.py
--- a/x2-vlm_amd/xvlm.py
+++ b/x2-vlm_amd/xvlm.py
@@ -177,15 +177,29 @@
     def get_text_embeds_12L(self, text_ids, text_atts, **unused):
         return self._bert(text_ids, attention_mask=text_atts).last_hidden_state
 
-    def get_cross_embeds(self, image_embeds, image_atts, text_ids=None, text_embeds=None, text_atts=None, kv_idx=None, **unused):
+    def get_cross_embeds(self, image_embeds, image_atts, text_ids=None, text_embeds=None, text_atts=None, kv_idx=None, out_rows=None,
+                         **unused):
         assert text_atts is not None
         if text_embeds is not None:
             return self._bert(encoder_embeds=text_embeds, attention_mask=text_atts, encoder_hidden_states=image_embeds,
-                              encoder_attention_mask=image_atts, mode="fusion", kv_idx=kv_idx).last_hidden_state
+                              encoder_attention_mask=image_atts, mode="fusion", kv_idx=kv_idx, out_rows=out_rows).last_hidden_state
         if text_ids is not None:
             return self._bert(text_ids, attention_mask=text_atts, encoder_hidden_states=image_embeds,
-                              encoder_attention_mask=image_atts, kv_idx=kv_idx).last_hidden_state
+                              encoder_attention_mask=image_atts, kv_idx=kv_idx, out_rows=out_rows).last_hidden_state
         raise ValueError
+
+    fusion_rows = os.environ.get("X2_FUSION_ROWS", "1") != "0"
+
+    def _cls_rows(self, S, L, device):
+        if not (self.fusion_rows and device.type == "cuda"):
+            return None
+        cache = self.__dict__.setdefault("_cls_row_tables", {})
+        rows = cache.get((S, L, device))
+        if rows is None:
+            rows = (torch.arange(S, device=device, dtype=torch.int32) * L).contiguous()
+            if not torch.cuda.is_current_stream_capturing():
+                cache[(S, L, device)] = rows
+        return rows
 
     def get_features(self, image_embeds=None, text_embeds=None):
         fi = ft = None
@@ -244,8 +258,10 @@
 
     def _fusion_cls(self, image_embeds, image_atts, text_embeds, text_atts, t_idx, kv):
         h0 = ops.gather_rows(text_embeds, t_idx)
-        out = self.get_cross_embeds(image_embeds, image_atts[kv.long()], text_embeds=h0, text_atts=text_atts[t_idx.long()], kv_idx=kv)
-        return out[:, 0, :]
+        rows = self._cls_rows(h0.shape[0], h0.shape[1], h0.device)
+        out = self.get_cross_embeds(image_embeds, image_atts[kv.long()], text_embeds=h0, text_atts=text_atts[t_idx.long()], kv_idx=kv,
+                                    out_rows=rows)
+        return out if rows is not None else out[:, 0, :]
 
     def _itm_loss(self, cls, B):
         logits = ops.mlp_head(self.itm_head, cls)
@@ -265,7 +281,10 @@
     def predict_bbox(self, image_embeds, text_embeds, text_atts):
         assert image_embeds.size(0) == text_embeds.size(0)
         ones = torch.ones(image_embeds.shape[:2], device=image_embeds.device)
-        cls = self.get_cross_embeds(image_embeds, ones, text_embeds=text_embeds, text_atts=text_atts)[:, 0, :]
+        rows = self._cls_rows(text_embeds.shape[0], text_embeds.shape[1], text_embeds.device)
+        cls = self.get_cross_embeds(image_embeds, ones, text_embeds=text_embeds, text_atts=text_atts, out_rows=rows)
+        if rows is None:
+            cls = cls[:, 0, :]
         return ops.mlp_head(self.bbox_head, cls).sigmoid()
 
     def get_bbox_loss(self, output_coord, target_bbox, is_image=None):
```

Result: no change. 2938 (median of 6 runs) (+1.0%).
